# rahul003/dmlc-core

Measured on AMD Instinct MI355X. Metric: parsed rows/sec (LibSVM->CSR in device memory), aggregate over GPUs, higher is better.
Workload: dtype fp32 values / u32 indices (text parse, no matmul)

## Files before the change

dmlc_core_amd/data/__init__.py:

```python
from __future__ import annotations

from typing import Dict, Iterator, Optional

from .. import _dmlc

__all__ = ["Parser", "RowBlockIter", "GPUParser", "ShuffledGPUParser", "DeviceCSR", "csr_to_torch",
           "iter_blocks", "write_synthetic", "to_sparse_csr", "GPUBlockDataset", "PageCache",
           "write_page_cache", "RowBatches", "row_order"]

write_synthetic = _dmlc.write_synthetic
pack_text = _dmlc.pack_text
pack_isa_supported = _dmlc.pack_isa_supported
unpack_text_reference = _dmlc.unpack_text_reference
unpack_text_device = _dmlc.unpack_text_device


def _host_blocks_uri(uri: str) -> str:
    q = uri.split("#", 1)[0]
    if "?" not in q:
        return uri
    args = dict(kv.split("=", 1) for kv in q.split("?", 1)[1].split("&") if "=" in kv)
    if not args.get("device", "").startswith("gpu") or "to_host" in args:
        return uri
    head, _, tail = uri.partition("#")
    return head + "&to_host=1" + ("#" + tail if tail else "")


def Parser(uri: str, part: int = 0, nparts: int = 1, type: str = "auto",
           index64: bool = False):
    cls = _dmlc.Parser64 if index64 else _dmlc.Parser
    return cls(_host_blocks_uri(uri), part, nparts, type)


def RowBlockIter(uri: str, part: int = 0, nparts: int = 1, type: str = "auto",
                 index64: bool = False):
    cls = _dmlc.RowBlockIter64 if index64 else _dmlc.RowBlockIter
    return cls(_host_blocks_uri(uri), part, nparts, type)


def iter_blocks(uri: str, part: int = 0, nparts: int = 1, type: str = "auto",
                index64: bool = False) -> Iterator[Dict]:
    p = Parser(uri, part, nparts, type, index64)
    while p.next():
        yield p.value()


def DeviceCSR(index64: bool = False):
    return _dmlc.DeviceCSR64() if index64 else _dmlc.DeviceCSR()


def PageCache(path: str, device: int = -1, index64: bool = False):
    cls = _dmlc.PageCache64 if index64 else _dmlc.PageCache
    return cls.open(path, device)


def write_page_cache(csr, path: str, page_mb: float = 64.0) -> int:
    cls = _dmlc.PageCache64 if isinstance(csr, _dmlc.DeviceCSR64) else _dmlc.PageCache
    return cls.write(csr, path, page_mb)


class GPUParser:

    def __init__(self, uri: str, part: int = 0, nparts: int = 1, format: str = "libsvm",
                 index64: bool = False, **config):
        cfg = {"format": format}
        cfg.update({k: str(v) for k, v in config.items()})
        self.index64 = index64
        self._where = {"uri": uri, "part": part, "nparts": nparts, "format": format}
        cls = _dmlc.DeviceParser64 if index64 else _dmlc.DeviceParser
        self._p = cls(uri, part, nparts, cfg)

    def parse_all(self, out=None):
        if out is None:
            out = DeviceCSR(self.index64)
        self._p.parse_all(out)
        return out

    def parse_all_hashed(self, dim: int, seed: int = 0, fp8: bool = True, scale: float = 1.0,
                         strategy: str = "auto", out: Optional[Dict] = None):
        import torch
        import torch.utils.dlpack as tdl

        if strategy not in ("auto", "fused", "csr"):
            raise ValueError(f"strategy must be auto, fused or csr, not {strategy!r}")
        if strategy == "csr":
            from .. import ops

            t = csr_to_torch(self.parse_all())
            x = ops.hashed_dense(t, int(dim), seed=seed, fp8=fp8, scale=scale)
            return {"x": x, "label": t["label"].clone(), "batch": None}

        handle = out.get("batch") if isinstance(out, dict) else out
        if handle is not None and torch.cuda.is_available():
            if getattr(self, "_ext_stream", None) is None:
                self._ext_stream = torch.cuda.ExternalStream(self._p.stream())
            self._ext_stream.wait_stream(torch.cuda.current_stream())
        d = self._p.parse_all_hashed(int(dim), float(scale), int(seed) & 0xFFFFFFFF, bool(fp8), handle)
        if isinstance(out, dict) and out.get("batch") is d["batch"] and "x" in out:
            x0 = out["x"]
            if (tuple(x0.shape) == (d["rows"], d["dim"]) and x0.data_ptr() == d["x_ptr"]
                    and out["label"].data_ptr() == d["label_ptr"]
                    and (x0.dtype == torch.float8_e4m3fn) == bool(fp8)):
                return out
        x = tdl.from_dlpack(d["x"]).view(d["rows"], d["dim"])
        if fp8:
            x = x.view(torch.float8_e4m3fn)
        return {"x": x, "label": tdl.from_dlpack(d["label"]), "batch": d["batch"]}

    def before_first(self):
        self._p.before_first()

    def tell(self) -> int:
        return self._p.tell()

    def seek(self, cursor: int) -> None:
        self._p.seek(int(cursor))

    def state_dict(self) -> Dict:
        return dict(self._where, cursor=self.tell())

    def load_state_dict(self, state: Dict) -> None:
        for k in ("uri", "part", "nparts", "format"):
            if state[k] != self._where[k]:
                raise ValueError(f"state is for {k}={state[k]!r}, parser has {self._where[k]!r}")
        self.seek(state["cursor"])

    def next(self) -> bool:
        return self._p.next()

    def value_to_host(self) -> Dict:
        return self._p.value_to_host()

    def value_torch(self) -> Dict:
        import torch.utils.dlpack as tdl

        return {k: None if c is None else tdl.from_dlpack(c)
                for k, c in self._p.value_capsules().items()}

    def stream(self) -> int:
        return self._p.stream()

    def stats(self) -> Dict:
        return self._p.stats()

    @property
    def partition_bytes(self) -> int:
        return self._p.partition_bytes()


class ShuffledGPUParser(GPUParser):

    def __init__(self, uri: str, part: int = 0, nparts: int = 1, num_shuffle_parts: int = 2,
                 shuffle_seed: int = 0, format: str = "libsvm", index64: bool = False,
                 **config):
        if num_shuffle_parts < 1:
            raise ValueError("num_shuffle_parts must be >= 1")
        self.k, self.seed = int(num_shuffle_parts), int(shuffle_seed)
        super().__init__(uri, part, nparts, format=format, index64=index64,
                         shuffle_parts=self.k, shuffle_seed=self.seed, **config)
        self._where.update(num_shuffle_parts=self.k, shuffle_seed=self.seed)

    @property
    def order(self):
        return list(self._p.visit_order())

    @property
    def epoch(self) -> int:
        return self._p.epoch()

    def state_dict(self) -> Dict:
        return dict(self._where, epoch=self.epoch, cursor=self.tell())

    def load_state_dict(self, state: Dict) -> None:
        for k in ("uri", "part", "nparts", "format", "num_shuffle_parts", "shuffle_seed"):
            if state[k] != self._where[k]:
                raise ValueError(f"state is for {k}={state[k]!r}, parser has {self._where[k]!r}")
        self._p.set_epoch(int(state["epoch"]))
        self.seek(state["cursor"])


def csr_to_torch(csr) -> Dict[str, Optional["object"]]:
    import torch.utils.dlpack as tdl

    out = {}
    for k, cap in csr.capsules().items():
        out[k] = None if cap is None else tdl.from_dlpack(cap)
    return out


def to_sparse_csr(t: Dict, num_cols: Optional[int] = None):
    import torch

    offset = t["offset"]
    crow = (offset.view(torch.int64) if offset.dtype == torch.uint64 else offset).to(torch.int64)
    crow = crow - crow[0]
    idx = t["index"]
    if idx.dtype == torch.uint32:
        col = idx.view(torch.int32).to(torch.int64)
    elif idx.dtype == torch.uint64:
        col = idx.view(torch.int64)
    else:
        col = idx.to(torch.int64)
    base = int(offset[0].item()) if offset.numel() else 0
    nnz = int(crow[-1].item()) if crow.numel() else 0
    col = col[base:base + nnz]
    val = t.get("value")
    val = torch.ones(nnz, dtype=torch.float32, device=col.device) if val is None else val[base:base + nnz]
    ncols = int(num_cols) if num_cols is not None else (int(col.max().item()) + 1 if nnz else 0)
    return torch.sparse_csr_tensor(crow, col, val, size=(crow.numel() - 1, ncols))


class GPUBlockDataset:

    def __init__(self, uri: str, part: int = 0, nparts: int = 1, format: str = "libsvm",
                 epochs: int = 1, **config):
        self.args = (uri, part, nparts, format, config)
        self.epochs = epochs

    def __iter__(self):
        uri, part, nparts, fmt, config = self.args
        p = GPUParser(uri, part, nparts, format=fmt, **config)
        for epoch in range(self.epochs):
            if epoch:
                p.before_first()
            while p.next():
                yield p.value_torch()


def row_order(n_rows: int, seed: int, epoch: int):
    import torch

    if n_rows < 0 or epoch < 0:
        raise ValueError("n_rows and epoch must be >= 0")
    g = torch.Generator(device="cpu")
    g.manual_seed((int(seed) * 1000003 + int(epoch)) % (1 << 32))
    return torch.randperm(int(n_rows), generator=g, dtype=torch.int64)


class RowBatches:

    def __init__(self, csr_dict: Dict, batch_rows: int, shuffle: bool = True, seed: int = 0,
                 drop_last: bool = False, buffers: int = 2):
        if batch_rows < 1:
            raise ValueError("batch_rows must be >= 1")
        if buffers < 1:
            raise ValueError("buffers must be >= 1")
        self.csr = csr_dict
        self.n_rows = int(csr_dict["offset"].numel()) - 1
        self.batch_rows, self.shuffle, self.seed = int(batch_rows), bool(shuffle), int(seed)
        self.drop_last, self.buffers = bool(drop_last), int(buffers)
        self.epoch, self._next = 0, 0
        self._out = [None] * self.buffers
        self._order = None

    def __len__(self) -> int:
        if self.drop_last:
            return self.n_rows // self.batch_rows
        return (self.n_rows + self.batch_rows - 1) // self.batch_rows

    def set_epoch(self, epoch: int) -> None:
        if epoch < 0:
            raise ValueError("epoch must be >= 0")
        self.epoch, self._next = int(epoch), 0

    def batch_bounds(self, k: int):
        if not 0 <= k < len(self):
            raise IndexError(f"batch {k} of {len(self)}")
        b = k * self.batch_rows
        return b, min(self.n_rows, b + self.batch_rows)

    def state_dict(self) -> Dict:
        return {"seed": self.seed, "epoch": self.epoch, "next_batch": self._next,
                "batch_rows": self.batch_rows, "n_rows": self.n_rows}

    def load_state_dict(self, state: Dict) -> None:
        for k in ("seed", "batch_rows", "n_rows"):
            if state[k] != getattr(self, k):
                raise ValueError(f"state is for {k}={state[k]!r}, iterator has {getattr(self, k)!r}")
        nb = int(state["next_batch"])
        if not 0 <= nb <= len(self):
            raise ValueError(f"state is for next_batch={nb}, iterator has {len(self)} batches")
        self.epoch, self._next = int(state["epoch"]), nb

    def _device_order(self):
        import torch

        if self._order is None or self._order[0] != (self.epoch, self.shuffle):
            dev = self.csr["index"].device
            if self.shuffle:
                order = row_order(self.n_rows, self.seed, self.epoch).to(dev)
            else:
                order = torch.arange(self.n_rows, dtype=torch.int64, device=dev)
            self._order = ((self.epoch, self.shuffle), order)
        return self._order[1]

    def _gather(self, rows, slot: int) -> Dict:
        from .. import ops

        out = self._out[slot]
        if out is None or out["_buffers"]["offset"].numel() < rows.numel() + 2:
            return ops.gather_rows(self.csr, rows)
        try:
            return ops.gather_rows(self.csr, rows, out=self._out[slot])
        except ops._GatherOutTooSmall as e:
            grown = ops.gather_buffers(self.csr, self.batch_rows, e.nnz + e.nnz // 4)
            return ops.gather_rows(self.csr, rows, out=grown)

    def __iter__(self):
        order = self._device_order() if len(self) > self._next else None
        while self._next < len(self):
            k = self._next
            b, e = self.batch_bounds(k)
            item = self._gather(order[b:e], k % self.buffers)
            self._out[k % self.buffers] = item
            self._next = k + 1
# ... 3 lines not shown
```

include/dmlc/gpu/device_parser.h:

```cpp
#ifndef DMLC_GPU_DEVICE_PARSER_H_
#define DMLC_GPU_DEVICE_PARSER_H_

#include <map>
#include <memory>
#include <string>
#include <vector>

#include "./device_row_block.h"

namespace dmlc {
namespace gpu {

struct DeviceParserConfig {
  std::string format{"libsvm"};
  size_t chunk_bytes{64UL << 20};
  int pinned_slots{3};
  int device_slots{3};
  int read_threads{8};
  int device{-1};
  int label_column{-1};
  int weight_column{-1};
  char delimiter{','};
  bool fast_path{true};
  bool one_pass{false};
  bool hash_one_pass{false};
  bool prelaunch{true};
  int zero_copy{-1};
  int packed_h2d{-1};
  bool pack_wait{false};
  bool pack_head{true};
  int copy_streams{2};
  size_t zc_pin_budget{64UL << 30};
  size_t zc_window_bytes{1UL << 30};
  bool hbm_cache{false};
  size_t replay_chunk_bytes{(2UL << 30) - (64UL << 20)};
  size_t replay_first_bytes{0};
  double wait_spin_us{50};
  unsigned shuffle_parts{1};
  int shuffle_seed{0};
  void Update(const std::map<std::string, std::string>& args);
};

struct DeviceHashedBatch {
  std::shared_ptr<DeviceBuffer> x{std::make_shared<DeviceBuffer>()};
  std::shared_ptr<DeviceBuffer> label{std::make_shared<DeviceBuffer>()};
  size_t rows{0}, row_cap{0};
  int dim{0};
  bool fp8{true};
  int device{0};
  void Reserve(size_t rows, hipStream_t stream);
};

struct DeviceParserStats {
  size_t bytes{0};
  size_t chunks{0};
  size_t rows{0};
  size_t nnz{0};
  size_t exact_chunks{0};
  size_t one_pass_chunks{0};
  size_t one_pass_reruns{0};
  double wait_reader_sec{0};
  double wait_gpu_sec{0};
  bool zero_copy{false};
  double register_sec{0};
  size_t zc_pin_budget{0}, zc_pinned_peak{0};
  double last_pass_sec{0}, last_fill_sec{0}, last_drain_sec{0};
  size_t waits_spun{0}, waits_slept{0}, waits_timed_out{0};
  size_t packed_chunks{0}, raw_chunks{0}, link_bytes{0}, exception_blocks{0};
  size_t head_packed{0};
  double pack_sec{0}, wait_pack_sec{0}, wait_pack_idle_sec{0};
  size_t unpack_staging_bytes{0};
};

template <typename IndexType>
class DeviceParser {
 public:
  static DeviceParser* Create(const std::string& uri, unsigned part_index, unsigned num_parts,
                              const DeviceParserConfig& cfg = DeviceParserConfig());
  virtual ~DeviceParser() = default;
  virtual void BeforeFirst() = 0;
  virtual size_t Tell() const = 0;
  virtual void Seek(size_t cursor) = 0;
  virtual unsigned Epoch() const { return 0; }
  virtual void SetEpoch(unsigned ) {}
  virtual std::vector<unsigned> VisitOrder() const { return {0}; }
  virtual bool Next() = 0;
  virtual const DeviceRowBlock<IndexType>& Value() const = 0;
  virtual void ParseAll(DeviceCSR<IndexType>* out) = 0;
  virtual void ParseAllHashed(DeviceHashedBatch* out, int dim, float scale, uint32_t seed,
                              bool fp8) = 0;
  virtual size_t PartitionBytes() const = 0;
  virtual const DeviceParserStats& Stats() const = 0;
  virtual hipStream_t stream() const = 0;
};

}
}
#endif
```

src/gpu/chunk_feed.cc:

```cpp
#include "./chunk_feed.h"

#include <dmlc/fault.h>
#include <dmlc/logging.h>
#include <dmlc/timer.h>

#include <algorithm>
#include <cstring>

#include "../io/filesys.h"
#include "../io/line_split.h"
#include "./kernels.h"
#include "./text_pack.h"

namespace dmlc {
namespace gpu {

ChunkFeed::ChunkFeed(const std::string& uri, unsigned part, unsigned nparts,
                     const DeviceParserConfig& cfg, bool csv_alphabet, hipStream_t compute,
                     DeviceParserStats* stats)
    : cfg_(cfg),
      compute_(compute),
      stats_(stats),
      walk_(&plan_, cfg.replay_first_bytes, cfg.replay_chunk_bytes) {
  io::URI path(uri.c_str());
  split_.reset(new io::LineSplitter(io::FileSystem::GetInstance(path), uri.c_str(), part, nparts));
  if (cfg_.shuffle_parts > 1) {
    const unsigned k = cfg_.shuffle_parts;
    std::vector<std::vector<EpochOrder::Segment>> subs;
    for (unsigned i = 0; i < k; ++i) {
      split_->ResetPartition(part * k + i, nparts * k);
      subs.push_back(split_->ShardSegments());
    }
    order_ = EpochOrder(part, nparts, k, cfg_.shuffle_seed, subs);
    reader_.reset(new io::ShardReader(split_.get(), cfg_.read_threads, order_.Segments(),
                                      order_.Stops()));
  } else {
    order_ = EpochOrder(part, nparts, 1, cfg_.shuffle_seed, {split_->ShardSegments()});
    reader_.reset(new io::ShardReader(split_.get(), cfg_.read_threads));
  }
  ncopy_ = (cfg_.copy_streams == 1 || cfg_.hbm_cache) ? 1 : 2;
  for (size_t s = 0; s < ncopy_; ++s) copy_[s].reset(new Stream());
  zeroed_.reset(new Event());
  for (int d = 0; d < cfg_.device_slots; ++d) {
    dtext_.emplace_back(new DeviceBuffer(cfg_.chunk_bytes + kTextPadBytes));
    MemsetOrdered(dtext_.back()->get(), cfg_.chunk_bytes + kTextPadBytes);
    copied_.emplace_back(new Event());
    parsed_.emplace_back(new Event());
    parsed_.back()->Record(compute_);
  }
  iter_.set_max_capacity(static_cast<size_t>(cfg_.pinned_slots));
  if (cfg_.zero_copy != 0) {
    zc_.reset(new ZeroCopySource());
    const double t0 = GetTime();
    zc_->SetDrain([this]() {
      RescueLookahead();
      SyncCopyStreams();
    });
    stats_->zc_pin_budget = ZeroCopySource::ShardPinBudget(cfg_.zc_pin_budget);
    if (!zc_->Init(split_.get(), cfg_.chunk_bytes, stats_->zc_pin_budget, cfg_.zc_window_bytes,
                   order_.shuffled() ? &order_.all_segments() : nullptr)) {
      CHECK(cfg_.zero_copy != 1) << "zero_copy=1 but the input cannot be mmap'ed + registered";
      zc_.reset();
    } else {
      stats_->register_sec = GetTime() - t0;
      stats_->zero_copy = true;
      if (order_.shuffled()) zc_->Reorder(order_.SegmentIndices());
    }
  }
  if (zc_ == nullptr) StartReader();
  if (zc_ != nullptr &&
      (cfg_.packed_h2d == 1 ||
       (cfg_.packed_h2d < 0 && cfg_.read_threads >= 2 && cfg_.chunk_bytes >= (size_t(1) << 20)))) {
    StartPacking(csv_alphabet);
  }
  if (cfg_.hbm_cache) StartCaching();
}

ChunkFeed::~ChunkFeed() {
  for (auto& s : copy_) {
    if (s) (void)hipStreamSynchronize(s->get());
  }
  if (unpack_) (void)hipStreamSynchronize(unpack_->get());
  (void)hipStreamSynchronize(compute_);
  for (auto& f : inflight_) {
    if (f.slot != nullptr) iter_.Recycle(&f.slot);
  }
  inflight_.clear();
  iter_.Destroy();
  pool_.reset();
  zc_.reset();
}

void ChunkFeed::SyncCopyStreams() const {
  for (size_t s = 0; s < ncopy_; ++s) copy_[s]->Synchronize();
}

void ChunkFeed::MemsetOrdered(void* ptr, size_t bytes) {
  DMLC_HIP_CHECK(hipMemsetAsync(ptr, 0, bytes, copy_[0]->get()));
  if (ncopy_ < 2) return;
  zeroed_->Record(copy_[0]->get());
  DMLC_HIP_CHECK(hipStreamWaitEvent(copy_[1]->get(), zeroed_->get(), 0));
}

bool ChunkFeed::SetEpoch(unsigned e) {
  if (head_) DropLookahead();
  if (!order_.shuffled()) return Seek(0);
  DrainInflight();
  order_.Apply(e);
  if (zc_ != nullptr) {
    zc_->Reorder(order_.SegmentIndices());
  } else {
    reorder_reader_ = true;
  }
  return Seek(0);
}

bool ChunkFeed::Seek(size_t cursor) {
  CHECK_LE(cursor, PartitionBytes()) << "DeviceParser::Seek: cursor beyond the partition";
  const bool keep_prelaunch = cursor == 0 && cache_complete_ && !order_.shuffled();
  if (cursor == 0 && reader_done_ && inflight_.empty() && busy_ == 0 && cursor_ != 0 &&
      cursor_ == PartitionBytes()) {
    head_armed_ = true;
  }
  const bool adopt = head_ && cursor == 0 && !(cfg_.hbm_cache && cache_complete_);
  DrainInflight(adopt);
  replay_ = false;
  caching_ = false;
  if (cfg_.hbm_cache) {
    if (cache_complete_) {
      plan_.Build(order_);
      const size_t i = plan_.FindCursor(cursor, PartitionBytes());
      if (i != ReplayPlan::kNotABoundary) {
        replay_ = true;
        walk_.Start(i);
        cursor_ = cursor;
        return keep_prelaunch;
      }
    } else if (cursor == 0) {
      StartCaching();
    } else {
      plan_.Clear();
      arena_fill_ = 0;
    }
  }
  if (zc_ != nullptr) {
    if (!adopt) zc_->Seek(cursor);
  } else {
    seek_pos_ = cursor;
    iter_.BeforeFirst();
  }
  cursor_ = cursor;
  return keep_prelaunch;
}

void ChunkFeed::StartReader() {
  const size_t cap = cfg_.chunk_bytes;
  io::ShardReader* reader = reader_.get();
  iter_.Init(
      [reader, cap](HostSlot** dptr) {
        if (*dptr == nullptr) {
          *dptr = new HostSlot();
          (*dptr)->buf.Reserve(cap + kTextPadBytes);
          (*dptr)->cap = cap;
        }
        ScopedRange r("pinned_fill");
        HostSlot* slot = *dptr;
        size_t n = reader->Fill(slot->buf.get<char>(), slot->cap);
        while (n == io::ShardReader::kNeedMore) {
          slot->cap = reader->NeedCapacity();
          slot->buf.Free();
          slot->buf.Reserve(slot->cap + kTextPadBytes);
          n = reader->Fill(slot->buf.get<char>(), slot->cap);
        }
        (*dptr)->size = n;
        (*dptr)->end_pos = reader->Tell();
        return (*dptr)->size != 0;
      },
      [this, reader]() {
        if (reorder_reader_) {
          reader->SetSegments(order_.Segments(), order_.Stops());
          reorder_reader_ = false;
        }
        reader->Seek(seek_pos_);
      });
}

bool ChunkFeed::NextPiece(Piece* out) {
  if (pool_ != nullptr) {
    out->job = NextPackJob();
    if (out->job == nullptr) return false;
    out->src = out->job->ptr;
    out->size = out->job->size;
    out->end_pos = out->job->end_pos;
  } else if (zc_ != nullptr) {
    ZeroCopySource::Piece piece;
    if (!zc_->Next(&piece)) return false;
    out->src = piece.ptr;
    out->size = piece.size;
    out->end_pos = zc_->Tell();
  } else {
    const double t0 = GetTime();
    if (!iter_.Next(&out->slot)) return false;
    stats_->wait_reader_sec += GetTime() - t0;
    out->src = out->slot->buf.get();
    out->size = out->slot->size;
    out->end_pos = out->slot->end_pos;
  }
  return true;
}

void ChunkFeed::FillFromCache() {
  while (static_cast<int>(inflight_.size()) < cfg_.device_slots && !walk_.AtEnd()) {
    const ReplayPlan::Step s = walk_.Next(merge_);
    inflight_.push_back(
        Inflight{nullptr, -1, s.size, s.end_pos, arena_->get<char>() + s.off, -1, false});
  }
  reader_done_ = walk_.AtEnd();
}

size_t ChunkFeed::CacheChunk(const Piece& p) {
  const size_t begin_pos = plan_.cached_end();
  CHECK_LE(arena_fill_ + p.size, arena_bytes_) << "HBM cache arena overflow";
  const char last = p.job != nullptr ? p.job->last
                    : p.size != 0    ? static_cast<const char*>(p.src)[p.size - 1]
                                     : '\n';
  CachedChunk c{arena_fill_, p.size, begin_pos, p.end_pos, 0, 0, 0, last == '\n' || last == '\r'};
  c.sub = order_.SubOf(begin_pos, &c.sub_begin);
  c.sub_end = c.sub_begin + (p.end_pos - begin_pos);
  CHECK_LE(c.sub_end, order_.sub_bytes(c.sub)) << "internal error: a chunk spans two sub-shards";
  plan_.Add(c);
  arena_fill_ += p.size;
  return c.off;
}

void ChunkFeed::FillPipeline() {
  if (replay_) {
    FillFromCache();
    return;
  }
  while (static_cast<int>(inflight_.size()) + busy_ < cfg_.device_slots && !reader_done_) {
    if (pool_ != nullptr && !PreparePackJob()) break;
    if (zc_ != nullptr) DMLC_FAULT_POINT("read");
    DMLC_FAULT_POINT("h2d");
    Piece p;
    if (!NextPiece(&p)) {
      reader_done_ = true;
      if (caching_) cache_complete_ = true;
      QueueHeadJobs();
      break;
    }
    const PackJob* job = p.job.get();
    const size_t size = p.size;
    const int d = next_dslot_;
    next_dslot_ = (next_dslot_ + 1) % cfg_.device_slots;
    if (size + kTextPadBytes > dtext_[d]->bytes()) {
      parsed_[d]->Synchronize();
      dtext_[d].reset(new DeviceBuffer(size + kTextPadBytes));
      MemsetOrdered(dtext_[d]->get(), size + kTextPadBytes);
    }
    char* dst = dtext_[d]->get<char>();
    if (caching_) dst = arena_->get<char>() + CacheChunk(p);
    const size_t cs = pass_chunks_++ % ncopy_;
    hipStream_t copy = copy_[cs]->get();
    DMLC_HIP_CHECK(hipStreamWaitEvent(copy, parsed_[d]->get(), 0));
    int pack_slot = -1;
    const bool packed = job != nullptr && job->state.load() == PackJob::kPacked;
    if (packed) {
      if (dstage_[d] == nullptr || dstage_[d]->bytes() < job->packed_bytes) {
        parsed_[d]->Synchronize();
        if (dstage_[d] != nullptr) stats_->unpack_staging_bytes -= dstage_[d]->bytes();
        dstage_[d].reset(
            new DeviceBuffer(std::max(job->packed_bytes, PackSlotBytes(cfg_.chunk_bytes))));
        stats_->unpack_staging_bytes += dstage_[d]->bytes();
      }
      DMLC_HIP_CHECK(hipMemcpyAsync(dstage_[d]->get(), job->out, job->packed_bytes,
                                    hipMemcpyHostToDevice, copy));
      copied_[d]->Record(copy);
      DMLC_HIP_CHECK(hipStreamWaitEvent(unpack_->get(), copied_[d]->get(), 0));
      LaunchUnpackText(dstage_[d]->get(), size, job->nexc, alphabet_, dst, unpack_->get());
      unpacked_[d]->Record(unpack_->get());
      pack_slot = job->slot;
      stats_->packed_chunks += 1;
      if (job->head && job->seq == 0) stats_->head_packed += 1;
      stats_->exception_blocks += job->nexc;
      stats_->link_bytes += job->packed_bytes;
    } else {
      DMLC_HIP_CHECK(hipMemcpyAsync(dst, p.src, size, hipMemcpyHostToDevice, copy));
      stats_->raw_chunks += 1;
      stats_->link_bytes += size;
      if (job != nullptr) {
        if (job->rescued) {
          pack_slot = job->slot;
        } else {
          free_pack_slots_.push_back(job->slot);
        }
      }
      copied_[d]->Record(copy);
    }
    last_copy_d_[cs] = d;
    inflight_.push_back(Inflight{p.slot, d, size, p.end_pos, dst, pack_slot, packed});
  }
}

void ChunkFeed::StartPacking(bool csv_alphabet) {
  PackAlphabet(csv_alphabet, cfg_.delimiter, alphabet_);
  pool_.reset(new PackPool(cfg_.read_threads, alphabet_, 0));
  pack_slots_ =
      std::vector<PinnedBuffer>(kPackLookahead + static_cast<size_t>(cfg_.device_slots) + 1);
  for (size_t i = 0; i < pack_slots_.size(); ++i) free_pack_slots_.push_back(static_cast<int>(i));
  dstage_.resize(static_cast<size_t>(cfg_.device_slots));
  unpack_.reset(new Stream());
  for (int d = 0; d < cfg_.device_slots; ++d) unpacked_.emplace_back(new Event());
}

size_t ChunkFeed::PackSlotBytes(size_t n, bool may_hold_raw) const {
  const size_t packed = static_cast<size_t>(kPackMaxRatio * static_cast<double>(n)) + 64;
  return std::max<size_t>(may_hold_raw ? std::max(packed, n) : packed, 4096);
}

bool ChunkFeed::LinkBusy() const {
  for (size_t s = 0; s < ncopy_; ++s) {
    if (last_copy_d_[s] >= 0 && !copied_[last_copy_d_[s]]->Query()) return true;
  }
  return false;
}

void ChunkFeed::FetchLookahead(size_t limit, bool head) {
  while (!la_end_ && la_.size() < limit) {
    ZeroCopySource::Piece piece;
    if (!zc_->Next(&piece)) {
      la_end_ = true;
      break;
    }
    std::unique_ptr<PackJob> job(new PackJob());
    job->ptr = piece.ptr;
    job->size = piece.size;
    job->end_pos = zc_->Tell();
    if (piece.size != 0) job->last = piece.ptr[piece.size - 1];
    job->seq = la_seq_++;
    job->head = head;
    CHECK(!free_pack_slots_.empty()) << "internal error: no free pack slot";
    job->slot = free_pack_slots_.back();
    free_pack_slots_.pop_back();
    PinnedBuffer& buf = pack_slots_[job->slot];
    if (buf.bytes() < PackSlotBytes(piece.size, zc_->windowed())) {
      buf.Reserve(PackSlotBytes(std::max(piece.size, cfg_.chunk_bytes), zc_->windowed()));
    }
    job->out = buf.get<uint8_t>();
    la_.push_back(std::move(job));
  }
}

void ChunkFeed::QueueHeadJobs() {
  if (pool_ == nullptr || !cfg_.pack_head || !head_armed_ || cfg_.pack_wait ||
      cfg_.shuffle_parts > 1 || zc_->windowed() || (cfg_.hbm_cache && cache_complete_)) {
    return;
  }
  CHECK(la_.empty()) << "internal error: lookahead left at the end of a pass";
  la_seq_ = submitted_ = la_pushed_ = 0;
  la_end_ = front_unpushed_ = false;
  pool_->SetSubmitted(0);
  zc_->Seek(0);
  FetchLookahead(kHeadJobs, true);
  for (; la_pushed_ < la_.size(); ++la_pushed_) pool_->Push(la_[la_pushed_].get());
  head_ = true;
}

bool ChunkFeed::PreparePackJob() {
  FetchLookahead(kPackLookahead, false);
  if (la_.empty()) return true;
  PackJob* job = la_.front().get();
  const int state = job->state.load();
  next_action_ = job->rescued ? SubmitAction::kSubmit
                              : DecideSubmit(state, cfg_.pack_wait != 0,
                                             inflight_.empty(), pool_behind_,
                                             [this]() { return LinkBusy(); });
  if (pool_behind_ && !job->rescued) {
    packed_in_a_row_ = state == PackJob::kPacked ? packed_in_a_row_ + 1 : 0;
    if (packed_in_a_row_ >= kPackCaughtUp) SetPoolBehind(false);
  }
  if (la_pushed_ == 0 && next_action_ == SubmitAction::kClaimRaw) {
    front_unpushed_ = true;
    la_pushed_ = 1;
  } else if (front_unpushed_ && next_action_ != SubmitAction::kClaimRaw) {
    front_unpushed_ = false;
    if (job->state.load() == PackJob::kQueued) pool_->Push(job);
  }
  for (; la_pushed_ < la_.size(); ++la_pushed_) {
    if (la_[la_pushed_]->state.load() == PackJob::kQueued) pool_->Push(la_[la_pushed_].get());
  }
  return next_action_ != SubmitAction::kDefer;
}

void ChunkFeed::SetPoolBehind(bool behind) {
  pool_behind_ = behind;
  packed_in_a_row_ = 0;
  pool_->SetDistance(behind ? kPackDistance : 0);
}

std::unique_ptr<PackJob> ChunkFeed::NextPackJob() {
  if (la_.empty()) return nullptr;
  std::unique_ptr<PackJob> job = std::move(la_.front());
  la_.pop_front();
  --la_pushed_;
  front_unpushed_ = false;
  pool_->SetSubmitted(++submitted_);
  if (next_action_ == SubmitAction::kClaimRaw && !pool_->TryClaimRaw(job.get())) {
    next_action_ = SubmitAction::kWait;
  }
  if (next_action_ == SubmitAction::kWait) {
    const bool idle = !LinkBusy();
    const double t0 = GetTime();
    try {
      pool_->Wait(job.get());
    } catch (...) {
      free_pack_slots_.push_back(job->slot);
      throw;
    }
    stats_->wait_pack_sec += GetTime() - t0;
    if (idle) {
      stats_->wait_pack_idle_sec += GetTime() - t0;
      if (WaitMeansPoolBehind(idle, cfg_.pack_wait, job->head && job->seq == 0)) {
        SetPoolBehind(true);
      }
    }
  }
  stats_->pack_sec = pool_->pack_sec();
  return job;
}

void ChunkFeed::RescueLookahead() {
  for (auto& job : la_) {
    if (job->rescued || !zc_->Releasing(job->ptr)) continue;
    if (!pool_->TryClaimRaw(job.get())) {
      try {
        pool_->Wait(job.get());
      } catch (...) {
        job->state.store(PackJob::kRejected);
      }
    }
    if (job->state.load() == PackJob::kPacked) continue;
    std::memcpy(job->out, job->ptr, job->size);
    job->ptr = reinterpret_cast<const char*>(job->out);
    job->rescued = true;
  }
}

void ChunkFeed::DropLookahead() {
  if (pool_ == nullptr) return;
  pool_->Quiesce();
  for (auto& job : la_) free_pack_slots_.push_back(job->slot);
  la_.clear();
  la_end_ = false;
  front_unpushed_ = false;
  head_ = false;
  la_seq_ = submitted_ = la_pushed_ = 0;
  pool_->SetSubmitted(0);
}

void ChunkFeed::ReleasePackSlot(int* pack_slot) {
  if (*pack_slot < 0) return;
  free_pack_slots_.push_back(*pack_slot);
  *pack_slot = -1;
}

void ChunkFeed::StartCaching() {
  plan_.Clear();
  arena_fill_ = 0;
  cache_complete_ = false;
  if (arena_ == nullptr) {
    arena_bytes_ =
        PartitionBytes() + std::max(split_->files().size(), order_.all_segments().size()) + 16;
    arena_.reset(new DeviceBuffer(arena_bytes_ + kTextPadBytes));
    MemsetOrdered(arena_->get(), arena_bytes_ + kTextPadBytes);
  }
  caching_ = true;
}

void ChunkFeed::DrainInflight(bool keep_head) {
  SyncCopyStreams();
  if (unpack_) unpack_->Synchronize();
  DMLC_HIP_CHECK(hipStreamSynchronize(compute_));
  while (!inflight_.empty()) {
    if (inflight_.front().slot != nullptr) iter_.Recycle(&inflight_.front().slot);
    ReleasePackSlot(&inflight_.front().pack_slot);
    inflight_.pop_front();
  }
  ReleasePackSlot(&cur_.pack_slot);
  if (keep_head) {
    head_ = false;
  } else {
    DropLookahead();
  }
  last_copy_d_[0] = last_copy_d_[1] = -1;
  pass_chunks_ = 0;
  reader_done_ = false;
  busy_ = 0;
}

bool ChunkFeed::Acquire(Chunk* out) {
  FillPipeline();
  if (inflight_.empty()) return false;
  cur_ = inflight_.front();
  inflight_.pop_front();
  busy_ = 1;
  if (cur_.d >= 0) {
    Event* ready = cur_.packed ? unpacked_[cur_.d].get() : copied_[cur_.d].get();
    DMLC_HIP_CHECK(hipStreamWaitEvent(compute_, ready->get(), 0));
  }
  out->text = cur_.text;
  out->size = cur_.size;
  out->resident = cur_.d < 0;
  return true;
}

void ChunkFeed::FirstSyncDone() {
  if (cur_.slot != nullptr) iter_.Recycle(&cur_.slot);
  ReleasePackSlot(&cur_.pack_slot);
  FillPipeline();
}

void ChunkFeed::Release(bool delivered) {
  if (!delivered) {
    (void)hipStreamSynchronize(compute_);
    if (cur_.d >= 0) (void)hipEventRecord(parsed_[cur_.d]->get(), compute_);
    busy_ = 0;
    ReleasePackSlot(&cur_.pack_slot);
    if (head_) DropLookahead();
    if (cur_.slot != nullptr) {
      try {
        iter_.Recycle(&cur_.slot);
      } catch (...) {
      }
    }
    return;
  }
  if (cur_.slot != nullptr) iter_.Recycle(&cur_.slot);
  ReleasePackSlot(&cur_.pack_slot);
  if (cur_.d >= 0) parsed_[cur_.d]->Record(compute_);
  busy_ = 0;
  cursor_ = cur_.end_pos;
  stats_->bytes += cur_.size;
  stats_->chunks += 1;
  if (zc_ != nullptr) stats_->zc_pinned_peak = zc_->PeakPinnedBytes();
}

bool ChunkFeed::PeekNextResident(const char** text, size_t* size) const {
  if (inflight_.empty() || inflight_.front().d >= 0) return false;
  *text = inflight_.front().text;
  *size = inflight_.front().size;
  return true;
}

bool ChunkFeed::NextEpochFirst(const char** text, size_t* size) const {
  if (!replay_ || !inflight_.empty() || !reader_done_ || order_.shuffled()) return false;
  ReplayPlan::Step s;
  if (!walk_.NextEpochFirst(merge_, &s) || s.size == 0) return false;
  *text = arena_->get<char>() + s.off;
  *size = s.size;
  return true;
}

}
}
```

src/gpu/chunk_feed.h:

```cpp
#ifndef DMLC_SRC_GPU_CHUNK_FEED_H_
#define DMLC_SRC_GPU_CHUNK_FEED_H_

#include <dmlc/gpu/device_parser.h>
#include <dmlc/gpu/hip_utils.h>
#include <dmlc/threadediter.h>

#include <deque>
#include <memory>
#include <string>
#include <vector>

#include "../io/input_split_base.h"
#include "../io/shard_reader.h"
#include "./epoch_order.h"
#include "./pack_pool.h"
#include "./replay_plan.h"
#include "./zero_copy_source.h"

namespace dmlc {
namespace gpu {

class ChunkFeed {
 public:
  struct Chunk {
    const char* text{nullptr};
    size_t size{0};
    bool resident{false};
  };

  ChunkFeed(const std::string& uri, unsigned part, unsigned nparts, const DeviceParserConfig& cfg,
            bool csv_alphabet, hipStream_t compute, DeviceParserStats* stats);
  ~ChunkFeed();
  ChunkFeed(const ChunkFeed&) = delete;
  ChunkFeed& operator=(const ChunkFeed&) = delete;

  bool Seek(size_t cursor);
  bool SetEpoch(unsigned e);
  bool BeforeFirst() { return order_.shuffled() ? SetEpoch(order_.epoch() + 1) : Seek(0); }
  size_t Tell() const { return cursor_; }
  unsigned Epoch() const { return order_.epoch(); }
  const std::vector<unsigned>& VisitOrder() const { return order_.order(); }
  size_t PartitionBytes() const {
    return zc_ != nullptr ? zc_->PartitionBytes() : reader_->PartitionBytes();
  }

  bool Acquire(Chunk* out);
  void FirstSyncDone();
  void Release(bool delivered);

  bool Replaying() const { return replay_; }
  bool MergingReplay() const { return replay_ && merge_.merge; }
  bool InputDone() const { return reader_done_; }

  bool PeekNextResident(const char** text, size_t* size) const;
  bool NextEpochFirst(const char** text, size_t* size) const;

  class ReplayMerge {
   public:
    ReplayMerge(ChunkFeed* feed, size_t limit) : feed_(feed) {
      feed_->merge_ = ReplayMergeSettings{true, limit};
    }
    ~ReplayMerge() { feed_->merge_ = ReplayMergeSettings(); }
    ReplayMerge(const ReplayMerge&) = delete;
    ReplayMerge& operator=(const ReplayMerge&) = delete;

   private:
    ChunkFeed* feed_;
  };

 private:
  struct HostSlot {
    PinnedBuffer buf;
    size_t cap{0};
    size_t size{0};
    size_t end_pos{0};
  };
  struct Inflight {
    HostSlot* slot;
    int d;
    size_t size;
    size_t end_pos;
    const char* text;
    int pack_slot;
    bool packed;
  };
  struct Piece {
    HostSlot* slot{nullptr};
    const void* src{nullptr};
    size_t size{0}, end_pos{0};
    std::unique_ptr<PackJob> job;
  };
  static constexpr size_t kPackLookahead = 4;
  static constexpr size_t kPackDistance = 2;
  static constexpr size_t kPackCaughtUp = 8;
  static constexpr size_t kHeadJobs = 2;

  void SyncCopyStreams() const;
  void MemsetOrdered(void* ptr, size_t bytes);
  void FetchLookahead(size_t limit, bool head);
  void QueueHeadJobs();
  void StartReader();
  void StartPacking(bool csv_alphabet);
  void StartCaching();
  void FillPipeline();
  void FillFromCache();
  bool NextPiece(Piece* out);
  size_t CacheChunk(const Piece& p);
  size_t PackSlotBytes(size_t n, bool may_hold_raw = false) const;
  bool LinkBusy() const;
  bool PreparePackJob();
  void SetPoolBehind(bool behind);
  std::unique_ptr<PackJob> NextPackJob();
  void RescueLookahead();
  void DropLookahead();
  void ReleasePackSlot(int* pack_slot);
  void DrainInflight(bool keep_head = false);

  DeviceParserConfig cfg_;
  hipStream_t compute_;
  DeviceParserStats* stats_;
  std::unique_ptr<io::InputSplitBase> split_;
  std::unique_ptr<io::ShardReader> reader_;
  EpochOrder order_;
  std::unique_ptr<Stream> copy_[2];
  size_t ncopy_{2};
  size_t pass_chunks_{0};
  std::unique_ptr<Event> zeroed_;
  std::vector<std::unique_ptr<DeviceBuffer>> dtext_;
  std::vector<std::unique_ptr<Event>> copied_, parsed_;
  ThreadedIter<HostSlot> iter_;
  std::unique_ptr<ZeroCopySource> zc_;
  std::unique_ptr<PackPool> pool_;
  std::deque<std::unique_ptr<PackJob>> la_;
  bool la_end_{false};
  size_t la_seq_{0}, submitted_{0};
  size_t la_pushed_{0};
  bool front_unpushed_{false};
  bool pool_behind_{false};
  size_t packed_in_a_row_{0};
  SubmitAction next_action_{SubmitAction::kSubmit};
  bool head_{false};
  bool head_armed_{false};
  int last_copy_d_[2]{-1, -1};
  std::vector<PinnedBuffer> pack_slots_;
  std::vector<int> free_pack_slots_;
  std::vector<std::unique_ptr<DeviceBuffer>> dstage_;
  std::unique_ptr<Stream> unpack_;
  std::vector<std::unique_ptr<Event>> unpacked_;
  uint8_t alphabet_[16];
  std::deque<Inflight> inflight_;
  Inflight cur_{nullptr, -1, 0, 0, nullptr, -1, false};
  int busy_{0};
  int next_dslot_{0};
  bool reader_done_{false};
  size_t cursor_{0};
  bool reorder_reader_{false};
  size_t seek_pos_{0};
  std::unique_ptr<DeviceBuffer> arena_;
  size_t arena_bytes_{0}, arena_fill_{0};
  bool caching_{false}, cache_complete_{false}, replay_{false};
  ReplayPlan plan_;
  ReplayWalk walk_;
  ReplayMergeSettings merge_;
};

}
}
#endif
```

src/gpu/device_parser.cc:

```cpp
#include <dmlc/gpu/device_parser.h>
#include <dmlc/fault.h>
#include <dmlc/logging.h>
#include <dmlc/timer.h>

#include <cstdlib>

#include <algorithm>
#include <cstring>
#include <memory>
#include <vector>

#include "../io/uri_spec.h"
#include "./chunk_feed.h"
#include "./host_wait.h"
#include "./kernels.h"
#include "./tile_pipeline.h"

namespace dmlc {
namespace gpu {

void DeviceParserConfig::Update(const std::map<std::string, std::string>& args) {
  for (const auto& kv : args) {
    const std::string& k = kv.first;
    const std::string& v = kv.second;
    if (k == "chunk_mb") {
      chunk_bytes = static_cast<size_t>(std::atof(v.c_str()) * (1 << 20));
    } else if (k == "chunk_bytes") {
      chunk_bytes = std::strtoull(v.c_str(), nullptr, 10);
    } else if (k == "pinned_slots") {
      pinned_slots = std::atoi(v.c_str());
    } else if (k == "device_slots") {
      device_slots = std::atoi(v.c_str());
    } else if (k == "read_threads") {
      read_threads = std::atoi(v.c_str());
    } else if (k == "device") {
      device = std::atoi(v.c_str());
    } else if (k == "format") {
      format = v;
    } else if (k == "label_column") {
      label_column = std::atoi(v.c_str());
    } else if (k == "weight_column") {
      weight_column = std::atoi(v.c_str());
    } else if (k == "delimiter") {
      CHECK_EQ(v.size(), 1U) << "delimiter must be one character";
      delimiter = v[0];
    } else if (k == "fast_path") {
      fast_path = v != "0" && v != "false";
    } else if (k == "one_pass") {
      one_pass = v != "0" && v != "false";
    } else if (k == "hash_one_pass") {
      hash_one_pass = v != "0" && v != "false";
    } else if (k == "prelaunch") {
      prelaunch = v != "0" && v != "false";
    } else if (k == "replay_chunk_mb") {
      replay_chunk_bytes = static_cast<size_t>(std::atof(v.c_str()) * (1 << 20));
    } else if (k == "replay_first_mb") {
      replay_first_bytes = static_cast<size_t>(std::atof(v.c_str()) * (1 << 20));
    } else if (k == "zc_pin_budget_mb") {
      zc_pin_budget = static_cast<size_t>(std::atof(v.c_str()) * (1 << 20));
    } else if (k == "zc_window_mb") {
      zc_window_bytes = static_cast<size_t>(std::atof(v.c_str()) * (1 << 20));
    } else if (k == "hbm_cache") {
      hbm_cache = v != "0" && v != "false";
    } else if (k == "wait_spin_us") {
      wait_spin_us = std::atof(v.c_str());
    } else if (k == "shuffle_parts") {
      shuffle_parts = static_cast<unsigned>(std::atoi(v.c_str()));
    } else if (k == "shuffle_seed") {
      shuffle_seed = std::atoi(v.c_str());
    } else if (k == "zero_copy") {
      zero_copy = (v == "auto" || v == "-1") ? -1 : ((v == "0" || v == "false") ? 0 : 1);
    } else if (k == "pack_wait") {
      pack_wait = v != "0" && v != "false";
    } else if (k == "pack_head") {
      pack_head = v != "0" && v != "false";
    } else if (k == "copy_streams") {
      copy_streams = std::atoi(v.c_str());
    } else if (k == "packed_h2d") {
      packed_h2d = (v == "auto" || v == "-1") ? -1 : ((v == "0" || v == "false") ? 0 : 1);
    }
  }
  chunk_bytes = (chunk_bytes + 4095) & ~size_t(4095);
  CHECK_GE(chunk_bytes, 4096U) << "chunk_bytes too small";
  CHECK_LT(chunk_bytes, size_t(1) << 31) << "chunk_bytes must be < 2 GiB";
  CHECK_LT(replay_chunk_bytes, size_t(1) << 31) << "replay_chunk_bytes must be < 2 GiB";
  CHECK_GE(pinned_slots, 1);
  CHECK_GE(device_slots, 1);
  CHECK(copy_streams == 1 || copy_streams == 2) << "copy_streams must be 1 or 2";
  CHECK_GE(shuffle_parts, 1U) << "shuffle_parts must be >= 1";
}

namespace {

struct ChunkPlan {
  size_t nlines{0}, ntok{0};
  uint64_t nrows{0}, nnz{0};
  unsigned flags{0};
};

template <typename IndexType>
class DeviceParserImpl : public DeviceParser<IndexType> {
 public:
  DeviceParserImpl(const std::string& uri, unsigned part, unsigned nparts,
                   const DeviceParserConfig& cfg)
      : cfg_(cfg) {
    if (cfg_.device >= 0) SetDevice(cfg_.device);
    DMLC_HIP_CHECK(hipGetDevice(&device_));
    if (cfg_.format == "libsvm") {
      tcfg_.format = TextFormat::kLibSVM;
    } else if (cfg_.format == "libfm") {
      tcfg_.format = TextFormat::kLibFM;
    } else if (cfg_.format == "csv") {
      tcfg_.format = TextFormat::kCSV;
    } else {
      LOG(FATAL) << "DeviceParser: unsupported format " << cfg_.format;
    }
    CHECK(tcfg_.format != TextFormat::kCSV || cfg_.label_column < 0 ||
          cfg_.label_column != cfg_.weight_column)
        << "label_column and weight_column must differ";
    tcfg_.label_column = cfg_.label_column;
    tcfg_.weight_column = cfg_.weight_column;
    tcfg_.delimiter = cfg_.delimiter;
    int least_prio = 0, greatest_prio = 0;
    DMLC_HIP_CHECK(hipDeviceGetStreamPriorityRange(&least_prio, &greatest_prio));
    compute_.reset(new Stream(greatest_prio));
    feed_.reset(new ChunkFeed(uri, part, nparts, cfg_, tcfg_.format == TextFormat::kCSV,
                              compute_->get(), &stats_));
    tiles_.Reserve(LineIndexTiles(cfg_.chunk_bytes) * sizeof(uint64_t));
    pre_.Init(2 * sizeof(ChunkMeta), cfg_.hbm_cache);
    pre_.cur.Reserve(TileCount(cfg_.chunk_bytes), true);
    hmeta_.Reserve(2 * sizeof(ChunkMeta));
    slots_.Reserve(std::max<size_t>(kMaxPartialBlocks, TileScratchSlots(TileCount(cfg_.chunk_bytes))) *
                   sizeof(MetaPartial));
  }

  ~DeviceParserImpl() override {
    if (compute_) (void)hipStreamSynchronize(compute_->get());
    if (pre_.stream) (void)hipStreamSynchronize(pre_.stream->get());
  }

  void BeforeFirst() override {
    if (!feed_->BeforeFirst()) pre_.Drop();
  }
  void SetEpoch(unsigned e) override {
    if (!feed_->SetEpoch(e)) pre_.Drop();
  }
  void Seek(size_t cursor) override {
    if (!feed_->Seek(cursor)) pre_.Drop();
  }
  unsigned Epoch() const override { return feed_->Epoch(); }
  std::vector<unsigned> VisitOrder() const override { return feed_->VisitOrder(); }
  size_t Tell() const override { return feed_->Tell(); }

  bool Next() override {
    block_.Clear();
    block_.device_ = device_;
    ResetEpoch();
    if (!ProcessOne(&block_, false)) return false;
    FinishEpoch(&block_);
    view_ = block_.View();
    return true;
  }

  const DeviceRowBlock<IndexType>& Value() const override { return view_; }

  void ParseAll(DeviceCSR<IndexType>* out) override {
    ScopedRange range("DeviceParser::ParseAll");
    out->device_ = device_;
    ResetEpoch();
    const bool one_pass = cfg_.one_pass && feed_->Replaying() && cfg_.fast_path &&
                          tcfg_.format != TextFormat::kCSV && !one_pass_off_;
    ChunkFeed::ReplayMerge merge(feed_.get(), one_pass ? ResidentMergeLimit() : 0);
    const double t0 = GetTime();
    double t_first = 0, t_last_in = 0;
    while (ProcessOne(out, true)) {
      const double t = GetTime();
      if (t_first == 0) t_first = t;
      if (feed_->InputDone() && t_last_in == 0) t_last_in = t;
    }
    FinishEpoch(out);
    const double t_end = GetTime();
    stats_.last_pass_sec = t_end - t0;
    stats_.last_fill_sec = t_first != 0 ? t_first - t0 : 0;
    stats_.last_drain_sec = t_last_in != 0 ? t_end - t_last_in : 0;
  }

  size_t PartitionBytes() const override { return feed_->PartitionBytes(); }
  const DeviceParserStats& Stats() const override { return stats_; }
  hipStream_t stream() const override { return compute_->get(); }

 private:
  void ResetEpoch() {
    acc_max_index_ = acc_max_field_ = 0;
    acc_flags_ = 0;
  }

  ChunkMeta WaitMapped(ChunkMeta* hm) {
    const double t0 = GetTime();
    const ChunkMeta v = TakePublished(hm, cfg_.wait_spin_us, 0.05, &wait_stats_, [this] {
      compute_->Synchronize();
      if (pre_.stream) pre_.stream->Synchronize();
    });
    stats_.wait_gpu_sec += GetTime() - t0;
    stats_.waits_spun = wait_stats_.spun;
    stats_.waits_slept = wait_stats_.slept;
    stats_.waits_timed_out = wait_stats_.timed_out;
    return v;
  }

  template <typename T>
  T ReadBack(const void* src) {
    const double t0 = GetTime();
    DMLC_HIP_CHECK(hipMemcpyAsync(hmeta_.get(), src, sizeof(T), hipMemcpyDeviceToHost,
                                  compute_->get()));
    compute_->Synchronize();
    stats_.wait_gpu_sec += GetTime() - t0;
    T v;
    std::memcpy(&v, hmeta_.get(), sizeof(T));
    return v;
  }

  size_t ForPartition(uint64_t n, size_t nbytes, double margin) const {
    const double scale =
        static_cast<double>(PartitionBytes()) / std::max<size_t>(nbytes, 1) * margin;
    return static_cast<size_t>(n * scale) + 1;
  }

  size_t ResidentMergeLimit() const {
    return std::min(2 * cfg_.replay_chunk_bytes, (size_t(1) << 31) - (size_t(64) << 20));
  }

  void EnsureScratch(size_t nbytes) {
    const size_t tiles = TileCount(nbytes);
    pre_.cur.Reserve(tiles, true);
    slots_.Reserve(std::max<size_t>(kMaxPartialBlocks, TileScratchSlots(tiles)) * sizeof(MetaPartial));
    tiles_.Reserve(LineIndexTiles(nbytes) * sizeof(uint64_t));
  }

  void EnsureLineBuffers(size_t nlines) {
    lines_.Reserve((nlines + 1) * sizeof(uint32_t));
    info_.Reserve((nlines + 1) * sizeof(uint64_t));
    partials_.Reserve((ScanPartials(nlines) + 2) * sizeof(uint64_t));
  }

  FillTarget<IndexType> MakeFillTarget(DeviceCSR<IndexType>* out, size_t row_base, size_t nnz_base,
                                       size_t row_limit, size_t nnz_limit, bool with_qid) {
    FillTarget<IndexType> tgt;
    tgt.offset = out->offset();
    tgt.label = out->label();
    tgt.weight = out->weight_capacity() >= out->row_capacity() && out->row_capacity() != 0
                     ? out->weight()
                     : nullptr;
    tgt.qid = with_qid ? out->qid() : nullptr;
    tgt.field = tcfg_.format == TextFormat::kLibFM ? out->field() : nullptr;
    tgt.index = out->index();
    tgt.value = out->value();
    tgt.row_base = row_base;
    tgt.nnz_base = nnz_base;
    tgt.row_limit = row_limit;
    tgt.nnz_limit = nnz_limit;
    return tgt;
  }

  FillTarget<IndexType> PrepareOutput(DeviceCSR<IndexType>* out, size_t row_base, size_t nnz_base,
                                      const ChunkPlan& plan, bool need_weight, size_t nbytes) {
    hipStream_t s = compute_->get();
    const bool libfm = tcfg_.format == TextFormat::kLibFM;
    if (row_base == 0) {
      out->Reserve(ForPartition(plan.nrows, nbytes, 1.05), ForPartition(plan.nnz, nbytes, 1.05),
                   libfm, s, 0, 0);
    }
    out->Reserve(row_base + plan.nrows, nnz_base + plan.nnz, libfm, s, row_base, nnz_base);
    if (need_weight) out->EnableWeight(s);
    if (plan.flags & kFlagQid) {
      out->EnableQid(s);
      out->has_qid_ = true;
    }
    return MakeFillTarget(out, row_base, nnz_base, row_base + plan.nrows, nnz_base + plan.nnz,
                          out->has_qid_);
  }

  void LaunchCountScan(const char* text, size_t nbytes, const TileScratchSet& set, hipStream_t s) {
    uint64_t* counts = set.counts.get<uint64_t>();
    uint32_t* flags = set.flags.get<uint32_t>();
    uint32_t* masks = set.masks.get<uint32_t>();
    if (tcfg_.format == TextFormat::kCSV) {
      LaunchCsvTileCount(text, nbytes, tcfg_.label_column, tcfg_.weight_column, tcfg_.delimiter,
                         counts, flags, masks, s);
      LaunchTileScanRaw(counts, flags, TileCount(nbytes), set.dmeta(), set.hmeta(), s);
    } else {
      LaunchTileCountScan(text, nbytes, counts, flags, masks, set.dmeta(), set.hmeta(), s);
    }
  }

  void CountScanCurrent(const char* text, size_t nbytes) {
    if (pre_.Adopt(text, nbytes, compute_->get())) return;
    pre_.Drop();
    LaunchCountScan(text, nbytes, pre_.cur, compute_->get());
  }

  bool FastParse(const char* text, size_t nbytes, DeviceCSR<IndexType>* out, size_t row_base,
                 size_t nnz_base, ChunkPlan* plan) {
    hipStream_t s = compute_->get();
    CountScanCurrent(text, nbytes);
    ChunkMeta* dmeta = pre_.cur.dmeta();
    ChunkMeta* hm = pre_.cur.hmeta();
    const ChunkMeta sizes = WaitMapped(hm);
    feed_->FirstSyncDone();
    if (sizes.flags & kFlagIrregular) return false;
    plan->nlines = sizes.nlines;
    plan->nrows = sizes.nrows;
    plan->nnz = sizes.nnz;
    if (tcfg_.format == TextFormat::kLibSVM) plan->flags |= sizes.flags & kFlagQid;
    bool need_weight = false;
    for (;;) {
      FillTarget<IndexType> tgt = PrepareOutput(out, row_base, nnz_base, *plan, need_weight, nbytes);
      if (tgt.qid != nullptr && plan->nrows != 0) {
        DMLC_HIP_CHECK(hipMemsetAsync(tgt.qid + row_base, 0, plan->nrows * sizeof(uint64_t), s));
      }
      LaunchTileFill<IndexType>(text, nbytes, tcfg_.format, pre_.cur.counts.get<uint64_t>(),
                                pre_.cur.masks.get<uint32_t>(), tgt,
                                slots_.get<MetaPartial>(), dmeta, hm, s);
      PrelaunchCount();
      ChunkMeta m = WaitMapped(hm);
      if (m.flags & kFlagIrregular) return false;
      if ((m.flags & kFlagNeedWeight) && !need_weight) {
        need_weight = true;
        m.flags &= ~kFlagNeedWeight;
        DMLC_HIP_CHECK(hipMemcpyAsync(dmeta, &sizes, sizeof(ChunkMeta), hipMemcpyHostToDevice, s));
        continue;
      }
      CHECK(!(m.flags & kFlagNeedWeight)) << "internal error: weight column not allocated";
      Accumulate(m);
      return true;
    }
  }

  bool CsvFastParse(const char* text, size_t nbytes, DeviceCSR<IndexType>* out, size_t row_base,
                    size_t nnz_base, ChunkPlan* plan) {
    hipStream_t s = compute_->get();
    const size_t ntiles = TileCount(nbytes);
    CountScanCurrent(text, nbytes);
    ChunkMeta* dmeta = pre_.cur.dmeta();
    ChunkMeta* hm = pre_.cur.hmeta();
    const ChunkMeta sizes = WaitMapped(hm);
    feed_->FirstSyncDone();
    if (sizes.flags & kFlagIrregular) return false;
    plan->nlines = sizes.nrows;
    plan->nrows = sizes.nrows;
    plan->nnz = sizes.nnz;
    const bool need_weight = tcfg_.weight_column >= 0;
    FillTarget<IndexType> tgt = PrepareOutput(out, row_base, nnz_base, *plan, need_weight, nbytes);
    LaunchCsvTileFill<IndexType>(text, nbytes, tcfg_.label_column, tcfg_.weight_column,
                                 tcfg_.delimiter, pre_.cur.counts.get<uint64_t>(),
                                 pre_.cur.masks.get<uint32_t>(), tgt,
                                 slots_.get<MetaPartial>(), s);
    LaunchTileFinish(slots_.get<MetaPartial>(), ntiles, dmeta, hm, tgt.offset, row_base, nnz_base,
                     s);
    PrelaunchCount();
    const ChunkMeta m = WaitMapped(hm);
    if (m.flags & kFlagIrregular) return false;
    Accumulate(m);
    return true;
  }

  ChunkPlan ExactIndex(const char* text, size_t nbytes, bool first_sync_done) {
    hipStream_t s = compute_->get();
    ChunkMeta* dmeta = pre_.cur.dmeta();
    ChunkPlan plan;
    DMLC_HIP_CHECK(hipMemsetAsync(dmeta, 0, sizeof(ChunkMeta), s));
    LaunchLineCount(text, nbytes, tiles_.get<uint64_t>(), dmeta, s);
    plan.nlines = ReadBack<ChunkMeta>(dmeta).nlines;
    if (!first_sync_done) feed_->FirstSyncDone();
    EnsureLineBuffers(plan.nlines);
    LaunchLineEmit(text, nbytes, tiles_.get<uint64_t>(), lines_.get<uint32_t>(), s);
    LaunchTextCount(text, nbytes, lines_.get<uint32_t>(), plan.nlines, tcfg_,
                    info_.get<uint64_t>(), slots_.get<MetaPartial>(), dmeta, s);
    uint64_t* total = partials_.get<uint64_t>() + ScanPartials(plan.nlines) + 1;
    LaunchScanU64(info_.get<uint64_t>(), plan.nlines, partials_.get<uint64_t>(), total, s);
    LaunchMetaFromTotal(total, dmeta, s);
// ... 322 lines not shown
```

src/gpu/kernels.h:

```cpp
#ifndef DMLC_GPU_KERNELS_H_
#define DMLC_GPU_KERNELS_H_

#include <hip/hip_runtime_api.h>

#include <cstddef>
#include <cstdint>

namespace dmlc {
namespace gpu {

constexpr size_t kTextPadBytes = 4096;
constexpr size_t kLineTileBytes = 4096;

enum class TextFormat : int { kLibSVM = 0, kLibFM = 1, kCSV = 2 };

struct TextParseConfig {
  TextFormat format{TextFormat::kLibSVM};
  int label_column{-1};
  int weight_column{-1};
  char delimiter{','};
};

struct ChunkMeta {
  unsigned long long nlines;
  unsigned long long nrows;
  unsigned long long nnz;
  unsigned long long max_index;
  unsigned long long max_field;
  unsigned int flags;
  unsigned int pad;
};
constexpr unsigned kFlagWeight = 1u;
constexpr unsigned kFlagQid = 2u;
constexpr unsigned kFlagValue = 4u;
constexpr unsigned kFlagField = 8u;
constexpr unsigned kFlagNegIndex = 256u;
constexpr unsigned kFlagOverflow = 512u;

struct MetaPartial {
  unsigned long long max_index;
  unsigned long long max_field;
  unsigned int flags;
  unsigned int pad;
};
constexpr int kMaxPartialBlocks = 8192;
void LaunchReducePartials(const MetaPartial* partials, int nblocks, ChunkMeta* meta,
                          hipStream_t stream);

struct CsrView {
  const uint64_t* offset;
  const void* index;
  const float* value;
  const void* field;
  size_t nrows;
  bool index64;
  bool paired;
};

template <typename IndexType>
struct FillTarget {
  uint64_t* offset;
  float* label;
  float* weight;
  uint64_t* qid;
  IndexType* field;
  IndexType* index;
  float* value;
  uint64_t row_base;
  uint64_t nnz_base;
  uint64_t row_limit;
  uint64_t nnz_limit;
};

size_t LineIndexTiles(size_t nbytes);
size_t ScanPartials(size_t n);

void LaunchLineCount(const char* text, size_t nbytes, uint64_t* tile_scratch, ChunkMeta* meta,
                     hipStream_t stream);
void LaunchLineEmit(const char* text, size_t nbytes, const uint64_t* tile_scratch,
                    uint32_t* line_starts, hipStream_t stream);

void LaunchTextCount(const char* text, size_t nbytes, const uint32_t* line_starts,
                     size_t nlines, const TextParseConfig& cfg, uint64_t* line_info,
                     MetaPartial* partials, ChunkMeta* meta, hipStream_t stream);

void LaunchScanU64(uint64_t* data, size_t n, uint64_t* partials, uint64_t* total,
                   hipStream_t stream);

void LaunchMetaFromTotal(const uint64_t* total, ChunkMeta* meta, hipStream_t stream);

template <typename IndexType>
void LaunchTextFill(const char* text, size_t nbytes, const uint32_t* line_starts,
                    size_t nlines, const TextParseConfig& cfg, const uint64_t* line_info,
                    const FillTarget<IndexType>& out, uint64_t nrows, uint64_t nnz,
                    MetaPartial* partials, ChunkMeta* meta, hipStream_t stream);

void LaunchCloseOffsets(uint64_t* offset, uint64_t row_end, uint64_t nnz_end, hipStream_t stream);

constexpr unsigned kFlagIrregular = 1024u;

struct LookBack {
  uint64_t* status;
  unsigned long long* ticket;
  unsigned long long ticket0;
};
constexpr size_t kTileBytes = 8192;
constexpr unsigned kFlagNeedWeight = 2048u;
size_t TileCount(size_t nbytes);
size_t TileScratchWords(size_t ntiles);
size_t TileScratchSlots(size_t ntiles);
void LaunchTileCountScan(const char* text, size_t nbytes, uint64_t* tile_counts,
                         uint32_t* tile_flags, uint32_t* tile_masks, ChunkMeta* meta,
                         ChunkMeta* host_meta, hipStream_t stream);
size_t TileMaskWords(size_t ntiles);
struct FillOnePass : LookBack {};
template <typename IndexType>
size_t LaunchTileFill(const char* text, size_t nbytes, TextFormat format,
                      const uint64_t* tile_prefix, const uint32_t* tile_masks,
                      const FillTarget<IndexType>& out, MetaPartial* partials, ChunkMeta* meta,
                      ChunkMeta* host_meta, hipStream_t stream,
                      const FillOnePass* one_pass = nullptr);

struct HashOnePass : LookBack {
  uint32_t tag;
  uint64_t row_cap;
};
template <typename IndexType>
size_t LaunchTileHashed(const char* text, size_t nbytes, TextFormat format,
                        const uint64_t* tile_prefix, const uint32_t* tile_masks,
                        uint64_t row_base, uint64_t nlines, int dim,
                        float scale, uint32_t seed, bool fp8, void* out, float* labels,
                        MetaPartial* partials, ChunkMeta* meta, ChunkMeta* host_meta,
                        hipStream_t stream, const HashOnePass* one_pass = nullptr);

void LaunchTileScanRaw(uint64_t* tile_counts, uint32_t* tile_flags, size_t ntiles,
                       ChunkMeta* meta, ChunkMeta* host_meta, hipStream_t stream);
void LaunchTileFinish(MetaPartial* partials, size_t nslots, ChunkMeta* meta, ChunkMeta* host_meta,
                      uint64_t* offset, uint64_t row_base, uint64_t nnz_base, hipStream_t stream);

void LaunchCsvTileCount(const char* text, size_t nbytes, int label_column, int weight_column,
                        char delimiter, uint64_t* tile_counts, uint32_t* tile_flags,
                        uint32_t* tile_masks, hipStream_t stream);
template <typename IndexType>
void LaunchCsvTileFill(const char* text, size_t nbytes, int label_column, int weight_column,
                       char delimiter, const uint64_t* tile_prefix, const uint32_t* tile_masks,
                       const FillTarget<IndexType>& out, MetaPartial* partials,
                       hipStream_t stream);

constexpr uint32_t kRecErrTruncated = 1;
constexpr uint32_t kRecErrBadPart = 2;
size_t RecordIOTiles(size_t nwords);
void LaunchRecordIOTileCount(const uint32_t* words, size_t nwords, uint64_t* tile_counts,
                             uint32_t* tile_flags, hipStream_t stream);
struct RecordIOOnePass : LookBack {
  ChunkMeta* meta;
  uint64_t rec_cap;
  uint64_t byte_cap;
};
struct RecordIOCaps {
  ChunkMeta* meta;
  uint64_t rec_cap;
  uint64_t byte_cap;
};
size_t LaunchRecordIOTileFill(const uint32_t* words, size_t nwords, const uint64_t* tile_prefix,
                              uint64_t* offset, uint64_t rec_base, uint8_t* data,
                              uint64_t byte_base, MetaPartial* partials, hipStream_t stream,
                              const RecordIOOnePass* one_pass = nullptr,
                              const RecordIOCaps* caps = nullptr);
void LaunchRecordIOTileCountChain(const uint32_t* words, size_t nwords, uint64_t* tile_counts,
                                  uint32_t* tile_flags, hipStream_t stream);
void LaunchRecordIOGather(const uint8_t* src, const uint64_t* src_off, const uint32_t* len,
                          const uint64_t* dst_off, size_t nrec, uint8_t* dst, hipStream_t stream);

void LaunchHashedDenseFP8(const CsrView& csr, int dim, float scale, uint32_t seed, uint8_t* out,
                          hipStream_t stream);
void LaunchHashedDenseF32(const CsrView& csr, int dim, uint32_t seed, float* out,
                          hipStream_t stream);
template <typename IndexType>
void LaunchTextHashed(const char* text, size_t nbytes, const uint32_t* line_starts, size_t nlines,
                      TextFormat format, const uint64_t* line_info, uint64_t row_base, int dim,
                      float scale, uint32_t seed, bool fp8, void* out, float* labels,
                      MetaPartial* partials, ChunkMeta* meta, hipStream_t stream);
void LaunchCSRSpMV(const CsrView& csr, const float* w, float bias, float* y, hipStream_t stream);
void LaunchCSRSpMVT(const CsrView& csr, const float* d, float* g, hipStream_t stream);
constexpr int kSpMMMaxCols = 256;
void LaunchCSRSpMM(const CsrView& csr, const float* w, const float* bias, int k, float* y,
                   hipStream_t stream);
void LaunchCSRSpMMT(const CsrView& csr, const float* d, int k, float* g, hipStream_t stream);
constexpr int kFFMMaxRank = 32;
constexpr uint32_t kFFMStagedRowEntries = 128;
constexpr uint32_t kFFMErrIndex = 1, kFFMErrField = 2;
void LaunchFFMForward(const CsrView& csr, const float* v, uint64_t features, int num_fields, int k,
                      float* y, int* error, hipStream_t stream);
void LaunchFFMBackward(const CsrView& csr, const float* g, const float* v, uint64_t features,
                       int num_fields, int k, float* dv, hipStream_t stream);
constexpr uint32_t kRankMaxLabel = 31;
constexpr uint32_t kRankWaveGroupRows = 256;
constexpr uint32_t kRankTileRows = 256;
constexpr uint32_t kRankErrGroup = 1, kRankErrLabel = 2;
void LaunchQidFlags(const uint64_t* qid, size_t rows, uint64_t* flag, hipStream_t stream);
void LaunchQidGroupPtr(const uint64_t* qid, size_t rows, const uint64_t* scanned,
                       const uint64_t* total, uint64_t capacity, uint64_t* group_ptr,
                       hipStream_t stream);
void LaunchRankLoss(const float* score, const float* label, const uint64_t* group_ptr, size_t groups,
                    uint64_t rows, bool ndcg_weights, float sigma, float* row_scratch, float* grad,
                    float* loss_g, int64_t* pairs_g, int* error, hipStream_t stream);
void LaunchRankNdcg(const float* score, const float* label, const uint64_t* group_ptr, size_t groups,
                    uint64_t rows, uint32_t k, float* ndcg, int* error, hipStream_t stream);
constexpr int kFmRank = 16;
constexpr int kFmCols = kFmRank + 1;
size_t FmForwardSharedBytes(int dim);
void LaunchFmForward(const uint8_t* x, int64_t rows, int dim, const void* wt_bf16, const float* q,
                     const float* bias, float sx, float* y, float* xv, int num_cus,
                     hipStream_t stream);
void LaunchFmBackward(const uint8_t* x, int64_t rows, int dim, const float* g, const float* xv,
                      int nblocks, float* part, hipStream_t stream);
void LaunchFmPrep(const float* w, const float* v, int dim, void* wt_bf16, float* q,
                  hipStream_t stream);
void LaunchFmReduceGrads(const float* part, int nblocks, int dim, const float* v, float sx,
                         float* z, float* gw, float* gv, hipStream_t stream);
enum FmLoss : int { kFmLogistic = 0, kFmSquared = 1 };
constexpr int kFmFusedMaxDim = 1024;
void LaunchFmFused(const uint8_t* x, int64_t rows, int dim, const void* wt_bf16, const float* q,
                   const float* bias, float sx, const float* label, const float* weight,
                   int loss, float inv_n, int nblocks, float* y, float* part, float* lpart,
                   hipStream_t stream);

void LaunchOffsetRebase(const uint64_t* src_offset, size_t nrows, uint64_t src_base,
                        uint64_t dst_base, uint64_t* dst_offset, hipStream_t stream);
void LaunchPageRebase(uint64_t* offset, size_t nrows, const uint64_t* page_row_end,
                      const uint64_t* page_nnz_base, int npages, hipStream_t stream);
void LaunchCSRTranspose(const CsrView& csr, uint64_t base, uint64_t nnz, uint64_t num_features,
                        uint64_t* col_ptr, uint32_t* row_out, float* val_out, void* scratch,
                        uint32_t* error, hipStream_t stream);
size_t CSRTransposeScratchBytes(uint64_t nnz, uint64_t num_features);
uint64_t CSRTransposeMaxFeatures();
constexpr uint32_t kGatherErrRow = 1;
constexpr uint32_t kGatherErrCapacity = 2;
constexpr uint32_t kGatherErrSource = 4;
uint64_t CSRGatherRunEntries();
size_t CSRGatherScratchWords(size_t n_sel);
void LaunchCSRGatherCount(const uint64_t* offset, uint64_t nrows_src, uint64_t src_entries,
                          const void* rows, bool rows64, size_t n_sel, const float* label,
                          const float* weight, const uint64_t* qid, uint64_t* out_offset,
                          float* out_label, float* out_weight, uint64_t* out_qid, uint32_t* error,
                          hipStream_t stream);
void LaunchCSRGatherFill(const CsrView& src, uint64_t src_entries, const void* rows, bool rows64,
                         size_t n_sel, uint64_t* out_offset, const uint64_t* total,
                         void* out_index, float* out_value, void* out_field,
                         uint64_t out_capacity, uint32_t* error, hipStream_t stream);
constexpr uint64_t kCompactMaxFeatures = 1ull << 32;
constexpr uint32_t kCompactErrIndex = 1;
size_t CompactScratchBytes(uint64_t num_features);
void LaunchCompactMark(const CsrView& csr, uint64_t base, uint64_t nnz, uint64_t num_features,
                       void* scratch, uint32_t* error, hipStream_t stream);
void LaunchCompactCount(uint64_t num_features, void* scratch, uint64_t* total, hipStream_t stream);
void LaunchCompactEmit(uint64_t num_features, const void* scratch, uint64_t capacity, int64_t* ids,
                       hipStream_t stream);
void LaunchCompactRemap(const CsrView& csr, uint64_t base, uint64_t nnz, uint64_t num_features,
                        const void* scratch, int32_t* slot, hipStream_t stream);
enum LazyRule : int { kLazyAdagrad = 0, kLazyFtrl = 1 };
struct LazyHyper {
  float a, b, c, d;
};
constexpr uint32_t kLazyErrIds = 1;
void LaunchLazyUpdate(int rule, float* param, const int64_t* ids, const float* grad, float* state0,
                      float* state1, uint64_t features, uint64_t nrows, uint64_t width,
                      const LazyHyper& hyper, uint32_t* error, hipStream_t stream);
void LaunchFill(float* p, size_t n, float v, hipStream_t stream);
void LaunchUnpackText(const void* packed, size_t n, uint32_t nexc, const uint8_t alphabet[16],
                      char* dst, hipStream_t stream);

}
}
#endif
```

src/gpu/pack_pool.h:

```cpp
#ifndef DMLC_SRC_GPU_PACK_POOL_H_
#define DMLC_SRC_GPU_PACK_POOL_H_

#include <dmlc/fault.h>
#include <dmlc/logging.h>
#include <dmlc/timer.h>

#include <algorithm>
#include <atomic>
#include <condition_variable>
#include <cstring>
#include <deque>
#include <exception>
#include <memory>
#include <mutex>
#include <thread>
#include <vector>

#include "./text_pack.h"

namespace dmlc {
namespace gpu {

struct PackJob {
  enum State : int { kQueued = 0, kPacking, kPacked, kRejected, kClaimedRaw, kFailed };
  const char* ptr{nullptr};
  size_t size{0};
  size_t end_pos{0};
  char last{'\n'};
  size_t seq{0};
  int slot{-1};
  uint8_t* out{nullptr};
  double ratio{kPackMaxRatio};
  std::atomic<int> state{kQueued};
  size_t packed_bytes{0};
  uint32_t nexc{0};
  bool rescued{false};
  bool head{false};
};

enum class SubmitAction : int {
  kSubmit = 0,
  kClaimRaw,
  kWait,
  kDefer
};

template <typename LinkBusy>
inline SubmitAction DecideSubmit(int state, bool pack_wait, bool nothing_inflight,
                                 bool pool_behind, LinkBusy&& link_busy) {
  if (state == PackJob::kFailed) return SubmitAction::kWait;
  if (state != PackJob::kQueued && state != PackJob::kPacking) return SubmitAction::kSubmit;
  if (pack_wait) return SubmitAction::kWait;
  if (!nothing_inflight && !pool_behind && link_busy()) return SubmitAction::kDefer;
  return state == PackJob::kQueued ? SubmitAction::kClaimRaw : SubmitAction::kWait;
}

inline bool WaitMeansPoolBehind(bool link_idle, bool pack_wait, bool head_of_pass) {
  return link_idle && !pack_wait && !head_of_pass;
}

class PackPool {
 public:
  static constexpr size_t kRangeBlocks = 1024;
  static constexpr size_t kCopyBlocks = 1024;

  PackPool(int threads, const uint8_t alphabet[16], size_t distance,
           size_t range_blocks = kRangeBlocks)
      : nthreads_(std::max(threads, 1)),
        distance_(distance),
        range_blocks_(std::max<size_t>(range_blocks, 1)),
        encoder_(alphabet) {
    std::memcpy(alphabet_, alphabet, 16);
    for (int t = 0; t < nthreads_; ++t) workers_.emplace_back([this]() { Work(); });
  }
  ~PackPool() {
    {
      std::unique_lock<std::mutex> lk(mu_);
      queue_.clear();
      cv_done_.wait(lk, [&] { return nopen_ == 0; });
      stop_ = true;
    }
    cv_work_.notify_all();
    for (auto& w : workers_) w.join();
  }
  PackPool(const PackPool&) = delete;
  PackPool& operator=(const PackPool&) = delete;

  void Push(PackJob* job) {
    {
      std::lock_guard<std::mutex> lk(mu_);
      queue_.push_back(job);
    }
    cv_work_.notify_all();
  }
  void SetDistance(size_t distance) { distance_.store(distance, std::memory_order_relaxed); }
  void SetSubmitted(size_t n) { submitted_.store(n, std::memory_order_relaxed); }
  bool TryClaimRaw(PackJob* job) {
    std::lock_guard<std::mutex> lk(mu_);
    int expect = PackJob::kQueued;
    if (!job->state.compare_exchange_strong(expect, PackJob::kClaimedRaw)) return false;
    queue_.erase(std::remove(queue_.begin(), queue_.end(), job), queue_.end());
    return true;
  }
  void Wait(PackJob* job) {
    std::unique_lock<std::mutex> lk(mu_);
    cv_done_.wait(lk, [&] {
      const int st = job->state.load();
      return st != PackJob::kPacking && st != PackJob::kQueued;
    });
    if (job->state.load() == PackJob::kFailed) {
      std::exception_ptr e = error_;
      error_ = nullptr;
      lk.unlock();
      if (e) std::rethrow_exception(e);
      LOG(FATAL) << "text pack failed";
    }
  }
  void Quiesce() {
    std::unique_lock<std::mutex> lk(mu_);
    queue_.clear();
    cv_done_.wait(lk, [&] { return nopen_ == 0; });
    error_ = nullptr;
  }
  double pack_sec() const { return pack_sec_.load(std::memory_order_relaxed); }

 private:
  struct Open {
    PackJob* job{nullptr};
    size_t nranges{0};
    size_t order{0};
    long exc_limit{0};
    std::atomic<size_t> next{0}, done{0};
    std::atomic<long> exc_total{0};
    std::atomic<bool> fits{true};
    std::vector<std::vector<uint32_t>> exc;
    std::vector<uint32_t> all;
    bool copying{false};
    int result{PackJob::kRejected};
    std::exception_ptr err;
  };
  static constexpr int kOpenJobs = 2;

  Open* ClaimLocked(size_t* range) {
    Open* order[kOpenJobs] = {&open_[0], &open_[1]};
    if (order[1]->job != nullptr && (order[0]->job == nullptr || order[1]->order < order[0]->order)) {
      std::swap(order[0], order[1]);
    }
    for (Open* o : order) {
      if (o->job == nullptr || o->next.load(std::memory_order_relaxed) >= o->nranges) continue;
      const size_t r = o->next.fetch_add(1);
      if (r < o->nranges) {
        *range = r;
        return o;
      }
    }
    return nullptr;
  }
  bool OpenLocked() {
    Open* o = open_[0].job == nullptr ? &open_[0] : open_[1].job == nullptr ? &open_[1] : nullptr;
    while (o != nullptr && !queue_.empty()) {
      PackJob* job = queue_.front();
      queue_.pop_front();
      const size_t distance = distance_.load(std::memory_order_relaxed);
      if (distance != 0 && job->seq < submitted_.load(std::memory_order_relaxed) + distance) {
        continue;
      }
      int expect = PackJob::kQueued;
      if (!job->state.compare_exchange_strong(expect, PackJob::kPacking)) continue;
      o->job = job;
      o->nranges = std::max<size_t>(1, (PackBlocks(job->size) + range_blocks_ - 1) / range_blocks_);
      o->order = ++opened_;
      o->exc_limit = PackMaxExceptions(job->size, job->ratio);
      o->next.store(0);
      o->done.store(0);
      o->exc_total.store(0);
      o->fits.store(o->exc_limit >= 0);
      if (o->exc.size() < o->nranges) o->exc.resize(o->nranges);
      o->err = nullptr;
      o->copying = false;
      o->result = PackJob::kRejected;
      try {
        DMLC_FAULT_POINT("pack");
      } catch (...) {
        o->err = std::current_exception();
        o->fits.store(false);
      }
      if (nopen_++ == 0) open_since_ = GetTime();
      return true;
    }
    return false;
  }
  void RunRange(Open* o, size_t r) {
    const PackJob* job = o->job;
    const uint8_t* text = reinterpret_cast<const uint8_t*>(job->ptr);
    if (o->copying) {
      PackCopyExceptions(text, job->size, o->all, r * kCopyBlocks,
                         std::min(o->all.size(), (r + 1) * kCopyBlocks), job->out);
      return;
    }
    std::vector<uint32_t>& exc = o->exc[r];
    exc.clear();
    if (!o->fits.load(std::memory_order_relaxed)) return;
    const size_t b0 = r * range_blocks_;
    const size_t b1 = std::min(PackBlocks(job->size), b0 + range_blocks_);
    if (!PackRange(text, job->size, b0, b1, encoder_, job->out + sizeof(PackedHeader), &exc,
                   &o->exc_total, o->exc_limit)) {
      o->fits.store(false, std::memory_order_relaxed);
    }
  }
  bool FinishPack(Open* o) {
    PackJob* job = o->job;
    if (!o->fits.load()) return false;
    try {
      o->all.clear();
      for (size_t r = 0; r < o->nranges; ++r) {
        o->all.insert(o->all.end(), o->exc[r].begin(), o->exc[r].end());
      }
      if (static_cast<long>(o->all.size()) > o->exc_limit) return false;
      job->packed_bytes = PackFinishHeader(job->size, alphabet_, o->all, job->out);
      job->nexc = static_cast<uint32_t>(o->all.size());
      o->result = PackJob::kPacked;
      const size_t ncopy = (o->all.size() + kCopyBlocks - 1) / kCopyBlocks;
      if (ncopy <= 1) {
        PackCopyExceptions(reinterpret_cast<const uint8_t*>(job->ptr), job->size, o->all, 0,
                           o->all.size(), job->out);
        return false;
      }
      {
        std::lock_guard<std::mutex> lk(mu_);
        o->copying = true;
        o->nranges = ncopy;
        o->done.store(0);
        o->next.store(1);
      }
      cv_work_.notify_all();
      return true;
    } catch (...) {
      std::lock_guard<std::mutex> lk(mu_);
      if (!o->err) o->err = std::current_exception();
      return false;
    }
  }
  void Settle(Open* o) {
    {
      std::lock_guard<std::mutex> lk(mu_);
      int result = o->result;
      if (o->err) {
        error_ = o->err;
        result = PackJob::kFailed;
      }
      o->job->state.store(result);
      o->job = nullptr;
      if (--nopen_ == 0) {
        pack_sec_.store(pack_sec_.load(std::memory_order_relaxed) + (GetTime() - open_since_),
                        std::memory_order_relaxed);
      }
    }
    cv_done_.notify_all();
    cv_work_.notify_all();
  }
  void Work() {
    for (;;) {
      Open* o = nullptr;
      size_t r = 0;
      {
        std::unique_lock<std::mutex> lk(mu_);
        for (;;) {
          if (stop_) return;
          if ((o = ClaimLocked(&r)) != nullptr) break;
          if (OpenLocked()) {
            cv_work_.notify_all();
            continue;
          }
          cv_work_.wait(lk);
        }
      }
      while (o != nullptr) {
        const size_t nranges = o->nranges;
        try {
          RunRange(o, r);
        } catch (...) {
          o->fits.store(false);
          std::lock_guard<std::mutex> lk(mu_);
          if (!o->err) o->err = std::current_exception();
        }
        const size_t next = o->next.fetch_add(1);
        if (o->done.fetch_add(1) + 1 == nranges) {
          if (!o->copying && FinishPack(o)) {
            r = 0;
          } else {
            Settle(o);
            o = nullptr;
          }
        } else if (next < nranges) {
          r = next;
        } else {
          o = nullptr;
        }
      }
    }
  }

  const int nthreads_;
  std::atomic<size_t> distance_;
  const size_t range_blocks_;
  const PackEncoder encoder_;
  uint8_t alphabet_[16];
  std::mutex mu_;
  std::condition_variable cv_work_, cv_done_;
  std::deque<PackJob*> queue_;
  Open open_[kOpenJobs];
  int nopen_{0};
  size_t opened_{0};
  double open_since_{0};
  std::atomic<size_t> submitted_{0};
  std::atomic<double> pack_sec_{0};
  std::exception_ptr error_;
  bool stop_{false};
  std::vector<std::thread> workers_;
};

}
}
#endif
```

src/gpu/unpack_kernels.hip:

```cpp
#include <hip/hip_runtime.h>

#include "./kernels.h"
#include "./text_pack.h"

namespace dmlc {
namespace gpu {

namespace {
constexpr int kThreads = 256;

struct Alphabet4 {
  uint32_t w[4];
};

__device__ __forceinline__ uint32_t decode(const Alphabet4& a, uint32_t code) {
  const uint32_t sel = code >> 2;
  const uint32_t lo = sel & 1 ? a.w[1] : a.w[0];
  const uint32_t hi = sel & 1 ? a.w[3] : a.w[2];
  const uint32_t word = sel & 2 ? hi : lo;
  return (word >> ((code & 3) * 8)) & 0xffu;
}

__global__ __launch_bounds__(kThreads) void k_unpack_nibbles(const uint64_t* __restrict__ nib,
                                                             size_t n, Alphabet4 alpha,
                                                             char* __restrict__ dst,
                                                             unsigned lead) {
  const size_t g = static_cast<size_t>(blockIdx.x) * kThreads + threadIdx.x;
  const long long s = static_cast<long long>(g) * 16 - static_cast<long long>(lead);
  const long long end = static_cast<long long>(n);
  if (s >= end) return;
  if (s >= 0 && s + 16 <= end) {
    const size_t w = static_cast<size_t>(s) >> 4;
    const unsigned sh = (static_cast<unsigned>(s) & 15u) * 4u;
    uint64_t v = nib[w];
    if (sh != 0) v = (v >> sh) | (nib[w + 1] << (64u - sh));
    uint32_t o[4];
#pragma unroll
    for (int q = 0; q < 4; ++q) {
      const uint32_t c = static_cast<uint32_t>(v >> (16 * q)) & 0xffffu;
      o[q] = decode(alpha, c & 15u) | (decode(alpha, (c >> 4) & 15u) << 8) |
             (decode(alpha, (c >> 8) & 15u) << 16) | (decode(alpha, c >> 12) << 24);
    }
    *reinterpret_cast<uint4*>(dst + s) = make_uint4(o[0], o[1], o[2], o[3]);
  } else {
    const uint8_t* bytes = reinterpret_cast<const uint8_t*>(nib);
    const long long j0 = s < 0 ? 0 : s;
    const long long j1 = s + 16 < end ? s + 16 : end;
    for (long long j = j0; j < j1; ++j) {
      const uint32_t b = bytes[j >> 1];
      dst[j] = static_cast<char>(decode(alpha, (j & 1) ? b >> 4 : b & 15u));
    }
  }
}

__global__ __launch_bounds__(kThreads) void k_unpack_exceptions(const uint32_t* __restrict__ index,
                                                                const uint8_t* __restrict__ raw,
                                                                size_t n, char* __restrict__ dst) {
  const size_t e = blockIdx.x;
  const size_t off = static_cast<size_t>(index[e]) * kPackBlockBytes + threadIdx.x;
  if (off < n) dst[off] = static_cast<char>(raw[e * kPackBlockBytes + threadIdx.x]);
}
}

void LaunchUnpackText(const void* packed, size_t n, uint32_t nexc, const uint8_t alphabet[16],
                      char* dst, hipStream_t stream) {
  static_assert(kPackBlockBytes == kThreads, "one lane per byte of an exception block");
  if (n == 0) return;
  const uint8_t* base = static_cast<const uint8_t*>(packed);
  const uint8_t* nib = base + sizeof(PackedHeader);
  const uint8_t* idx = nib + NibbleAreaBytes(n);
  const uint8_t* raw = idx + ((static_cast<size_t>(nexc) * 4 + 15) & ~size_t(15));
  Alphabet4 alpha;
  for (int i = 0; i < 4; ++i) {
    alpha.w[i] = static_cast<uint32_t>(alphabet[4 * i]) | static_cast<uint32_t>(alphabet[4 * i + 1]) << 8 |
                 static_cast<uint32_t>(alphabet[4 * i + 2]) << 16 |
                 static_cast<uint32_t>(alphabet[4 * i + 3]) << 24;
  }
  const unsigned lead = static_cast<unsigned>(reinterpret_cast<uintptr_t>(dst) & 15u);
  const size_t groups = (n + lead + 15) / 16;
  hipLaunchKernelGGL(k_unpack_nibbles, dim3((groups + kThreads - 1) / kThreads), dim3(kThreads), 0,
                     stream, reinterpret_cast<const uint64_t*>(nib), n, alpha, dst, lead);
  if (nexc != 0) {
    hipLaunchKernelGGL(k_unpack_exceptions, dim3(nexc), dim3(kThreads), 0, stream,
                       reinterpret_cast<const uint32_t*>(idx), raw, n, dst);
  }
}

}
}
```

src/python/module.cc:

```cpp
#include <dmlc/data.h>
#include <dmlc/fault.h>
#include <dmlc/dist/communicator.h>
#include <dmlc/dist/tracker_client.h>
#include <dmlc/gpu/device_page_cache.h>
#include <dmlc/gpu/device_parser.h>
#include <dmlc/gpu/device_recordio.h>
#include <dmlc/gpu/hip_utils.h>
#include <dmlc/input_split_shuffle.h>
#include <dmlc/io.h>
#include <dmlc/logging.h>
#include <dmlc/recordio.h>
#include <dmlc/synthetic.h>
#include <dmlc/timer.h>
#include <pybind11/numpy.h>
#include <pybind11/pybind11.h>
#include <pybind11/stl.h>

#include <memory>
#include <string>
#include <tuple>
#include <vector>

#include "../gpu/kernels.h"
#include "../gpu/text_pack.h"
#include "../io/http.h"
#include "../io/line_split.h"
#include "../io/recordio_split.h"
#include "../io/shard_reader.h"
#include "./dlpack.h"

namespace py = pybind11;
using namespace dmlc;

namespace {

struct DLCtx {
  std::shared_ptr<void> owner;
  std::vector<int64_t> shape;
};

void DLDeleter(DLManagedTensor* t) {
  delete static_cast<DLCtx*>(t->manager_ctx);
  delete t;
}

void CapsuleDeleter(PyObject* cap) {
  if (PyCapsule_IsValid(cap, "dltensor")) {
    auto* t = static_cast<DLManagedTensor*>(PyCapsule_GetPointer(cap, "dltensor"));
    if (t != nullptr && t->deleter != nullptr) t->deleter(t);
  }
}

template <typename T>
DLDataType DType() {
  DLDataType d;
  d.lanes = 1;
  d.bits = sizeof(T) * 8;
  d.code = std::is_floating_point<T>::value ? kDLFloat
                                            : (std::is_signed<T>::value ? kDLInt : kDLUInt);
  return d;
}

template <typename T>
py::object ToCapsule(const T* ptr, int64_t n, int device, std::shared_ptr<void> owner) {
  auto* ctx = new DLCtx();
  ctx->owner = std::move(owner);
  ctx->shape = {n};
  auto* t = new DLManagedTensor();
  t->dl_tensor.data = const_cast<T*>(ptr);
  t->dl_tensor.device = DLDevice{kDLROCM, device};
  t->dl_tensor.ndim = 1;
  t->dl_tensor.dtype = DType<T>();
  t->dl_tensor.shape = ctx->shape.data();
  t->dl_tensor.strides = nullptr;
  t->dl_tensor.byte_offset = 0;
  t->manager_ctx = ctx;
  t->deleter = DLDeleter;
  return py::reinterpret_steal<py::object>(PyCapsule_New(t, "dltensor", CapsuleDeleter));
}

template <typename T>
py::array_t<T> ToNumpy(const T* ptr, size_t n) {
  py::array_t<T> a(n);
  if (n != 0) std::memcpy(a.mutable_data(), ptr, n * sizeof(T));
  return a;
}

template <typename I>
py::dict BlockToDict(const RowBlock<I>& b) {
  py::dict d;
  const size_t nnz = b.offset[b.size] - b.offset[0];
  std::vector<uint64_t> off(b.size + 1);
  for (size_t i = 0; i <= b.size; ++i) off[i] = b.offset[i] - b.offset[0];
  d["offset"] = ToNumpy(off.data(), off.size());
  d["label"] = ToNumpy(b.label, b.size);
  d["weight"] = b.weight ? py::object(ToNumpy(b.weight, b.size)) : py::none();
  d["qid"] = b.qid ? py::object(ToNumpy(b.qid, b.size)) : py::none();
  d["field"] = b.field ? py::object(ToNumpy(b.field + b.offset[0], nnz)) : py::none();
  d["index"] = ToNumpy(b.index + b.offset[0], nnz);
  d["value"] = b.value ? py::object(ToNumpy(b.value + b.offset[0], nnz)) : py::none();
  return d;
}

template <typename I>
class PyParser {
 public:
  PyParser(const std::string& uri, unsigned part, unsigned nparts, const std::string& type) {
    py::gil_scoped_release nogil;
    p_.reset(Parser<I>::Create(uri.c_str(), part, nparts, type.c_str()));
  }
  ~PyParser() {
    py::gil_scoped_release nogil;
    p_.reset();
  }
  bool Next() {
    py::gil_scoped_release nogil;
    return p_->Next();
  }
  py::dict Value() { return BlockToDict(p_->Value()); }
  void BeforeFirst() { p_->BeforeFirst(); }
  size_t BytesRead() const { return p_->BytesRead(); }
  py::tuple Drain() {
    size_t rows = 0, nnz = 0;
    double t0 = GetTime();
    {
      py::gil_scoped_release nogil;
      while (p_->Next()) {
        const auto& b = p_->Value();
        rows += b.size;
        nnz += b.offset[b.size] - b.offset[0];
      }
    }
    return py::make_tuple(rows, nnz, GetTime() - t0);
  }

 private:
  std::unique_ptr<Parser<I>> p_;
};

template <typename I>
class PyRowBlockIter {
 public:
  PyRowBlockIter(const std::string& uri, unsigned part, unsigned nparts, const std::string& type) {
    py::gil_scoped_release nogil;
    it_.reset(RowBlockIter<I>::Create(uri.c_str(), part, nparts, type.c_str()));
  }
  bool Next() {
    py::gil_scoped_release nogil;
    return it_->Next();
  }
  py::dict Value() { return BlockToDict(it_->Value()); }
  void BeforeFirst() { it_->BeforeFirst(); }
  size_t NumCol() const { return it_->NumCol(); }

 private:
  std::unique_ptr<RowBlockIter<I>> it_;
};

class PyPartitionReader {
 public:
  PyPartitionReader(const std::string& uri, unsigned part, unsigned nparts,
                    const std::string& type, int nthread, size_t chunk_bytes)
      : buf_(chunk_bytes, '\0') {
    CHECK(type == "text" || type == "recordio")
        << "PartitionReader: type must be text or recordio, got " << type;
    py::gil_scoped_release nogil;
    io::URI path(uri.c_str());
    io::FileSystem* fs = io::FileSystem::GetInstance(path);
    if (type == "text") {
      split_.reset(new io::LineSplitter(fs, uri.c_str(), part, nparts));
    } else {
      split_.reset(new io::RecordIOSplitter(fs, uri.c_str(), part, nparts));
    }
    reader_.reset(new io::ShardReader(split_.get(), nthread));
  }
  ~PyPartitionReader() {
    py::gil_scoped_release nogil;
    reader_.reset();
    split_.reset();
  }
  py::object Next() {
    size_t n;
    {
      py::gil_scoped_release nogil;
      n = reader_->Fill(&buf_[0], buf_.size());
      while (n == io::ShardReader::kNeedMore) {
        buf_.resize(reader_->NeedCapacity());
        n = reader_->Fill(&buf_[0], buf_.size());
      }
    }
    if (n == 0) return py::none();
    return py::bytes(buf_.data(), n);
  }
  size_t Tell() const { return reader_->Tell(); }
  void Seek(size_t pos) { reader_->Seek(pos); }
  size_t PartitionBytes() const { return reader_->PartitionBytes(); }

 private:
  std::string buf_;
  std::unique_ptr<io::InputSplitBase> split_;
  std::unique_ptr<io::ShardReader> reader_;
};

class PyInputSplit {
 public:
  PyInputSplit(const std::string& uri, unsigned part, unsigned nparts, const std::string& type,
               const std::string& index_uri, bool shuffle, int seed, size_t batch_size,
               unsigned num_shuffle_parts) {
    py::gil_scoped_release nogil;
    if (num_shuffle_parts > 0) {
      CHECK(index_uri.empty()) << "num_shuffle_parts does not combine with an index file";
      s_.reset(InputSplitShuffle::Create(uri.c_str(), part, nparts, type.c_str(),
                                         num_shuffle_parts, seed));
      return;
    }
    s_.reset(index_uri.empty()
                 ? InputSplit::Create(uri.c_str(), part, nparts, type.c_str())
                 : InputSplit::Create(uri.c_str(), index_uri.c_str(), part, nparts, type.c_str(),
                                      shuffle, seed, batch_size));
  }
  ~PyInputSplit() {
    py::gil_scoped_release nogil;
    s_.reset();
  }
  py::object NextRecord() {
    InputSplit::Blob b;
    bool ok;
    {
      py::gil_scoped_release nogil;
      ok = s_->NextRecord(&b);
    }
    if (!ok) return py::none();
    return py::bytes(static_cast<const char*>(b.dptr), b.size);
  }
  py::object NextChunk() {
    InputSplit::Blob b;
    bool ok;
    {
      py::gil_scoped_release nogil;
      ok = s_->NextChunk(&b);
    }
    if (!ok) return py::none();
    return py::bytes(static_cast<const char*>(b.dptr), b.size);
  }
  py::object NextBatch(size_t n) {
    InputSplit::Blob b;
    bool ok;
    {
      py::gil_scoped_release nogil;
      ok = s_->NextBatch(&b, n);
    }
    if (!ok) return py::none();
    return py::bytes(static_cast<const char*>(b.dptr), b.size);
  }
  void BeforeFirst() {
    py::gil_scoped_release nogil;
    s_->BeforeFirst();
  }
  void ResetPartition(unsigned part, unsigned nparts) { s_->ResetPartition(part, nparts); }
  size_t TotalSize() { return s_->GetTotalSize(); }
  void HintChunkSize(size_t n) { s_->HintChunkSize(n); }

 private:
  std::unique_ptr<InputSplit> s_;
};

class PyStream {
 public:
  PyStream(const std::string& uri, const std::string& mode) {
    py::gil_scoped_release nogil;
    s_.reset(Stream::Create(uri.c_str(), mode.c_str()));
  }
  ~PyStream() {
    py::gil_scoped_release nogil;
    s_.reset();
  }
  py::bytes Read(size_t n) {
    std::string buf(n, '\0');
    {
      py::gil_scoped_release nogil;
      size_t got = s_->Read(&buf[0], n);
      buf.resize(got);
    }
    return py::bytes(buf);
  }
  void Write(const std::string& data) {
    py::gil_scoped_release nogil;
    s_->Write(data.data(), data.size());
  }
  void Close() {
    py::gil_scoped_release nogil;
    s_.reset();
  }

 private:
  std::unique_ptr<Stream> s_;
};

class PyRecordIOWriter {
 public:
  explicit PyRecordIOWriter(const std::string& uri)
      : s_(Stream::Create(uri.c_str(), "w")), w_(new RecordIOWriter(s_.get())) {}
  void Write(const std::string& rec) { w_->WriteRecord(rec.data(), rec.size()); }
  size_t Tell() const { return w_->Tell(); }
  size_t ExceptCounter() const { return w_->except_counter(); }
  void Close() {
    w_.reset();
    s_.reset();
  }

 private:
  std::unique_ptr<Stream> s_;
  std::unique_ptr<RecordIOWriter> w_;
};

class PyRecordIOReader {
 public:
  explicit PyRecordIOReader(const std::string& uri)
      : s_(Stream::Create(uri.c_str(), "r")), r_(new RecordIOReader(s_.get())) {}
  py::object Next() {
    std::string rec;
    if (!r_->NextRecord(&rec)) return py::none();
    return py::bytes(rec);
  }

 private:
  std::unique_ptr<Stream> s_;
  std::unique_ptr<RecordIOReader> r_;
};

template <typename I>
class PyDeviceCSR {
 public:
  PyDeviceCSR() : csr_(std::make_shared<gpu::DeviceCSR<I>>()) {}
  std::shared_ptr<gpu::DeviceCSR<I>> csr_;
  size_t rows() const { return csr_->rows_; }
  size_t nnz() const { return csr_->nnz_; }
  uint64_t max_index() const { return csr_->max_index_; }
  uint64_t max_field() const { return csr_->max_field_; }
  size_t allocated_bytes() const { return csr_->AllocatedBytes(); }
  py::dict Capsules() {
    auto v = csr_->View();
    std::shared_ptr<void> owner = csr_;
    py::dict d;
    d["offset"] = ToCapsule(v.offset, static_cast<int64_t>(v.size + 1), v.device, owner);
    d["label"] = ToCapsule(v.label, static_cast<int64_t>(v.size), v.device, owner);
    d["index"] = ToCapsule(v.index, static_cast<int64_t>(v.nnz), v.device, owner);
    d["value"] = v.value ? ToCapsule(v.value, static_cast<int64_t>(v.nnz), v.device, owner)
                         : py::none();
    d["weight"] = v.weight ? ToCapsule(v.weight, static_cast<int64_t>(v.size), v.device, owner)
                           : py::none();
    d["qid"] = v.qid ? ToCapsule(v.qid, static_cast<int64_t>(v.size), v.device, owner)
                     : py::none();
    d["field"] = v.field ? ToCapsule(v.field, static_cast<int64_t>(v.nnz), v.device, owner)
                         : py::none();
    return d;
  }
  py::dict ToHost() {
    auto h = gpu::CopyToHost(csr_->View());
    return BlockToDict(h.GetBlock());
  }
  void Clear() { csr_->Clear(); }
};

template <typename I>
class PyDeviceParser {
 public:
  PyDeviceParser(const std::string& uri, unsigned part, unsigned nparts, py::dict cfg_dict) {
    gpu::DeviceParserConfig cfg;
    std::map<std::string, std::string> args;
    for (auto kv : cfg_dict) args[py::str(kv.first)] = py::str(kv.second);
    cfg.Update(args);
    py::gil_scoped_release nogil;
    p_.reset(gpu::DeviceParser<I>::Create(uri, part, nparts, cfg));
  }
  void ParseAll(PyDeviceCSR<I>& out) {
    py::gil_scoped_release nogil;
    p_->ParseAll(out.csr_.get());
  }
  py::dict ParseAllHashed(int dim, float scale, uint32_t seed, bool fp8, py::object out) {
    std::shared_ptr<gpu::DeviceHashedBatch> batch;
    if (!out.is_none()) batch = out.cast<std::shared_ptr<gpu::DeviceHashedBatch>>();
    if (batch == nullptr) batch = std::make_shared<gpu::DeviceHashedBatch>();
    {
      py::gil_scoped_release nogil;
      p_->ParseAllHashed(batch.get(), dim, scale, seed, fp8);
    }
    py::dict d;
    const int64_t n = static_cast<int64_t>(batch->rows) * dim;
    if (fp8) {
      d["x"] = ToCapsule(batch->x->get<uint8_t>(), n, batch->device, batch->x);
    } else {
      d["x"] = ToCapsule(batch->x->get<float>(), n, batch->device, batch->x);
    }
    d["label"] = ToCapsule(batch->label->get<float>(), static_cast<int64_t>(batch->rows),
                           batch->device, batch->label);
    d["rows"] = batch->rows;
    d["dim"] = dim;
    d["x_ptr"] = reinterpret_cast<uintptr_t>(batch->x->get());
    d["label_ptr"] = reinterpret_cast<uintptr_t>(batch->label->get());
    d["batch"] = py::cast(batch);
    return d;
  }
  bool Next() {
    py::gil_scoped_release nogil;
    return p_->Next();
  }
  py::dict ValueToHost() {
    auto h = gpu::CopyToHost(p_->Value());
    return BlockToDict(h.GetBlock());
  }
  py::tuple ValueShape() const {
    const auto& v = p_->Value();
    return py::make_tuple(v.size, v.nnz, v.max_index);
  }
  void BeforeFirst() {
    py::gil_scoped_release nogil;
    p_->BeforeFirst();
  }
  size_t Tell() const { return p_->Tell(); }
  void Seek(size_t cursor) {
    py::gil_scoped_release nogil;
    p_->Seek(cursor);
  }
  unsigned Epoch() const { return p_->Epoch(); }
  void SetEpoch(unsigned e) {
    py::gil_scoped_release nogil;
    p_->SetEpoch(e);
  }
  std::vector<unsigned> VisitOrder() const { return p_->VisitOrder(); }
  size_t PartitionBytes() const { return p_->PartitionBytes(); }
  py::dict Stats() const {
    const auto& s = p_->Stats();
    py::dict d;
    d["bytes"] = s.bytes;
    d["chunks"] = s.chunks;
    d["rows"] = s.rows;
    d["nnz"] = s.nnz;
    d["exact_chunks"] = s.exact_chunks;
    d["one_pass_chunks"] = s.one_pass_chunks;
    d["one_pass_reruns"] = s.one_pass_reruns;
    d["wait_reader_sec"] = s.wait_reader_sec;
    d["wait_gpu_sec"] = s.wait_gpu_sec;
    d["zero_copy"] = s.zero_copy;
    d["register_sec"] = s.register_sec;
    d["zc_pin_budget"] = s.zc_pin_budget;
    d["zc_pinned_peak"] = s.zc_pinned_peak;
    d["last_pass_sec"] = s.last_pass_sec;
    d["last_fill_sec"] = s.last_fill_sec;
    d["last_drain_sec"] = s.last_drain_sec;
    d["waits_spun"] = s.waits_spun;
    d["waits_slept"] = s.waits_slept;
    d["waits_timed_out"] = s.waits_timed_out;
    d["packed_chunks"] = s.packed_chunks;
    d["raw_chunks"] = s.raw_chunks;
    d["link_bytes"] = s.link_bytes;
    d["exception_blocks"] = s.exception_blocks;
    d["head_packed"] = s.head_packed;
    d["pack_sec"] = s.pack_sec;
    d["wait_pack_sec"] = s.wait_pack_sec;
    d["wait_pack_idle_sec"] = s.wait_pack_idle_sec;
    d["unpack_staging_bytes"] = s.unpack_staging_bytes;
    return d;
  }
  uintptr_t Stream() const { return reinterpret_cast<uintptr_t>(p_->stream()); }
  py::dict ValueCapsules() {
    const auto& v = p_->Value();
    std::shared_ptr<void> owner = p_;
    py::dict d;
    d["offset"] = ToCapsule(v.offset, static_cast<int64_t>(v.size + 1), v.device, owner);
    d["label"] = ToCapsule(v.label, static_cast<int64_t>(v.size), v.device, owner);
    d["index"] = ToCapsule(v.index, static_cast<int64_t>(v.nnz), v.device, owner);
    d["value"] = v.value ? ToCapsule(v.value, static_cast<int64_t>(v.nnz), v.device, owner)
                         : py::none();
    d["weight"] = v.weight ? ToCapsule(v.weight, static_cast<int64_t>(v.size), v.device, owner)
                           : py::none();
    d["qid"] = v.qid ? ToCapsule(v.qid, static_cast<int64_t>(v.size), v.device, owner) : py::none();
    d["field"] = v.field ? ToCapsule(v.field, static_cast<int64_t>(v.nnz), v.device, owner)
                         : py::none();
    return d;
  }

 private:
  std::shared_ptr<gpu::DeviceParser<I>> p_;
};

template <typename I>
class PyPageCache {
 public:
  explicit PyPageCache(std::unique_ptr<gpu::DevicePageCache<I>> c) : c_(std::move(c)) {}
  static py::object Open(const std::string& path, int device) {
    std::unique_ptr<gpu::DevicePageCache<I>> c;
    {
      py::gil_scoped_release nogil;
      c = gpu::DevicePageCache<I>::Open(path, device);
    }
    if (c == nullptr) return py::none();
    return py::cast(new PyPageCache<I>(std::move(c)), py::return_value_policy::take_ownership);
  }
  static size_t Write(PyDeviceCSR<I>& csr, const std::string& path, double page_mb) {
    py::gil_scoped_release nogil;
    return gpu::DevicePageCache<I>::Write(*csr.csr_, path, static_cast<size_t>(page_mb * (1 << 20)));
  }
  void Load(PyDeviceCSR<I>& out) {
    py::gil_scoped_release nogil;
    c_->Load(out.csr_.get());
  }
  py::list Pages() const {
    py::list l;
    for (const auto& p : c_->pages()) {
      py::dict d;
      d["rows"] = p.rows;
      d["nnz"] = p.nnz;
      d["begin"] = p.begin;
      d["end"] = p.end;
      d["max_index"] = p.max_index;
      l.append(d);
    }
    return l;
  }
  std::unique_ptr<gpu::DevicePageCache<I>> c_;
};

template <typename I>
void BindIndexType(py::module_& m, const std::string& suffix) {
  py::class_<PyParser<I>>(m, ("Parser" + suffix).c_str())
      .def(py::init<const std::string&, unsigned, unsigned, const std::string&>(),
           py::arg("uri"), py::arg("part") = 0, py::arg("nparts") = 1, py::arg("type") = "auto")
      .def("next", &PyParser<I>::Next)
      .def("value", &PyParser<I>::Value)
      .def("before_first", &PyParser<I>::BeforeFirst)
      .def("bytes_read", &PyParser<I>::BytesRead)
      .def("drain", &PyParser<I>::Drain);
  py::class_<PyRowBlockIter<I>>(m, ("RowBlockIter" + suffix).c_str())
      .def(py::init<const std::string&, unsigned, unsigned, const std::string&>(),
           py::arg("uri"), py::arg("part") = 0, py::arg("nparts") = 1, py::arg("type") = "auto")
      .def("next", &PyRowBlockIter<I>::Next)
      .def("value", &PyRowBlockIter<I>::Value)
      .def("before_first", &PyRowBlockIter<I>::BeforeFirst)
      .def("num_col", &PyRowBlockIter<I>::NumCol);
  py::class_<PyDeviceCSR<I>>(m, ("DeviceCSR" + suffix).c_str())
      .def(py::init<>())
      .def_property_readonly("rows", &PyDeviceCSR<I>::rows)
      .def_property_readonly("nnz", &PyDeviceCSR<I>::nnz)
      .def_property_readonly("max_index", &PyDeviceCSR<I>::max_index)
      .def_property_readonly("max_field", &PyDeviceCSR<I>::max_field)
      .def_property_readonly("allocated_bytes", &PyDeviceCSR<I>::allocated_bytes)
      .def("capsules", &PyDeviceCSR<I>::Capsules)
      .def("to_host", &PyDeviceCSR<I>::ToHost)
      .def("clear", &PyDeviceCSR<I>::Clear);
  py::class_<PyPageCache<I>>(m, ("PageCache" + suffix).c_str())
      .def_static("open", &PyPageCache<I>::Open, py::arg("path"), py::arg("device") = -1)
      .def_static("write", &PyPageCache<I>::Write, py::arg("csr"), py::arg("path"),
                  py::arg("page_mb") = 64.0)
      .def("load", &PyPageCache<I>::Load)
      .def("pages", &PyPageCache<I>::Pages)
      .def_property_readonly("rows", [](const PyPageCache<I>& c) { return c.c_->rows(); })
      .def_property_readonly("nnz", [](const PyPageCache<I>& c) { return c.c_->nnz(); })
      .def_property_readonly("bytes", [](const PyPageCache<I>& c) { return c.c_->bytes(); })
      .def_property_readonly("zero_copy", [](const PyPageCache<I>& c) { return c.c_->zero_copy(); });
  py::class_<PyDeviceParser<I>>(m, ("DeviceParser" + suffix).c_str())
      .def(py::init<const std::string&, unsigned, unsigned, py::dict>(), py::arg("uri"),
           py::arg("part") = 0, py::arg("nparts") = 1, py::arg("config") = py::dict())
      .def("parse_all", &PyDeviceParser<I>::ParseAll)
      .def("parse_all_hashed", &PyDeviceParser<I>::ParseAllHashed, py::arg("dim"),
           py::arg("scale") = 1.0f, py::arg("seed") = 0u, py::arg("fp8") = true,
           py::arg("out") = py::none())
      .def("next", &PyDeviceParser<I>::Next)
      .def("value_to_host", &PyDeviceParser<I>::ValueToHost)
      .def("value_shape", &PyDeviceParser<I>::ValueShape)
      .def("value_capsules", &PyDeviceParser<I>::ValueCapsules)
      .def("before_first", &PyDeviceParser<I>::BeforeFirst)
      .def("tell", &PyDeviceParser<I>::Tell)
      .def("seek", &PyDeviceParser<I>::Seek)
      .def("epoch", &PyDeviceParser<I>::Epoch)
      .def("set_epoch", &PyDeviceParser<I>::SetEpoch)
      .def("visit_order", &PyDeviceParser<I>::VisitOrder)
      .def("partition_bytes", &PyDeviceParser<I>::PartitionBytes)
      .def("stats", &PyDeviceParser<I>::Stats)
      .def("stream", &PyDeviceParser<I>::Stream);
}

class PyDeviceRecordIO {
 public:
  PyDeviceRecordIO(const std::string& uri, unsigned part, unsigned nparts, py::dict kwargs) {
    gpu::DeviceRecordIOConfig cfg;
    std::map<std::string, std::string> args;
    for (auto kv : kwargs) args[py::str(kv.first)] = py::str(kv.second);
    cfg.Update(args);
    {
      py::gil_scoped_release nogil;
      reader_.reset(gpu::DeviceRecordIOReader::Create(uri, part, nparts, cfg));
    }
    DMLC_HIP_CHECK(hipGetDevice(&device_));
  }
  bool Next() {
    py::gil_scoped_release nogil;
    return reader_->Next();
  }
  py::dict ValueCapsules() { return Batch(reader_->Value()); }
  py::tuple ValueToHost() { return ToHost(reader_->Value()); }
  py::tuple ResidentToHost() { return ToHost(Resident()); }
  void BeforeFirst() { reader_->BeforeFirst(); }
  size_t PartitionBytes() const { return reader_->PartitionBytes(); }
  py::dict Stats() const {
    const auto& s = reader_->Stats();
    py::dict d;
    d["bytes"] = s.bytes;
    d["chunks"] = s.chunks;
    d["records"] = s.records;
    d["zero_copy"] = s.zero_copy;
    d["wait_reader_sec"] = s.wait_reader_sec;
    d["wait_gpu_sec"] = s.wait_gpu_sec;
    d["replayed_chunks"] = s.replayed_chunks;
    d["one_pass_chunks"] = s.one_pass_chunks;
    d["one_pass_reruns"] = s.one_pass_reruns;
    d["chain_counts"] = s.chain_counts;
    return d;
  }
  uintptr_t Stream() const { return reinterpret_cast<uintptr_t>(reader_->stream()); }

 private:
  const gpu::DeviceRecordBatch& Resident() { return resident_view_; }
  py::dict Batch(const gpu::DeviceRecordBatch& b) {
    py::dict d;
    d["size"] = b.size;
    d["bytes"] = b.bytes;
    d["offset"] = ToCapsule(b.offset, static_cast<int64_t>(b.size + 1), device_, reader_);
    d["data"] = ToCapsule(b.data, static_cast<int64_t>(b.bytes), device_, reader_);
    return d;
  }
  py::tuple ToHost(const gpu::DeviceRecordBatch& b) {
    std::vector<uint64_t> off(b.size + 1, 0);
    std::string data(b.bytes, '\0');
    DMLC_HIP_CHECK(hipStreamSynchronize(reader_->stream()));
    if (b.size > 0) {
      DMLC_HIP_CHECK(hipMemcpy(off.data(), b.offset, off.size() * 8, hipMemcpyDeviceToHost));
    }
    if (b.bytes > 0) DMLC_HIP_CHECK(hipMemcpy(&data[0], b.data, b.bytes, hipMemcpyDeviceToHost));
    return py::make_tuple(ToNumpy(off.data(), off.size()), py::bytes(data));
  }
  std::shared_ptr<gpu::DeviceRecordIOReader> reader_;
  gpu::DeviceRecordBatch resident_view_;
  int device_{0};

  friend void BindRecordIO(py::module_& m);
};

void BindRecordIO(py::module_& m) {
  py::class_<PyDeviceRecordIO>(m, "DeviceRecordIO")
      .def(py::init<const std::string&, unsigned, unsigned, py::dict>(), py::arg("uri"),
           py::arg("part") = 0, py::arg("nparts") = 1, py::arg("config") = py::dict())
      .def("next", &PyDeviceRecordIO::Next)
      .def("read_all",
           [](PyDeviceRecordIO& self) {
             {
               py::gil_scoped_release nogil;
               self.resident_view_ = self.reader_->ReadAll();
             }
             return self.Batch(self.resident_view_);
           })
      .def("value", &PyDeviceRecordIO::ValueCapsules)
      .def("value_to_host", &PyDeviceRecordIO::ValueToHost)
      .def("resident_to_host", &PyDeviceRecordIO::ResidentToHost)
      .def("before_first", &PyDeviceRecordIO::BeforeFirst)
      .def("partition_bytes", &PyDeviceRecordIO::PartitionBytes)
      .def("stats", &PyDeviceRecordIO::Stats)
      .def("stream", &PyDeviceRecordIO::Stream);
}

py::object PackTextPy(const std::string& text, const std::string& format, const std::string& delimiter,
                      double ratio, int isa) {
  CHECK(format == "libsvm" || format == "libfm" || format == "csv") << "unknown format " << format;
  CHECK_EQ(delimiter.size(), 1U) << "delimiter must be one character";
  CHECK(gpu::PackIsaSupported(static_cast<gpu::PackIsa>(isa))) << "instruction set not supported";
  uint8_t alphabet[16];
  gpu::PackAlphabet(format == "csv", delimiter[0], alphabet);
  std::vector<uint8_t> packed;
  if (!gpu::PackText(reinterpret_cast<const uint8_t*>(text.data()), text.size(), alphabet, ratio,
                     &packed, static_cast<gpu::PackIsa>(isa))) {
    return py::none();
  }
  return py::bytes(reinterpret_cast<const char*>(packed.data()), packed.size());
}

size_t CheckedPackedSize(const std::string& packed) {
  CHECK_GE(packed.size(), sizeof(gpu::PackedHeader)) << "not a packed chunk";
  const gpu::PackedView v = gpu::ViewPacked(reinterpret_cast<const uint8_t*>(packed.data()));
  CHECK_EQ(v.bytes, packed.size()) << "packed chunk size mismatch";
  for (uint32_t i = 0; i < v.header.nexc; ++i) {
    uint32_t b;
    std::memcpy(&b, reinterpret_cast<const uint8_t*>(v.exc_index) + 4 * i, 4);
    CHECK_LT(static_cast<size_t>(b), gpu::PackBlocks(v.header.n)) << "exception block out of range";
  }
  return v.header.n;
}

py::bytes UnpackTextReferencePy(const std::string& packed) {
  std::string out(CheckedPackedSize(packed), '\0');
  gpu::UnpackReference(reinterpret_cast<const uint8_t*>(packed.data()),
                       reinterpret_cast<uint8_t*>(&out[0]));
  return py::bytes(out);
}

py::bytes UnpackTextDevicePy(const std::string& packed, size_t dst_offset, size_t pad, int fill) {
  const size_t n = CheckedPackedSize(packed);
  const gpu::PackedView v = gpu::ViewPacked(reinterpret_cast<const uint8_t*>(packed.data()));
  gpu::DeviceBuffer src(packed.size()), dst(dst_offset + n + pad);
  gpu::Stream stream;
  DMLC_HIP_CHECK(hipMemcpyAsync(src.get(), packed.data(), packed.size(), hipMemcpyHostToDevice,
                                stream.get()));
  DMLC_HIP_CHECK(hipMemsetAsync(dst.get(), fill, dst_offset + n + pad, stream.get()));
  gpu::LaunchUnpackText(src.get(), n, v.header.nexc, v.header.alphabet,
                        dst.get<char>() + dst_offset, stream.get());
  DMLC_HIP_CHECK(hipGetLastError());
  std::string out(dst_offset + n + pad, '\0');
  DMLC_HIP_CHECK(hipMemcpyAsync(&out[0], dst.get(), out.size(), hipMemcpyDeviceToHost, stream.get()));
  stream.Synchronize();
  return py::bytes(out);
}

template <typename T>
T* Ptr(uintptr_t p) {
  return reinterpret_cast<T*>(p);
}

using CsrArg = std::tuple<uintptr_t, uintptr_t, uintptr_t, uintptr_t, size_t, bool, bool>;

gpu::CsrView View(const CsrArg& a) {
  return gpu::CsrView{Ptr<const uint64_t>(std::get<0>(a)), Ptr<const void>(std::get<1>(a)),
                      Ptr<const float>(std::get<2>(a)),    Ptr<const void>(std::get<3>(a)),
                      std::get<4>(a),                      std::get<5>(a),
                      std::get<6>(a)};
}

}

PYBIND11_MODULE(_dmlc, m) {
  m.doc() = "dmlc-core for MI355X: native runtime bindings";
  py::register_exception<dmlc::Error>(m, "DMLCError");
  m.def("pack_text", &PackTextPy, py::arg("text"), py::arg("format") = "libsvm",
        py::arg("delimiter") = ",", py::arg("ratio") = gpu::kPackMaxRatio, py::arg("isa") = 0);
  m.def("pack_isa_supported",
        [](int isa) { return gpu::PackIsaSupported(static_cast<gpu::PackIsa>(isa)); });
  m.def("unpack_text_reference", &UnpackTextReferencePy, py::arg("packed"));
  m.def("unpack_text_device", &UnpackTextDevicePy, py::arg("packed"), py::arg("dst_offset") = 0,
        py::arg("pad") = 64, py::arg("fill") = 0xA5);
  py::class_<gpu::DeviceHashedBatch, std::shared_ptr<gpu::DeviceHashedBatch>>(m, "HashedBatch")
      .def_readonly("rows", &gpu::DeviceHashedBatch::rows)
      .def_readonly("row_capacity", &gpu::DeviceHashedBatch::row_cap)
      .def_readonly("dim", &gpu::DeviceHashedBatch::dim);
  BindIndexType<uint32_t>(m, "");
  BindIndexType<uint64_t>(m, "64");
  BindRecordIO(m);
  py::class_<PyPartitionReader>(m, "PartitionReader")
      .def(py::init<const std::string&, unsigned, unsigned, const std::string&, int, size_t>(),
           py::arg("uri"), py::arg("part") = 0, py::arg("nparts") = 1, py::arg("type") = "text",
           py::arg("nthread") = 8, py::arg("chunk_bytes") = 64UL << 20)
      .def("next", &PyPartitionReader::Next)
      .def("tell", &PyPartitionReader::Tell)
      .def("seek", &PyPartitionReader::Seek)
      .def("partition_bytes", &PyPartitionReader::PartitionBytes);
  py::class_<PyInputSplit>(m, "InputSplit")
      .def(py::init<const std::string&, unsigned, unsigned, const std::string&,
                    const std::string&, bool, int, size_t, unsigned>(),
           py::arg("uri"), py::arg("part") = 0, py::arg("nparts") = 1, py::arg("type") = "text",
           py::arg("index_uri") = "", py::arg("shuffle") = false, py::arg("seed") = 0,
           py::arg("batch_size") = 256, py::arg("num_shuffle_parts") = 0)
      .def("next_record", &PyInputSplit::NextRecord)
      .def("next_chunk", &PyInputSplit::NextChunk)
      .def("next_batch", &PyInputSplit::NextBatch)
      .def("before_first", &PyInputSplit::BeforeFirst)
      .def("reset_partition", &PyInputSplit::ResetPartition)
      .def("total_size", &PyInputSplit::TotalSize)
      .def("hint_chunk_size", &PyInputSplit::HintChunkSize);
  py::class_<PyStream>(m, "Stream")
      .def(py::init<const std::string&, const std::string&>(), py::arg("uri"),
           py::arg("mode") = "r")
      .def("read", &PyStream::Read)
      .def("write", &PyStream::Write)
      .def("close", &PyStream::Close);
  py::class_<PyRecordIOWriter>(m, "RecordIOWriter")
      .def(py::init<const std::string&>())
      .def("write", &PyRecordIOWriter::Write)
      .def("tell", &PyRecordIOWriter::Tell)
      .def("except_counter", &PyRecordIOWriter::ExceptCounter)
      .def("close", &PyRecordIOWriter::Close);
  py::class_<PyRecordIOReader>(m, "RecordIOReader")
      .def(py::init<const std::string&>())
      .def("next", &PyRecordIOReader::Next);
  m.def(
      "write_synthetic",
      [](const std::string& path, uint64_t row_begin, uint64_t row_end, const std::string& format,
         uint64_t seed, uint32_t min_nnz, uint32_t max_nnz, uint64_t num_features,
         uint32_t num_fields, uint32_t csv_columns, uint32_t record_bytes, uint32_t weight_every,
         bool qid, int nthread, const std::string& shape) {
        synthetic::Spec s;
        s.format = format;
        s.seed = seed;
        s.min_nnz = min_nnz;
        s.max_nnz = max_nnz;
        s.num_features = num_features;
        s.num_fields = num_fields;
        s.csv_columns = csv_columns;
        s.record_bytes = record_bytes;
        s.weight_every = weight_every;
        s.qid = qid;
        s.shape = shape;
        py::gil_scoped_release nogil;
        return synthetic::WriteRows(s, path, row_begin, row_end, nthread);
      },
      py::arg("path"), py::arg("row_begin"), py::arg("row_end"), py::arg("format") = "libsvm",
      py::arg("seed") = 0, py::arg("min_nnz") = 20, py::arg("max_nnz") = 60,
      py::arg("num_features") = 1000000, py::arg("num_fields") = 32, py::arg("csv_columns") = 29,
      py::arg("record_bytes") = 512, py::arg("weight_every") = 0, py::arg("qid") = false,
      py::arg("nthread") = 8, py::arg("shape") = "uniform");
  auto stream_of = [](uintptr_t s) { return reinterpret_cast<hipStream_t>(s); };
  m.def(
      "fm_forward",
      [stream_of](uintptr_t x, int64_t rows, int dim, uintptr_t wt, uintptr_t q, uintptr_t bias,
                  float sx, uintptr_t y, uintptr_t xv, int num_cus, uintptr_t stream) {
        CHECK(dim > 0 && dim % 128 == 0 && dim <= 2048)
            << "HashedFM kernels need dim a multiple of 128, <= 2048 (got " << dim << ")";
        gpu::LaunchFmForward(reinterpret_cast<const uint8_t*>(x), rows, dim,
                             reinterpret_cast<const void*>(wt), reinterpret_cast<const float*>(q),
                             reinterpret_cast<const float*>(bias), sx, reinterpret_cast<float*>(y),
                             reinterpret_cast<float*>(xv), num_cus, stream_of(stream));
      },
      py::arg("x"), py::arg("rows"), py::arg("dim"), py::arg("wt"), py::arg("q"), py::arg("bias"),
      py::arg("sx"), py::arg("y"), py::arg("xv"), py::arg("num_cus"), py::arg("stream"));
  m.def(
      "fm_backward",
      [stream_of](uintptr_t x, int64_t rows, int dim, uintptr_t g, uintptr_t xv, int nblocks,
                  uintptr_t part, uintptr_t stream) {
        CHECK(dim > 0 && dim % 128 == 0) << "HashedFM kernels need dim a multiple of 128";
        gpu::LaunchFmBackward(reinterpret_cast<const uint8_t*>(x), rows, dim,
                              reinterpret_cast<const float*>(g), reinterpret_cast<const float*>(xv),
                              nblocks, reinterpret_cast<float*>(part), stream_of(stream));
      },
      py::arg("x"), py::arg("rows"), py::arg("dim"), py::arg("g"), py::arg("xv"),
      py::arg("nblocks"), py::arg("part"), py::arg("stream"));
  m.def(
      "fm_prep",
      [stream_of](uintptr_t w, uintptr_t v, int dim, uintptr_t wt, uintptr_t q, uintptr_t stream) {
        gpu::LaunchFmPrep(reinterpret_cast<const float*>(w), reinterpret_cast<const float*>(v),
                          dim, reinterpret_cast<void*>(wt), reinterpret_cast<float*>(q),
                          stream_of(stream));
      },
      py::arg("w"), py::arg("v"), py::arg("dim"), py::arg("wt"), py::arg("q"), py::arg("stream"));
  m.def(
      "fm_reduce_grads",
      [stream_of](uintptr_t part, int nblocks, int dim, uintptr_t v, float sx, uintptr_t z,
                  uintptr_t gw, uintptr_t gv, uintptr_t stream) {
        gpu::LaunchFmReduceGrads(reinterpret_cast<const float*>(part), nblocks, dim,
                                 reinterpret_cast<const float*>(v), sx, reinterpret_cast<float*>(z),
                                 reinterpret_cast<float*>(gw), reinterpret_cast<float*>(gv),
                                 stream_of(stream));
      },
      py::arg("part"), py::arg("nblocks"), py::arg("dim"), py::arg("v"), py::arg("sx"),
      py::arg("z"), py::arg("gw"), py::arg("gv"), py::arg("stream"));
  m.def(
      "fm_fused",
      [stream_of](uintptr_t x, int64_t rows, int dim, uintptr_t wt, uintptr_t q, uintptr_t bias,
                  float sx, uintptr_t label, uintptr_t weight, int loss, float inv_n, int nblocks,
                  uintptr_t y, uintptr_t part, uintptr_t lpart, uintptr_t stream) {
        CHECK(dim == 128 || dim == 256 || dim == 512 || dim == 1024)
            << "fused HashedFM step: dim must be 128, 256, 512 or 1024 (got " << dim << ")";
        CHECK(loss == gpu::kFmLogistic || loss == gpu::kFmSquared) << "unknown loss " << loss;
        gpu::LaunchFmFused(reinterpret_cast<const uint8_t*>(x), rows, dim,
                           reinterpret_cast<const void*>(wt), reinterpret_cast<const float*>(q),
                           reinterpret_cast<const float*>(bias), sx,
                           reinterpret_cast<const float*>(label),
                           reinterpret_cast<const float*>(weight), loss, inv_n, nblocks,
                           reinterpret_cast<float*>(y), reinterpret_cast<float*>(part),
                           reinterpret_cast<float*>(lpart), stream_of(stream));
      },
      py::arg("x"), py::arg("rows"), py::arg("dim"), py::arg("wt"), py::arg("q"), py::arg("bias"),
      py::arg("sx"), py::arg("label"), py::arg("weight"), py::arg("loss"), py::arg("inv_n"),
      py::arg("nblocks"), py::arg("y"), py::arg("part"), py::arg("lpart"), py::arg("stream"));
  m.attr("fm_rank") = gpu::kFmRank;
  m.def("shuffle_parts_order", &InputSplitShuffle::VisitOrder, py::arg("part"), py::arg("nparts"),
        py::arg("num_shuffle_parts"), py::arg("seed"), py::arg("epoch"),
        "sub-shard visiting order of InputSplitShuffle in a given epoch");
  m.def(
      "spmv",
      [stream_of](const CsrArg& csr, uintptr_t w, float bias, uintptr_t y, uintptr_t stream) {
        gpu::LaunchCSRSpMV(View(csr), Ptr<const float>(w), bias, Ptr<float>(y), stream_of(stream));
      },
      py::arg("csr"), py::arg("w"), py::arg("bias"), py::arg("y"), py::arg("stream"));
  m.def(
      "spmv_t",
      [stream_of](const CsrArg& csr, uintptr_t d, uintptr_t g, uintptr_t stream) {
        gpu::LaunchCSRSpMVT(View(csr), Ptr<const float>(d), Ptr<float>(g), stream_of(stream));
      },
      py::arg("csr"), py::arg("d"), py::arg("g"), py::arg("stream"));
  m.def(
      "spmm",
      [stream_of](const CsrArg& csr, uintptr_t w, uintptr_t bias, int k, uintptr_t y,
                  uintptr_t stream) {
        gpu::LaunchCSRSpMM(View(csr), Ptr<const float>(w), Ptr<const float>(bias), k,
                           Ptr<float>(y), stream_of(stream));
      },
      py::arg("csr"), py::arg("w"), py::arg("bias"), py::arg("k"), py::arg("y"),
      py::arg("stream"));
  m.def(
      "spmm_t",
      [stream_of](const CsrArg& csr, uintptr_t d, int k, uintptr_t g, uintptr_t stream) {
        gpu::LaunchCSRSpMMT(View(csr), Ptr<const float>(d), k, Ptr<float>(g), stream_of(stream));
      },
      py::arg("csr"), py::arg("d"), py::arg("k"), py::arg("g"), py::arg("stream"));
  m.def("spmm_max_cols", []() { return gpu::kSpMMMaxCols; },
        "widest dense operand (columns) ops.spmm / ops.spmm_t take");
  m.def(
      "ffm_forward",
      [stream_of](const CsrArg& csr, uintptr_t v, uint64_t features, int num_fields, int k,
                  uintptr_t y, uintptr_t error, uintptr_t stream) {
        gpu::LaunchFFMForward(View(csr), Ptr<const float>(v), features, num_fields, k,
                              Ptr<float>(y), Ptr<int>(error), stream_of(stream));
      },
      py::arg("csr"), py::arg("v"), py::arg("features"), py::arg("num_fields"), py::arg("k"),
      py::arg("y"), py::arg("error"), py::arg("stream"));
  m.def(
      "ffm_backward",
      [stream_of](const CsrArg& csr, uintptr_t g, uintptr_t v, uint64_t features, int num_fields,
                  int k, uintptr_t dv, uintptr_t stream) {
        gpu::LaunchFFMBackward(View(csr), Ptr<const float>(g), Ptr<const float>(v), features,
                               num_fields, k, Ptr<float>(dv), stream_of(stream));
      },
      py::arg("csr"), py::arg("g"), py::arg("v"), py::arg("features"), py::arg("num_fields"),
      py::arg("k"), py::arg("dv"), py::arg("stream"));
  m.def("ffm_max_rank", []() { return gpu::kFFMMaxRank; },
        "largest factor rank (a multiple of 4) ops.ffm / ops.ffm_t take");
  m.def("ffm_staged_row_entries", []() { return gpu::kFFMStagedRowEntries; },
        "entries of a row FF1 / FF2 stage in LDS; longer rows re-read global memory");
  m.def(
      "qid_flags",
      [stream_of](uintptr_t qid, size_t rows, uintptr_t flag, uintptr_t partials, uintptr_t total,
                  uintptr_t stream) {
        auto* f = Ptr<uint64_t>(flag);
        gpu::LaunchQidFlags(Ptr<const uint64_t>(qid), rows, f, stream_of(stream));
        gpu::LaunchScanU64(f, rows, Ptr<uint64_t>(partials), Ptr<uint64_t>(total),
                           stream_of(stream));
      },
      py::arg("qid"), py::arg("rows"), py::arg("flag"), py::arg("partials"), py::arg("total"),
      py::arg("stream"));
  m.def(
      "qid_group_ptr",
      [stream_of](uintptr_t qid, size_t rows, uintptr_t scanned, uintptr_t total,
                  uint64_t capacity, uintptr_t group_ptr, uintptr_t stream) {
        gpu::LaunchQidGroupPtr(Ptr<const uint64_t>(qid), rows, Ptr<const uint64_t>(scanned),
                               Ptr<const uint64_t>(total), capacity, Ptr<uint64_t>(group_ptr),
                               stream_of(stream));
      },
      py::arg("qid"), py::arg("rows"), py::arg("scanned"), py::arg("total"), py::arg("capacity"),
      py::arg("group_ptr"), py::arg("stream"));
  m.def("qid_scan_words", [](size_t rows) { return gpu::ScanPartials(rows) + 1; }, py::arg("rows"),
        "u64 words of scan scratch qid_flags needs next to its `rows` flags");
  m.def(
      "rank_loss",
      [stream_of](uintptr_t score, uintptr_t label, uintptr_t group_ptr, size_t groups,
                  uint64_t rows, bool ndcg_weights, float sigma, uintptr_t row_scratch,
                  uintptr_t grad, uintptr_t loss_g, uintptr_t pairs_g, uintptr_t error,
                  uintptr_t stream) {
        gpu::LaunchRankLoss(Ptr<const float>(score), Ptr<const float>(label),
                            Ptr<const uint64_t>(group_ptr), groups, rows, ndcg_weights, sigma,
                            Ptr<float>(row_scratch), Ptr<float>(grad), Ptr<float>(loss_g),
                            Ptr<int64_t>(pairs_g), Ptr<int>(error), stream_of(stream));
      },
      py::arg("score"), py::arg("label"), py::arg("group_ptr"), py::arg("groups"), py::arg("rows"),
      py::arg("ndcg_weights"), py::arg("sigma"), py::arg("row_scratch"), py::arg("grad"),
      py::arg("loss_g"), py::arg("pairs_g"), py::arg("error"), py::arg("stream"));
  m.def(
      "rank_ndcg",
      [stream_of](uintptr_t score, uintptr_t label, uintptr_t group_ptr, size_t groups,
                  uint64_t rows, uint32_t k, uintptr_t ndcg, uintptr_t error, uintptr_t stream) {
        gpu::LaunchRankNdcg(Ptr<const float>(score), Ptr<const float>(label),
                            Ptr<const uint64_t>(group_ptr), groups, rows, k, Ptr<float>(ndcg),
                            Ptr<int>(error), stream_of(stream));
      },
      py::arg("score"), py::arg("label"), py::arg("group_ptr"), py::arg("groups"), py::arg("rows"),
      py::arg("k"), py::arg("ndcg"), py::arg("error"), py::arg("stream"));
  m.def("rank_wave_group_rows", []() { return gpu::kRankWaveGroupRows; },
        "rows of a group RK1 (one wave per group) takes; longer groups run on RK2");
  m.def("rank_tile_rows", []() { return gpu::kRankTileRows; },
        "rows of the tiles RK2 passes a long group through LDS in");
  m.def("rank_max_label", []() { return gpu::kRankMaxLabel; },
        "largest label ops.rank_loss / ops.ndcg take");
  m.attr("rank_err_group") = gpu::kRankErrGroup;
  m.attr("rank_err_label") = gpu::kRankErrLabel;
  m.def(
      "csr_transpose",
      [stream_of](const CsrArg& csr, uint64_t base, uint64_t nnz, uint64_t num_features,
                  uintptr_t col_ptr, uintptr_t row_out, uintptr_t val_out, uintptr_t scratch,
                  uintptr_t error, uintptr_t stream) {
        gpu::LaunchCSRTranspose(View(csr), base, nnz, num_features, Ptr<uint64_t>(col_ptr),
                                Ptr<uint32_t>(row_out), Ptr<float>(val_out), Ptr<void>(scratch),
                                Ptr<uint32_t>(error), stream_of(stream));
      },
      py::arg("csr"), py::arg("base"), py::arg("nnz"), py::arg("num_features"),
      py::arg("col_ptr"), py::arg("row_out"), py::arg("val_out"), py::arg("scratch"),
      py::arg("error"), py::arg("stream"));
  m.def("csr_transpose_scratch_bytes", &gpu::CSRTransposeScratchBytes, py::arg("nnz"),
        py::arg("num_features"));
  m.def("csr_transpose_max_features", &gpu::CSRTransposeMaxFeatures);
  m.def(
      "csr_gather_count",
      [stream_of](uintptr_t offset, uint64_t nrows_src, uint64_t src_entries, uintptr_t rows,
                  bool rows64, size_t n_sel, uintptr_t label, uintptr_t weight, uintptr_t qid,
                  uintptr_t out_offset, uintptr_t out_label, uintptr_t out_weight,
                  uintptr_t out_qid, uintptr_t scratch, uintptr_t total, uintptr_t error,
                  uintptr_t stream) {
        auto* oo = Ptr<uint64_t>(out_offset);
        gpu::LaunchCSRGatherCount(Ptr<const uint64_t>(offset), nrows_src, src_entries,
                                  Ptr<const void>(rows), rows64, n_sel, Ptr<const float>(label),
                                  Ptr<const float>(weight), Ptr<const uint64_t>(qid), oo,
                                  Ptr<float>(out_label), Ptr<float>(out_weight),
                                  Ptr<uint64_t>(out_qid), Ptr<uint32_t>(error), stream_of(stream));
        gpu::LaunchScanU64(oo, n_sel, Ptr<uint64_t>(scratch), Ptr<uint64_t>(total),
                           stream_of(stream));
      },
      py::arg("offset"), py::arg("nrows_src"), py::arg("src_entries"), py::arg("rows"),
      py::arg("rows64"), py::arg("n_sel"), py::arg("label"), py::arg("weight"), py::arg("qid"),
      py::arg("out_offset"), py::arg("out_label"), py::arg("out_weight"), py::arg("out_qid"),
      py::arg("scratch"), py::arg("total"), py::arg("error"), py::arg("stream"));
  m.def(
      "csr_gather_fill",
      [stream_of](const CsrArg& csr, uint64_t src_entries, uintptr_t rows, bool rows64,
                  size_t n_sel, uintptr_t out_offset, uintptr_t total, uintptr_t out_index,
                  uintptr_t out_value, uintptr_t out_field, uint64_t out_capacity,
                  uintptr_t error, uintptr_t stream) {
        gpu::LaunchCSRGatherFill(View(csr), src_entries, Ptr<const void>(rows), rows64, n_sel,
                                 Ptr<uint64_t>(out_offset), Ptr<const uint64_t>(total),
                                 Ptr<void>(out_index), Ptr<float>(out_value), Ptr<void>(out_field),
                                 out_capacity, Ptr<uint32_t>(error), stream_of(stream));
      },
      py::arg("csr"), py::arg("src_entries"), py::arg("rows"), py::arg("rows64"),
      py::arg("n_sel"), py::arg("out_offset"), py::arg("total"), py::arg("out_index"),
      py::arg("out_value"), py::arg("out_field"), py::arg("out_capacity"), py::arg("error"),
      py::arg("stream"));
  m.def("csr_gather_scratch_words", &gpu::CSRGatherScratchWords, py::arg("n_sel"));
  m.def("csr_gather_run_entries", &gpu::CSRGatherRunEntries);
  m.def(
      "compact_mark",
      [stream_of](const CsrArg& csr, uint64_t base, uint64_t nnz, uint64_t num_features,
                  uintptr_t scratch, uintptr_t total, uintptr_t error, uintptr_t stream) {
// ... 232 lines not shown
```

Before: 177.3 million.

## Add dense per-chunk text code for packed host-to-device transfer with GPU unpack

```diff
diff --git a/dmlc_core_amd/data/__init__.py b/dmlc_core_amd/data/__init__.py
--- a/dmlc_core_amd/data/__init__.py
+++ b/dmlc_core_amd/data/__init__.py
@@ -10,7 +10,9 @@
 
 write_synthetic = _dmlc.write_synthetic
 pack_text = _dmlc.pack_text
+pack_text_pool = _dmlc.pack_text_pool
 pack_isa_supported = _dmlc.pack_isa_supported
+pack_isa_supported_dense = _dmlc.pack_isa_supported_dense
 unpack_text_reference = _dmlc.unpack_text_reference
 unpack_text_device = _dmlc.unpack_text_device
 
diff --git a/include/dmlc/gpu/device_parser.h b/include/dmlc/gpu/device_parser.h
--- a/include/dmlc/gpu/device_parser.h
+++ b/include/dmlc/gpu/device_parser.h
@@ -27,6 +27,7 @@
   bool prelaunch{true};
   int zero_copy{-1};
   int packed_h2d{-1};
+  int pack_code{-1};
   bool pack_wait{false};
   bool pack_head{true};
   int copy_streams{2};
@@ -67,6 +68,7 @@
   double last_pass_sec{0}, last_fill_sec{0}, last_drain_sec{0};
   size_t waits_spun{0}, waits_slept{0}, waits_timed_out{0};
   size_t packed_chunks{0}, raw_chunks{0}, link_bytes{0}, exception_blocks{0};
+  size_t dense_chunks{0}, escape_bytes{0}, raw_blocks{0};
   size_t head_packed{0};
   double pack_sec{0}, wait_pack_sec{0}, wait_pack_idle_sec{0};
   size_t unpack_staging_bytes{0};
diff --git a/src/gpu/chunk_feed.cc b/src/gpu/chunk_feed.cc
--- a/src/gpu/chunk_feed.cc
+++ b/src/gpu/chunk_feed.cc
@@ -11,6 +11,7 @@
 #include "../io/line_split.h"
 #include "./kernels.h"
 #include "./text_pack.h"
+#include "./text_pack_dense.h"
 
 namespace dmlc {
 namespace gpu {
@@ -277,7 +278,16 @@
                                     hipMemcpyHostToDevice, copy));
       copied_[d]->Record(copy);
       DMLC_HIP_CHECK(hipStreamWaitEvent(unpack_->get(), copied_[d]->get(), 0));
-      LaunchUnpackText(dstage_[d]->get(), size, job->nexc, alphabet_, dst, unpack_->get());
+      if (job->dense) {
+        LaunchUnpackDense(dstage_[d]->get(), size,
+                          static_cast<uint32_t>(DenseRanges(size, pool_->range_blocks())),
+                          static_cast<uint32_t>(pool_->range_blocks()), dst, unpack_->get());
+        stats_->dense_chunks += 1;
+        stats_->escape_bytes += job->escape_bytes;
+        stats_->raw_blocks += job->raw_blocks;
+      } else {
+        LaunchUnpackText(dstage_[d]->get(), size, job->nexc, alphabet_, dst, unpack_->get());
+      }
       unpacked_[d]->Record(unpack_->get());
       pack_slot = job->slot;
       stats_->packed_chunks += 1;
@@ -304,7 +314,12 @@
 
 void ChunkFeed::StartPacking(bool csv_alphabet) {
   PackAlphabet(csv_alphabet, cfg_.delimiter, alphabet_);
-  pool_.reset(new PackPool(cfg_.read_threads, alphabet_, 0));
+  const bool dense = cfg_.pack_code == 1 ||
+                     (cfg_.pack_code < 0 && cfg_.chunk_bytes >= (size_t(1) << 20) &&
+                      cfg_.read_threads >= kDenseMinThreads);
+  pool_.reset(new PackPool(cfg_.read_threads, alphabet_, 0, PackPool::kRangeBlocks,
+                           dense ? PackCode::kDense : PackCode::kNibble, csv_alphabet,
+                           cfg_.delimiter));
   pack_slots_ =
       std::vector<PinnedBuffer>(kPackLookahead + static_cast<size_t>(cfg_.device_slots) + 1);
   for (size_t i = 0; i < pack_slots_.size(); ++i) free_pack_slots_.push_back(static_cast<int>(i));
diff --git a/src/gpu/chunk_feed.h b/src/gpu/chunk_feed.h
--- a/src/gpu/chunk_feed.h
+++ b/src/gpu/chunk_feed.h
@@ -93,6 +93,7 @@
   static constexpr size_t kPackLookahead = 4;
   static constexpr size_t kPackDistance = 2;
   static constexpr size_t kPackCaughtUp = 8;
+  static constexpr int kDenseMinThreads = 16;
   static constexpr size_t kHeadJobs = 2;
 
   void SyncCopyStreams() const;
diff --git a/src/gpu/device_parser.cc b/src/gpu/device_parser.cc
--- a/src/gpu/device_parser.cc
+++ b/src/gpu/device_parser.cc
@@ -76,6 +76,10 @@
       pack_head = v != "0" && v != "false";
     } else if (k == "copy_streams") {
       copy_streams = std::atoi(v.c_str());
+    } else if (k == "pack_code") {
+      CHECK(v == "auto" || v == "-1" || v == "nibble" || v == "dense")
+          << "pack_code must be auto, nibble or dense";
+      pack_code = v == "nibble" ? 0 : (v == "dense" ? 1 : -1);
     } else if (k == "packed_h2d") {
       packed_h2d = (v == "auto" || v == "-1") ? -1 : ((v == "0" || v == "false") ? 0 : 1);
     }
diff --git a/src/gpu/kernels.h b/src/gpu/kernels.h
--- a/src/gpu/kernels.h
+++ b/src/gpu/kernels.h
@@ -270,6 +270,8 @@
 void LaunchFill(float* p, size_t n, float v, hipStream_t stream);
 void LaunchUnpackText(const void* packed, size_t n, uint32_t nexc, const uint8_t alphabet[16],
                       char* dst, hipStream_t stream);
+void LaunchUnpackDense(const void* packed, size_t n, uint32_t nranges, uint32_t range_blocks,
+                       char* dst, hipStream_t stream);
 
 }
 }
diff --git a/src/gpu/pack_pool.h b/src/gpu/pack_pool.h
--- a/src/gpu/pack_pool.h
+++ b/src/gpu/pack_pool.h
@@ -17,6 +17,7 @@
 #include <vector>
 
 #include "./text_pack.h"
+#include "./text_pack_dense.h"
 
 namespace dmlc {
 namespace gpu {
@@ -34,6 +35,9 @@
   std::atomic<int> state{kQueued};
   size_t packed_bytes{0};
   uint32_t nexc{0};
+  DenseTable table;
+  bool dense{false};
+  size_t escape_bytes{0}, raw_blocks{0};
   bool rescued{false};
   bool head{false};
 };
@@ -59,16 +63,22 @@
   return link_idle && !pack_wait && !head_of_pass;
 }
 
+enum class PackCode : int { kNibble = 0, kDense = 1 };
+
 class PackPool {
  public:
   static constexpr size_t kRangeBlocks = 1024;
   static constexpr size_t kCopyBlocks = 1024;
 
   PackPool(int threads, const uint8_t alphabet[16], size_t distance,
-           size_t range_blocks = kRangeBlocks)
+           size_t range_blocks = kRangeBlocks, PackCode code = PackCode::kNibble,
+           bool csv = false, char delimiter = ',')
       : nthreads_(std::max(threads, 1)),
         distance_(distance),
         range_blocks_(std::max<size_t>(range_blocks, 1)),
+        code_(code),
+        csv_(csv),
+        delimiter_(delimiter),
         encoder_(alphabet) {
     std::memcpy(alphabet_, alphabet, 16);
     for (int t = 0; t < nthreads_; ++t) workers_.emplace_back([this]() { Work(); });
@@ -87,6 +97,10 @@
   PackPool& operator=(const PackPool&) = delete;
 
   void Push(PackJob* job) {
+    if (code_ == PackCode::kDense) {
+      job->table = DenseSelectTable(reinterpret_cast<const uint8_t*>(job->ptr), job->size, csv_,
+                                    delimiter_);
+    }
     {
       std::lock_guard<std::mutex> lk(mu_);
       queue_.push_back(job);
@@ -123,6 +137,8 @@
     error_ = nullptr;
   }
   double pack_sec() const { return pack_sec_.load(std::memory_order_relaxed); }
+  PackCode code() const { return code_; }
+  size_t range_blocks() const { return range_blocks_; }
 
  private:
   struct Open {
@@ -138,6 +154,10 @@
     bool copying{false};
     int result{PackJob::kRejected};
     std::exception_ptr err;
+    std::atomic<size_t> cursor{0}, escape_bytes{0}, raw_blocks{0};
+    size_t limit{0};
+    std::vector<DenseDirEntry> dir;
+    std::unique_ptr<DenseEncoder> dense;
   };
   static constexpr int kOpenJobs = 2;
 
@@ -180,6 +200,18 @@
       o->copying = false;
       o->result = PackJob::kRejected;
       try {
+        if (code_ == PackCode::kDense) {
+          const size_t nranges = DenseRanges(job->size, range_blocks_);
+          o->dense.reset(new DenseEncoder(job->table));
+          o->dir.assign(nranges, DenseDirEntry{0, 0});
+          o->cursor.store(DenseHeaderBytes(nranges, DenseEntryBytes(job->table)));
+          o->escape_bytes.store(0);
+          o->raw_blocks.store(0);
+          o->limit = job->ratio < 0
+                         ? DenseMaxBytes(job->size, range_blocks_)
+                         : static_cast<size_t>(job->ratio * static_cast<double>(job->size));
+          o->fits.store(true);
+        }
         DMLC_FAULT_POINT("pack");
       } catch (...) {
         o->err = std::current_exception();
@@ -190,7 +222,27 @@
     }
     return false;
   }
-  void RunRange(Open* o, size_t r) {
+  void RunRangeDense(Open* o, size_t r, uint8_t* scratch) {
+    const PackJob* job = o->job;
+    if (!o->fits.load(std::memory_order_relaxed)) return;
+    const size_t b0 = r * range_blocks_;
+    const size_t b1 = std::min(PackBlocks(job->size), b0 + range_blocks_);
+    if (b0 >= b1) return;
+    size_t escapes = 0, raw = 0;
+    const size_t len = PackRangeDense(reinterpret_cast<const uint8_t*>(job->ptr), job->size, b0,
+                                      b1, *o->dense, scratch, &escapes, &raw);
+    const size_t at = o->cursor.fetch_add(len);
+    if (at + len > o->limit) {
+      o->fits.store(false, std::memory_order_relaxed);
+      return;
+    }
+    DenseCopyOut(scratch, len, job->out + at);
+    o->dir[r] = DenseDirEntry{static_cast<uint32_t>(at), static_cast<uint32_t>(len)};
+    o->escape_bytes.fetch_add(escapes, std::memory_order_relaxed);
+    o->raw_blocks.fetch_add(raw, std::memory_order_relaxed);
+  }
+  void RunRange(Open* o, size_t r, uint8_t* scratch) {
+    if (code_ == PackCode::kDense) return RunRangeDense(o, r, scratch);
     const PackJob* job = o->job;
     const uint8_t* text = reinterpret_cast<const uint8_t*>(job->ptr);
     if (o->copying) {
@@ -212,6 +264,16 @@
     PackJob* job = o->job;
     if (!o->fits.load()) return false;
     try {
+      if (code_ == PackCode::kDense) {
+        DenseWriteHeader(job->size, range_blocks_, job->table, o->dir, job->out);
+        job->packed_bytes = o->cursor.load();
+        job->nexc = 0;
+        job->dense = true;
+        job->escape_bytes = o->escape_bytes.load();
+        job->raw_blocks = o->raw_blocks.load();
+        o->result = PackJob::kPacked;
+        return false;
+      }
       o->all.clear();
       for (size_t r = 0; r < o->nranges; ++r) {
         o->all.insert(o->all.end(), o->exc[r].begin(), o->exc[r].end());
@@ -260,6 +322,10 @@
     cv_work_.notify_all();
   }
   void Work() {
+    std::vector<uint8_t> buffer(
+        code_ == PackCode::kDense ? DenseRangeCapacity(range_blocks_) + 64 : 0);
+    uint8_t* scratch =
+        buffer.data() + ((64 - (reinterpret_cast<uintptr_t>(buffer.data()) & 63)) & 63);
     for (;;) {
       Open* o = nullptr;
       size_t r = 0;
@@ -278,7 +344,7 @@
       while (o != nullptr) {
         const size_t nranges = o->nranges;
         try {
-          RunRange(o, r);
+          RunRange(o, r, scratch);
         } catch (...) {
           o->fits.store(false);
           std::lock_guard<std::mutex> lk(mu_);
@@ -304,6 +370,9 @@
   const int nthreads_;
   std::atomic<size_t> distance_;
   const size_t range_blocks_;
+  const PackCode code_;
+  const bool csv_;
+  const char delimiter_;
   const PackEncoder encoder_;
   uint8_t alphabet_[16];
   std::mutex mu_;
diff --git a/src/gpu/text_pack_dense.cc b/src/gpu/text_pack_dense.cc
--- /dev/null
+++ b/src/gpu/text_pack_dense.cc
@@ -0,0 +1,667 @@
+#include "./text_pack_dense.h"
+
+#include <dmlc/logging.h>
+
+#include <algorithm>
+#include <cstring>
+
+#if defined(__x86_64__)
+#include <immintrin.h>
+#define DMLC_PACK_X86 1
+#else
+#define DMLC_PACK_X86 0
+#endif
+
+namespace dmlc {
+namespace gpu {
+
+namespace {
+
+constexpr uint8_t kBad = 0x80;
+
+inline bool Blank(uint8_t c) { return c == ' ' || c == '\t' || c == '\r' || c == '\n'; }
+
+size_t BlockScalarDense(const uint8_t* src, size_t len, const DenseEncoder& e, uint8_t* out,
+                        uint8_t* meta, size_t* escapes, size_t* raw_blocks) {
+  uint8_t codes[kPackBlockBytes + 1];
+  uint8_t lits[kPackBlockBytes];
+  size_t cnt = 0, nlit = 0;
+  for (size_t i = 0; i < len;) {
+    int hit = -1;
+    for (int m = 0; m < e.nmulti && hit < 0; ++m) {
+      if (i + e.mlen[m] <= len && std::memcmp(src + i, e.mbytes[m], e.mlen[m]) == 0) hit = m;
+    }
+    if (hit >= 0) {
+      codes[cnt++] = e.mcode[hit];
+      i += e.mlen[hit];
+      continue;
+    }
+    const uint8_t c = e.enc[src[i]];
+    if (c & kBad) {
+      codes[cnt++] = e.table.escape;
+      lits[nlit++] = src[i];
+    } else {
+      codes[cnt++] = c;
+    }
+    ++i;
+  }
+  codes[cnt] = 0;
+  const size_t nb = (cnt + 1) / 2;
+  if (nb + nlit > kDenseMaxPayload) {
+    std::memcpy(out, src, len);
+    meta[0] = meta[1] = kDenseRawMeta;
+    if (raw_blocks != nullptr) ++*raw_blocks;
+    return len;
+  }
+  for (size_t k = 0; k < nb; ++k) {
+    out[k] = static_cast<uint8_t>(codes[2 * k] | (codes[2 * k + 1] << 4));
+  }
+  std::memcpy(out + nb, lits, nlit);
+  meta[0] = static_cast<uint8_t>(nb);
+  meta[1] = static_cast<uint8_t>(nlit);
+  if (escapes != nullptr) *escapes += nlit;
+  return nb + nlit;
+}
+
+#if DMLC_PACK_X86
+#define DMLC_DENSE_TARGET \
+  __attribute__((target("avx512f,avx512bw,avx512vl,avx512vbmi,avx512vbmi2,avx2,popcnt")))
+
+struct DenseBlock {
+  alignas(64) uint8_t codes[kPackBlockBytes + 64];
+  alignas(64) uint8_t lits[kPackBlockBytes + 64];
+  const uint8_t* src;
+  uint8_t* out;
+  size_t cnt, nlit;
+  bool raw;
+};
+
+DMLC_DENSE_TARGET inline void BlockPayloadAvx512(const DenseBlock* blk) {
+  uint8_t* out = blk->out;
+  if (blk->raw) {
+    for (int v = 0; v < 4; ++v) {
+      _mm512_storeu_si512(out + 64 * v, _mm512_loadu_si512(blk->src + 64 * v));
+    }
+    return;
+  }
+  const __m512i k1001 = _mm512_set1_epi16(0x1001);
+  const size_t cnt = blk->cnt, nlit = blk->nlit;
+  for (size_t k = 0; k < cnt; k += 64) {
+    const __m512i a = _mm512_load_si512(blk->codes + k);
+    _mm256_storeu_si256(reinterpret_cast<__m256i*>(out + k / 2),
+                        _mm512_cvtepi16_epi8(_mm512_maddubs_epi16(a, k1001)));
+  }
+  if (nlit != 0) {
+    uint8_t* lit = out + (cnt + 1) / 2;
+    if (nlit <= 64) {
+      _mm512_storeu_si512(lit, _mm512_load_si512(blk->lits));
+    } else {
+      std::memcpy(lit, blk->lits, nlit);
+    }
+  }
+}
+
+template <int NM>
+DMLC_DENSE_TARGET void RangeAvx512Dense(const uint8_t* text, size_t n, size_t block_begin,
+                                        size_t block_end, const DenseEncoder& e, uint8_t* meta,
+                                        uint8_t* payload, size_t* pos, size_t* escapes,
+                                        size_t* raw_blocks) {
+  constexpr int kM = NM > 0 ? NM : 1;
+  const __m512i tlo = _mm512_loadu_si512(e.enc);
+  const __m512i thi = _mm512_loadu_si512(e.enc + 64);
+  const __m512i vesc = _mm512_set1_epi8(static_cast<char>(e.table.escape));
+  __m512i mcode[kM], mb[kM][4];
+  int mlen[kM];
+  int maxlen = 1;
+  for (int m = 0; m < NM; ++m) {
+    mcode[m] = _mm512_set1_epi8(static_cast<char>(e.mcode[m]));
+    mlen[m] = e.mlen[m];
+    maxlen = std::max(maxlen, mlen[m]);
+    for (int k = 0; k < 4; ++k) mb[m][k] = _mm512_set1_epi8(static_cast<char>(e.mbytes[m][k]));
+  }
+  DenseBlock blocks[2];
+  DenseBlock* blk = &blocks[0];
+  DenseBlock* prev = nullptr;
+  size_t at = *pos, nesc = 0, nraw = 0;
+  for (size_t b = block_begin; b < block_end; ++b) {
+    const size_t off = b * kPackBlockBytes;
+    uint8_t* mt = meta + 2 * (b - block_begin);
+    if (off + kPackBlockBytes + 3 > n) {
+      if (prev != nullptr) BlockPayloadAvx512(prev);
+      prev = nullptr;
+      at += BlockScalarDense(text + off, std::min(kPackBlockBytes, n - off), e, payload + at, mt,
+                             &nesc, &nraw);
+      continue;
+    }
+    const uint8_t* src = text + off;
+    uint8_t* codes = blk->codes;
+    uint8_t* lits = blk->lits;
+    size_t cnt = 0, nlit = 0;
+    uint64_t carry = 0;
+#pragma GCC unroll 4
+    for (int v = 0; v < 4; ++v) {
+      const uint8_t* p = src + 64 * v;
+      const __m512i x0 = _mm512_loadu_si512(p);
+      __m512i code = _mm512_permutex2var_epi8(tlo, x0, thi);
+      uint64_t esc = _mm512_movepi8_mask(_mm512_or_si512(code, x0));
+      uint64_t cover = carry, start = 0;
+      carry = 0;
+      if (NM != 0) {
+        const __m512i x1 = _mm512_loadu_si512(p + 1);
+        const __m512i x2 = maxlen > 2 ? _mm512_loadu_si512(p + 2) : x1;
+        const __m512i x3 = maxlen > 3 ? _mm512_loadu_si512(p + 3) : x1;
+#pragma GCC unroll 4
+        for (int m = 0; m < NM; ++m) {
+          const int len = mlen[m];
+          __mmask64 k = _mm512_cmpeq_epi8_mask(x0, mb[m][0]);
+          k = _mm512_mask_cmpeq_epi8_mask(k, x1, mb[m][1]);
+          if (len > 2) k = _mm512_mask_cmpeq_epi8_mask(k, x2, mb[m][2]);
+          if (len > 3) k = _mm512_mask_cmpeq_epi8_mask(k, x3, mb[m][3]);
+          uint64_t mk = k;
+          if (v == 3) mk &= ~uint64_t(0) >> (len - 1);
+          code = _mm512_mask_mov_epi8(code, mk, mcode[m]);
+          start |= mk;
+          cover |= mk << 1;
+          carry |= mk >> 63;
+          if (len > 2) {
+            cover |= mk << 2;
+            carry |= mk >> 62;
+          }
+          if (len > 3) {
+            cover |= mk << 3;
+            carry |= mk >> 61;
+          }
+        }
+      }
+      const uint64_t keep = ~cover;
+      esc &= keep & ~start;
+      code = _mm512_mask_mov_epi8(code, esc, vesc);
+      _mm512_storeu_si512(codes + cnt, _mm512_maskz_compress_epi8(keep, code));
+      cnt += static_cast<size_t>(_mm_popcnt_u64(keep));
+      if (esc != 0) {
+        _mm512_storeu_si512(lits + nlit, _mm512_maskz_compress_epi8(esc, x0));
+        nlit += static_cast<size_t>(_mm_popcnt_u64(esc));
+      }
+    }
+    codes[cnt] = 0;
+    const size_t nb = (cnt + 1) / 2;
+    const bool raw = nb + nlit > kDenseMaxPayload;
+    blk->src = src;
+    blk->out = payload + at;
+    blk->cnt = cnt;
+    blk->nlit = nlit;
+    blk->raw = raw;
+    if (raw) {
+      mt[0] = mt[1] = kDenseRawMeta;
+      ++nraw;
+      at += kPackBlockBytes;
+    } else {
+      mt[0] = static_cast<uint8_t>(nb);
+      mt[1] = static_cast<uint8_t>(nlit);
+      nesc += nlit;
+      at += nb + nlit;
+    }
+    if (prev != nullptr) BlockPayloadAvx512(prev);
+    prev = blk;
+    blk = blk == &blocks[0] ? &blocks[1] : &blocks[0];
+  }
+  if (prev != nullptr) BlockPayloadAvx512(prev);
+  *pos = at;
+  if (escapes != nullptr) *escapes += nesc;
+  if (raw_blocks != nullptr) *raw_blocks += nraw;
+}
+
+DMLC_DENSE_TARGET void CopyOutAvx512(const uint8_t* src, size_t bytes, uint8_t* dst) {
+  size_t k = 0;
+  for (; k < bytes && ((reinterpret_cast<uintptr_t>(dst + k) & 63) != 0); k += 16) {
+    _mm_stream_si128(reinterpret_cast<__m128i*>(dst + k),
+                     _mm_loadu_si128(reinterpret_cast<const __m128i*>(src + k)));
+  }
+  for (; k + 64 <= bytes; k += 64) {
+    _mm512_stream_si512(reinterpret_cast<__m512i*>(dst + k), _mm512_loadu_si512(src + k));
+  }
+  for (; k < bytes; k += 16) {
+    _mm_stream_si128(reinterpret_cast<__m128i*>(dst + k),
+                     _mm_loadu_si128(reinterpret_cast<const __m128i*>(src + k)));
+  }
+}
+#endif
+
+struct Candidate {
+  uint64_t score;
+  int len;
+  uint8_t bytes[4];
+};
+
+bool CandidateBefore(const Candidate& a, const Candidate& b) {
+  if (a.score != b.score) return a.score > b.score;
+  if (a.len != b.len) return a.len < b.len;
+  return std::memcmp(a.bytes, b.bytes, 4) < 0;
+}
+
+}
+
+bool DenseCompatible(const uint8_t* a, int alen, const uint8_t* b, int blen) {
+  const bool same = alen == blen && std::memcmp(a, b, alen) == 0;
+  for (int pass = 0; pass < 2; ++pass) {
+    const uint8_t* x = pass == 0 ? a : b;
+    const uint8_t* y = pass == 0 ? b : a;
+    const int xl = pass == 0 ? alen : blen, yl = pass == 0 ? blen : alen;
+    for (int s = (same || pass == 1) ? 1 : 0; s < xl; ++s) {
+      const int shared = std::min(xl - s, yl);
+      if (std::memcmp(x + s, y, shared) == 0) return false;
+    }
+  }
+  return true;
+}
+
+bool DenseTableValid(const DenseTable& t) {
+  if (t.escape > 15 || t.len[t.escape] != 0) return false;
+  bool single[256] = {false};
+  for (int c = 0; c < 16; ++c) {
+    if (t.len[c] > 4) return false;
+    if (t.len[c] == 1) {
+      if (single[t.bytes[c][0]]) return false;
+      single[t.bytes[c][0]] = true;
+    }
+    if (t.len[c] < 2) continue;
+    for (int d = 0; d <= c; ++d) {
+      if (t.len[d] >= 2 && !DenseCompatible(t.bytes[c], t.len[c], t.bytes[d], t.len[d])) {
+        return false;
+      }
+    }
+  }
+  return true;
+}
+
+bool DenseMakeTable(const std::vector<std::vector<uint8_t>>& entries, DenseTable* out) {
+  if (entries.size() > 15) return false;
+  std::memset(out, 0, sizeof(*out));
+  for (size_t c = 0; c < entries.size(); ++c) {
+    if (entries[c].empty() || entries[c].size() > 4) return false;
+    out->len[c] = static_cast<uint8_t>(entries[c].size());
+    std::memcpy(out->bytes[c], entries[c].data(), entries[c].size());
+  }
+  out->escape = static_cast<uint8_t>(entries.size());
+  return DenseTableValid(*out);
+}
+
+DenseTable DenseDefaultTable(bool csv, char delimiter) {
+  uint8_t alphabet[16];
+  PackAlphabet(csv, delimiter, alphabet);
+  DenseTable t;
+  std::memset(&t, 0, sizeof(t));
+  for (int c = 0; c < 15; ++c) {
+    t.bytes[c][0] = alphabet[c];
+    t.len[c] = 1;
+  }
+  t.escape = 15;
+  return t;
+}
+
+DenseTable DenseSelectTable(const uint8_t* text, size_t n, bool csv, char delimiter) {
+  uint8_t alphabet[16];
+  PackAlphabet(csv, delimiter, alphabet);
+  bool format[256] = {false};
+  for (int c = 0; c < 16; ++c) format[alphabet[c]] = true;
+
+  struct Window {
+    size_t begin, end;
+  };
+  std::vector<Window> windows;
+  for (size_t at = 0; at < n; at += kDenseSampleStride) {
+    windows.push_back(Window{at, std::min(n, at + kDenseSampleBytes)});
+  }
+  uint32_t count[256] = {0};
+  size_t sampled = 0;
+  for (const Window& w : windows) {
+    for (size_t i = w.begin; i < w.end; ++i) ++count[text[i]];
+    sampled += w.end - w.begin;
+  }
+  int order[256];
+  for (int b = 0; b < 256; ++b) order[b] = b;
+  std::stable_sort(order, order + 256, [&](int a, int b) { return count[a] > count[b]; });
+  uint8_t cls[256] = {0}, cls_byte[16] = {0};
+  int ncls = 0;
+  for (int k = 0; k < 256 && ncls < 15; ++k) {
+    const int b = order[k];
+    if (count[b] == 0) break;
+    if (Blank(static_cast<uint8_t>(b))) continue;
+    cls[b] = static_cast<uint8_t>(++ncls);
+    cls_byte[ncls] = static_cast<uint8_t>(b);
+  }
+  uint32_t c2[256] = {0};
+  std::vector<uint32_t> c3(4096, 0);
+  for (const Window& w : windows) {
+    unsigned h = 0, run = 0;
+    for (size_t i = w.begin; i < w.end; ++i) {
+      const unsigned c = cls[text[i]];
+      h = ((h << 4) | c) & 0xfffu;
+      run = c != 0 ? run + 1 : 0;
+      c2[h & 0xffu] += run >= 2;
+      c3[h] += run >= 3;
+    }
+  }
+  std::vector<Candidate> cand;
+  auto add = [&](unsigned h, int len, uint32_t cnt) {
+    const uint64_t score = static_cast<uint64_t>(len - 1) * cnt;
+    if (cnt == 0 || score * 256 < sampled) return;
+    Candidate c;
+    c.score = score;
+    c.len = len;
+    std::memset(c.bytes, 0, 4);
+    for (int k = 0; k < len; ++k) c.bytes[k] = cls_byte[(h >> (4 * (len - 1 - k))) & 15u];
+    cand.push_back(c);
+  };
+  for (unsigned h = 0; h < 256; ++h) add(h, 2, c2[h]);
+  for (unsigned h = 0; h < 4096; ++h) add(h, 3, c3[h]);
+  std::sort(cand.begin(), cand.end(), CandidateBefore);
+  std::vector<int64_t> left(count, count + 256);
+  auto loss = [](const std::vector<int64_t>& a, size_t slots) {
+    std::vector<int64_t> v(a);
+    std::sort(v.begin(), v.end(), [](int64_t x, int64_t y) { return x > y; });
+    int64_t sum = 0;
+    for (size_t k = slots; k < v.size(); ++k) sum += 2 * v[k];
+    return sum;
+  };
+  std::vector<Candidate> multi;
+  int64_t cur_loss = loss(left, 15);
+  const size_t tries = std::min<size_t>(cand.size(), 64);
+  for (size_t i = 0; i < tries && static_cast<int>(multi.size()) < kDenseMaxMulti; ++i) {
+    const Candidate& c = cand[i];
+    bool ok = DenseCompatible(c.bytes, c.len, c.bytes, c.len);
+    for (size_t k = 0; k < multi.size() && ok; ++k) {
+      ok = DenseCompatible(c.bytes, c.len, multi[k].bytes, multi[k].len);
+    }
+    if (!ok) continue;
+    std::vector<int64_t> after(left);
+    const int64_t cnt = static_cast<int64_t>(c.score) / (c.len - 1);
+    for (int k = 0; k < c.len; ++k) after[c.bytes[k]] = std::max<int64_t>(0, after[c.bytes[k]] - cnt);
+    const int64_t new_loss = loss(after, 15 - multi.size() - 1);
+    if (static_cast<int64_t>(c.score) <= new_loss - cur_loss + static_cast<int64_t>(sampled / 256)) {
+      continue;
+    }
+    multi.push_back(c);
+    left.swap(after);
+    cur_loss = new_loss;
+  }
+  std::stable_sort(order, order + 256, [&](int a, int b) {
+    if (left[a] != left[b]) return left[a] > left[b];
+    if (count[a] != count[b]) return count[a] > count[b];
+    return format[a] && !format[b];
+  });
+  const size_t nsingle = 15 - multi.size();
+  std::vector<uint8_t> singles;
+  for (int k = 0; k < 256 && singles.size() < nsingle; ++k) {
+    if (count[order[k]] == 0 && !format[order[k]]) break;
+    singles.push_back(static_cast<uint8_t>(order[k]));
+  }
+  std::sort(singles.begin(), singles.end());
+  DenseTable t;
+  std::memset(&t, 0, sizeof(t));
+  int code = 0;
+  for (uint8_t b : singles) {
+    t.bytes[code][0] = b;
+    t.len[code++] = 1;
+  }
+  for (const Candidate& c : multi) {
+    std::memcpy(t.bytes[code], c.bytes, 4);
+    t.len[code++] = static_cast<uint8_t>(c.len);
+  }
+  t.escape = static_cast<uint8_t>(code);
+  return t;
+}
+
+DenseEncoder::DenseEncoder(const DenseTable& t) : table(t), nmulti(0) {
+  CHECK(DenseTableValid(t)) << "dense pack: the table breaks the no-overlap rule";
+  std::memset(enc, kBad, sizeof(enc));
+  for (int c = 0; c < 16; ++c) {
+    if (t.len[c] == 1 && t.bytes[c][0] < 0x80) enc[t.bytes[c][0]] = static_cast<uint8_t>(c);
+    if (t.len[c] >= 2) {
+      mcode[nmulti] = static_cast<uint8_t>(c);
+      mlen[nmulti] = t.len[c];
+      std::memcpy(mbytes[nmulti], t.bytes[c], 4);
+      ++nmulti;
+    }
+  }
+}
+
+bool PackIsaSupportedDense(PackIsa isa) {
+#if DMLC_PACK_X86
+  if (isa == PackIsa::kAvx512) {
+    return PackIsaSupported(isa) && __builtin_cpu_supports("avx512vbmi2") &&
+           __builtin_cpu_supports("popcnt");
+  }
+#endif
+  return PackIsaSupported(isa);
+}
+
+size_t PackRangeDense(const uint8_t* text, size_t n, size_t block_begin, size_t block_end,
+                      const DenseEncoder& e, uint8_t* out, size_t* escapes, size_t* raw_blocks,
+                      PackIsa isa) {
+  const size_t nblocks = block_end - block_begin;
+  const size_t meta_bytes = DenseMetaBytes(nblocks);
+  std::memset(out + 2 * nblocks, 0, meta_bytes - 2 * nblocks);
+  uint8_t* payload = out + meta_bytes;
+  size_t pos = 0;
+  bool simd = false;
+#if DMLC_PACK_X86
+  static const bool have512 = PackIsaSupportedDense(PackIsa::kAvx512);
+  if ((isa == PackIsa::kAvx512 || (isa == PackIsa::kAuto && have512)) &&
+      e.nmulti <= kDenseMaxMulti) {
+    switch (e.nmulti) {
+#define DMLC_DENSE_CASE(NM)                                                                \
+  case NM:                                                                                 \
+    RangeAvx512Dense<NM>(text, n, block_begin, block_end, e, out, payload, &pos, escapes, \
+                         raw_blocks);                                                      \
+    break;
+      DMLC_DENSE_CASE(0)
+      DMLC_DENSE_CASE(1)
+      default:
+        static_assert(kDenseMaxMulti == 2, "a case per count of multi-byte entries");
+        DMLC_DENSE_CASE(2)
+#undef DMLC_DENSE_CASE
+    }
+    simd = true;
+  }
+#endif
+  if (!simd) {
+    for (size_t b = block_begin; b < block_end; ++b) {
+      const size_t off = b * kPackBlockBytes;
+      pos += BlockScalarDense(text + off, std::min(kPackBlockBytes, n - off), e, payload + pos,
+                              out + 2 * (b - block_begin), escapes, raw_blocks);
+    }
+  }
+  const size_t used = meta_bytes + pos;
+  const size_t length = DenseAlign(used, kDenseRangeAlign);
+  std::memset(out + used, 0, length - used);
+  return length;
+}
+
+void DenseWriteHeader(size_t n, size_t range_blocks, const DenseTable& table,
+                      const std::vector<DenseDirEntry>& dir, uint8_t* packed) {
+  DenseHeader h;
+  std::memset(&h, 0, sizeof(h));
+  h.n = n;
+  h.nranges = static_cast<uint32_t>(dir.size());
+  h.magic = kDenseMagic;
+  h.range_blocks = static_cast<uint32_t>(range_blocks);
+  h.escape = table.escape;
+  const size_t entry_bytes = DenseEntryBytes(table);
+  h.entry_bytes = static_cast<uint8_t>(entry_bytes);
+  const size_t total = DenseHeaderBytes(dir.size(), entry_bytes);
+  std::memset(packed + sizeof(h), 0, total - sizeof(h));
+  uint8_t* at = packed + sizeof(h);
+  for (int c = 0; c < 16; ++c) {
+    h.len[c / 2] |= static_cast<uint8_t>(table.len[c] << (4 * (c & 1)));
+    std::memcpy(at, table.bytes[c], table.len[c]);
+    at += table.len[c];
+  }
+  std::memcpy(packed, &h, sizeof(h));
+  if (!dir.empty()) {
+    std::memcpy(packed + DenseDirOffset(entry_bytes), dir.data(),
+                dir.size() * sizeof(DenseDirEntry));
+  }
+}
+
+void DenseCopyOut(const uint8_t* src, size_t bytes, uint8_t* dst) {
+#if DMLC_PACK_X86
+  static const bool have512 = __builtin_cpu_supports("avx512f");
+  if (have512 && bytes % 16 == 0 && (reinterpret_cast<uintptr_t>(dst) & 15) == 0) {
+    CopyOutAvx512(src, bytes, dst);
+    _mm_sfence();
+    return;
+  }
+#endif
+  std::memcpy(dst, src, bytes);
+}
+
+bool PackTextDense(const uint8_t* text, size_t n, const DenseTable& table, size_t range_blocks,
+                   double ratio, std::vector<uint8_t>* packed, PackIsa isa, size_t* escapes,
+                   size_t* raw_blocks) {
+  CHECK_GE(range_blocks, 1u);
+  const DenseEncoder encoder(table);
+  const size_t nranges = DenseRanges(n, range_blocks);
+  const size_t limit = ratio < 0 ? DenseMaxBytes(n, range_blocks)
+                                 : static_cast<size_t>(ratio * static_cast<double>(n));
+  std::vector<uint8_t> range(DenseRangeCapacity(range_blocks));
+  std::vector<DenseDirEntry> dir(nranges);
+  packed->assign(DenseHeaderBytes(nranges, DenseEntryBytes(table)), 0);
+  for (size_t r = 0; r < nranges; ++r) {
+    const size_t b0 = r * range_blocks, b1 = std::min(PackBlocks(n), b0 + range_blocks);
+    const size_t len =
+        PackRangeDense(text, n, b0, b1, encoder, range.data(), escapes, raw_blocks, isa);
+    dir[r].offset = static_cast<uint32_t>(packed->size());
+    dir[r].length = static_cast<uint32_t>(len);
+    packed->insert(packed->end(), range.begin(), range.begin() + len);
+    if (packed->size() > limit) return false;
+  }
+  if (packed->size() > limit) return false;
+  DenseWriteHeader(n, range_blocks, table, dir, packed->data());
+  return true;
+}
+
+bool IsDenseChunk(const uint8_t* packed, size_t bytes) {
+  if (bytes < sizeof(DenseHeader)) return false;
+  DenseHeader h;
+  std::memcpy(&h, packed, sizeof(h));
+  return h.magic == kDenseMagic;
+}
+
+namespace {
+struct DenseView {
+  DenseHeader h;
+  DenseTable table;
+  const uint8_t* dir;
+};
+
+DenseView ViewDense(const uint8_t* packed) {
+  DenseView v;
+  std::memcpy(&v.h, packed, sizeof(v.h));
+  std::memset(&v.table, 0, sizeof(v.table));
+  v.table.escape = v.h.escape;
+  const uint8_t* at = packed + sizeof(DenseHeader);
+  size_t left = v.h.entry_bytes;
+  for (int c = 0; c < 16; ++c) {
+    const uint8_t len = (v.h.len[c / 2] >> (4 * (c & 1))) & 15u;
+    v.table.len[c] = len;
+    if (len <= 4 && len <= left) {
+      std::memcpy(v.table.bytes[c], at, len);
+      at += len;
+      left -= len;
+    } else {
+      v.table.len[c] = 15;
+    }
+  }
+  v.dir = packed + DenseDirOffset(v.h.entry_bytes);
+  return v;
+}
+
+inline DenseDirEntry DirEntry(const DenseView& v, size_t r) {
+  DenseDirEntry e;
+  std::memcpy(&e, v.dir + r * sizeof(e), sizeof(e));
+  return e;
+}
+}
+
+size_t DenseCheck(const uint8_t* packed, size_t bytes) {
+  CHECK_GE(bytes, sizeof(DenseHeader)) << "not a dense chunk";
+  const DenseView v = ViewDense(packed);
+  CHECK_EQ(v.h.magic, kDenseMagic) << "not a dense chunk";
+  CHECK_LT(v.h.escape, 16u) << "dense chunk: escape code";
+  CHECK_LE(DenseDirOffset(v.h.entry_bytes), bytes) << "dense chunk: entries";
+  CHECK(DenseTableValid(v.table) && DenseEntryBytes(v.table) == v.h.entry_bytes)
+      << "dense chunk: table";
+  const size_t header_bytes = DenseHeaderBytes(v.h.nranges, v.h.entry_bytes);
+  const size_t n = v.h.n;
+  if (n == 0) {
+    CHECK_EQ(v.h.nranges, 0u);
+    return 0;
+  }
+  CHECK_GE(v.h.range_blocks, 1u) << "dense chunk: range_blocks";
+  CHECK_EQ(DenseRanges(n, v.h.range_blocks), v.h.nranges) << "dense chunk: range count";
+  CHECK_LE(header_bytes, bytes) << "dense chunk: directory";
+  for (size_t r = 0; r < v.h.nranges; ++r) {
+    const DenseDirEntry e = DirEntry(v, r);
+    CHECK(e.offset >= header_bytes &&
+          static_cast<size_t>(e.offset) + e.length <= bytes)
+        << "dense chunk: range " << r << " outside the chunk";
+    const size_t b0 = r * v.h.range_blocks;
+    const size_t nblocks = std::min<size_t>(v.h.range_blocks, PackBlocks(n) - b0);
+    size_t used = DenseMetaBytes(nblocks);
+    CHECK_LE(used, e.length) << "dense chunk: metadata of range " << r;
+    const uint8_t* meta = packed + e.offset;
+    for (size_t b = 0; b < nblocks; ++b) {
+      const size_t len = std::min(kPackBlockBytes, n - (b0 + b) * kPackBlockBytes);
+      const bool raw = meta[2 * b] == kDenseRawMeta && meta[2 * b + 1] == kDenseRawMeta;
+      if (!raw) {
+        CHECK(meta[2 * b] <= kPackBlockBytes / 2 &&
+              static_cast<size_t>(meta[2 * b]) + meta[2 * b + 1] <= kDenseMaxPayload)
+            << "dense chunk: metadata of block " << b0 + b;
+      }
+      used += raw ? len : static_cast<size_t>(meta[2 * b]) + meta[2 * b + 1];
+    }
+    CHECK_LE(used, e.length) << "dense chunk: payloads of range " << r;
+  }
+  return n;
+}
+
+DenseDirEntry DenseDirectory(const uint8_t* packed, size_t r) {
+  return DirEntry(ViewDense(packed), r);
+}
+
+void UnpackDenseReference(const uint8_t* packed, uint8_t* dst) {
+  const DenseView v = ViewDense(packed);
+  const size_t n = v.h.n;
+  for (size_t r = 0; r < v.h.nranges; ++r) {
+    const DenseDirEntry e = DirEntry(v, r);
+    const size_t b0 = r * v.h.range_blocks;
+    const size_t nblocks = std::min<size_t>(v.h.range_blocks, PackBlocks(n) - b0);
+    const uint8_t* meta = packed + e.offset;
+    const uint8_t* p = meta + DenseMetaBytes(nblocks);
+    for (size_t b = 0; b < nblocks; ++b) {
+      uint8_t* o = dst + (b0 + b) * kPackBlockBytes;
+      const size_t len = std::min(kPackBlockBytes, n - (b0 + b) * kPackBlockBytes);
+      if (meta[2 * b] == kDenseRawMeta && meta[2 * b + 1] == kDenseRawMeta) {
+        std::memcpy(o, p, len);
+        p += len;
+        continue;
+      }
+      const size_t nb = meta[2 * b], nlit = meta[2 * b + 1];
+      const uint8_t* lit = p + nb;
+      size_t at = 0;
+      for (size_t k = 0; k < 2 * nb && at < len; ++k) {
+        const unsigned c = (k & 1) ? p[k / 2] >> 4 : p[k / 2] & 15u;
+        if (c == v.table.escape) {
+          o[at++] = *lit++;
+        } else {
+          for (int j = 0; j < v.table.len[c] && at < len; ++j) o[at++] = v.table.bytes[c][j];
+        }
+      }
+      p += nb + nlit;
+    }
+  }
+}
+
+}
+}
diff --git a/src/gpu/text_pack_dense.h b/src/gpu/text_pack_dense.h
--- /dev/null
+++ b/src/gpu/text_pack_dense.h
@@ -0,0 +1,105 @@
+#ifndef DMLC_SRC_GPU_TEXT_PACK_DENSE_H_
+#define DMLC_SRC_GPU_TEXT_PACK_DENSE_H_
+
+#include <cstddef>
+#include <cstdint>
+#include <vector>
+
+#include "./text_pack.h"
+
+namespace dmlc {
+namespace gpu {
+
+constexpr uint32_t kDenseMagic = 0x45534e44u;
+constexpr size_t kDenseMaxPayload = 192;
+constexpr size_t kDenseRangeAlign = 16;
+constexpr uint8_t kDenseRawMeta = 0xff;
+constexpr int kDenseMaxMulti = 2;
+
+struct DenseTable {
+  uint8_t bytes[16][4];
+  uint8_t len[16];
+  uint8_t escape;
+};
+
+struct DenseHeader {
+  uint64_t n;
+  uint32_t nranges;
+  uint32_t magic;
+  uint32_t range_blocks;
+  uint8_t escape;
+  uint8_t entry_bytes;
+  uint16_t reserved;
+  uint8_t len[8];
+};
+static_assert(sizeof(DenseHeader) == 32, "DenseHeader is 32 bytes");
+
+struct DenseDirEntry {
+  uint32_t offset;
+  uint32_t length;
+};
+
+inline size_t DenseAlign(size_t x, size_t a) { return (x + a - 1) / a * a; }
+inline size_t DenseRanges(size_t n, size_t range_blocks) {
+  return (PackBlocks(n) + range_blocks - 1) / range_blocks;
+}
+inline size_t DenseDirOffset(size_t entry_bytes) {
+  return sizeof(DenseHeader) + DenseAlign(entry_bytes, 8);
+}
+inline size_t DenseHeaderBytes(size_t nranges, size_t entry_bytes) {
+  return DenseAlign(DenseDirOffset(entry_bytes) + nranges * sizeof(DenseDirEntry),
+                    kDenseRangeAlign);
+}
+inline size_t DenseMetaBytes(size_t nblocks) { return DenseAlign(2 * nblocks, 16); }
+inline size_t DenseRangeCapacity(size_t nblocks) {
+  return DenseAlign(DenseMetaBytes(nblocks) + nblocks * kPackBlockBytes, kDenseRangeAlign) + 128;
+}
+inline size_t DenseMaxBytes(size_t n, size_t range_blocks) {
+  const size_t nranges = DenseRanges(n, range_blocks);
+  return DenseHeaderBytes(nranges, 60) + nranges * DenseRangeCapacity(range_blocks);
+}
+
+bool DenseCompatible(const uint8_t* a, int alen, const uint8_t* b, int blen);
+bool DenseTableValid(const DenseTable& t);
+inline size_t DenseEntryBytes(const DenseTable& t) {
+  size_t sum = 0;
+  for (int c = 0; c < 16; ++c) sum += t.len[c];
+  return sum;
+}
+DenseDirEntry DenseDirectory(const uint8_t* packed, size_t r);
+DenseTable DenseDefaultTable(bool csv, char delimiter);
+bool DenseMakeTable(const std::vector<std::vector<uint8_t>>& entries, DenseTable* out);
+
+DenseTable DenseSelectTable(const uint8_t* text, size_t n, bool csv, char delimiter);
+constexpr size_t kDenseSampleBytes = 4096;
+constexpr size_t kDenseSampleStride = size_t(4) << 20;
+
+struct DenseEncoder {
+  DenseTable table;
+  uint8_t enc[256];
+  int nmulti;
+  uint8_t mcode[15], mlen[15];
+  uint8_t mbytes[15][4];
+  explicit DenseEncoder(const DenseTable& t);
+};
+
+size_t PackRangeDense(const uint8_t* text, size_t n, size_t block_begin, size_t block_end,
+                      const DenseEncoder& encoder, uint8_t* out, size_t* escapes,
+                      size_t* raw_blocks, PackIsa isa = PackIsa::kAuto);
+bool PackIsaSupportedDense(PackIsa isa);
+
+void DenseWriteHeader(size_t n, size_t range_blocks, const DenseTable& table,
+                      const std::vector<DenseDirEntry>& dir, uint8_t* packed);
+void DenseCopyOut(const uint8_t* src, size_t bytes, uint8_t* dst);
+
+bool PackTextDense(const uint8_t* text, size_t n, const DenseTable& table, size_t range_blocks,
+                   double ratio, std::vector<uint8_t>* packed, PackIsa isa = PackIsa::kAuto,
+                   size_t* escapes = nullptr, size_t* raw_blocks = nullptr);
+
+bool IsDenseChunk(const uint8_t* packed, size_t bytes);
+size_t DenseCheck(const uint8_t* packed, size_t bytes);
+void UnpackDenseReference(const uint8_t* packed, uint8_t* dst);
+
+}
+}
+#endif
diff --git a/src/gpu/unpack_kernels.hip b/src/gpu/unpack_kernels.hip
--- a/src/gpu/unpack_kernels.hip
+++ b/src/gpu/unpack_kernels.hip
@@ -1,7 +1,10 @@
 #include <hip/hip_runtime.h>
+
+#include <algorithm>
 
 #include "./kernels.h"
 #include "./text_pack.h"
+#include "./text_pack_dense.h"
 
 namespace dmlc {
 namespace gpu {
@@ -60,6 +63,152 @@
   const size_t off = static_cast<size_t>(index[e]) * kPackBlockBytes + threadIdx.x;
   if (off < n) dst[off] = static_cast<char>(raw[e * kPackBlockBytes + threadIdx.x]);
 }
+constexpr int kGroupBlocks = 16;
+constexpr int kGroupBytes = kGroupBlocks * static_cast<int>(kPackBlockBytes);
+
+__device__ __forceinline__ uint32_t dense_payload(const uint8_t* meta, uint32_t i, uint32_t raw_len) {
+  const uint32_t m0 = meta[2 * i], m1 = meta[2 * i + 1];
+  return (m0 == kDenseRawMeta && m1 == kDenseRawMeta) ? raw_len : m0 + m1;
+}
+
+__global__ __launch_bounds__(kThreads) void k_unpack_dense(const uint8_t* __restrict__ packed,
+                                                           size_t n, uint32_t range_blocks,
+                                                           uint32_t groups_per_range,
+                                                           char* __restrict__ dst) {
+  __shared__ uint32_t s_out[kGroupBytes / 4 + 4];
+  __shared__ uint32_t s_entry[16], s_count[16];
+  __shared__ uint32_t s_off[kGroupBlocks];
+  __shared__ uint32_t s_base;
+  const uint32_t tid = threadIdx.x, lane = tid & 63u, wave = tid >> 6;
+  const uint32_t r = blockIdx.x / groups_per_range, g = blockIdx.x % groups_per_range;
+  const size_t total_blocks = (n + kPackBlockBytes - 1) / kPackBlockBytes;
+  const size_t rb0 = static_cast<size_t>(r) * range_blocks;
+  const uint32_t nblocks =
+      static_cast<uint32_t>(total_blocks - rb0 < range_blocks ? total_blocks - rb0 : range_blocks);
+  const uint32_t gb0 = g * kGroupBlocks;
+  if (gb0 >= nblocks) return;
+  const uint32_t gblocks = nblocks - gb0 < kGroupBlocks ? nblocks - gb0 : kGroupBlocks;
+
+  const DenseHeader* h = reinterpret_cast<const DenseHeader*>(packed);
+  const uint32_t entry_bytes = h->entry_bytes;
+  if (tid < 16) {
+    uint32_t at = 0, len = 0;
+    for (uint32_t c = 0; c <= tid; ++c) {
+      at += len;
+      len = (h->len[c / 2] >> (4 * (c & 1))) & 15u;
+    }
+    uint32_t e = 0;
+    for (uint32_t j = 0; j < 4; ++j) {
+      if (j < len && at + j < entry_bytes) {
+        e |= static_cast<uint32_t>(packed[sizeof(DenseHeader) + at + j]) << (8 * j);
+      }
+    }
+    s_entry[tid] = e;
+    s_count[tid] = tid == h->escape ? 0x10001u : (len <= 4 ? len : 0u);
+  }
+  if (tid == 0) s_base = 0;
+  const DenseDirEntry dir = reinterpret_cast<const DenseDirEntry*>(
+      packed + sizeof(DenseHeader) + ((entry_bytes + 7u) & ~7u))[r];
+  const uint8_t* meta = packed + dir.offset;
+  const uint8_t* payload = meta + ((2u * nblocks + 15u) & ~15u);
+  __syncthreads();
+  uint32_t sum = 0;
+  for (uint32_t i = tid; i < gb0; i += kThreads) sum += dense_payload(meta, i, kPackBlockBytes);
+  for (int d = 32; d > 0; d >>= 1) sum += __shfl_down(sum, d);
+  if (lane == 0 && sum != 0) atomicAdd(&s_base, sum);
+  __syncthreads();
+  if (tid < gblocks) {
+    uint32_t off = s_base;
+    for (uint32_t j = 0; j < tid; ++j) off += dense_payload(meta, gb0 + j, kPackBlockBytes);
+    s_off[tid] = off;
+  }
+  __syncthreads();
+
+  uint8_t* out8 = reinterpret_cast<uint8_t*>(s_out);
+  for (uint32_t k = 0; k < 4; ++k) {
+    const uint32_t bi = wave * 4 + k;
+    if (bi >= gblocks) break;
+    const size_t tb = rb0 + gb0 + bi;
+    const uint32_t blen = static_cast<uint32_t>(
+        n - tb * kPackBlockBytes < kPackBlockBytes ? n - tb * kPackBlockBytes : kPackBlockBytes);
+    const uint8_t* p = payload + s_off[bi];
+    uint8_t* o = out8 + bi * kPackBlockBytes;
+    const uint32_t m0 = meta[2 * (gb0 + bi)], m1 = meta[2 * (gb0 + bi) + 1];
+    if (m0 == kDenseRawMeta && m1 == kDenseRawMeta) {
+      for (uint32_t j = lane; j < blen; j += 64) o[j] = p[j];
+      continue;
+    }
+    const uint8_t* lit = p + m0;
+    const uint32_t b0 = 2 * lane < m0 ? p[2 * lane] : 0u;
+    const uint32_t b1 = 2 * lane + 1 < m0 ? p[2 * lane + 1] : 0u;
+    const uint32_t code[4] = {b0 & 15u, b0 >> 4, b1 & 15u, b1 >> 4};
+    uint32_t cnt[4], total = 0;
+#pragma unroll
+    for (int q = 0; q < 4; ++q) {
+      cnt[q] = s_count[code[q]];
+      total += cnt[q];
+    }
+    uint32_t incl = total;
+    for (int d = 1; d < 64; d <<= 1) {
+      const uint32_t t = __shfl_up(incl, d);
+      if (lane >= static_cast<uint32_t>(d)) incl += t;
+    }
+    uint32_t pos = (incl - total) & 0xffffu, esc = (incl - total) >> 16;
+#pragma unroll
+    for (int q = 0; q < 4; ++q) {
+      const uint32_t len = cnt[q] & 0xffffu;
+      if (cnt[q] >> 16) {
+        if (pos < blen && esc < m1) o[pos] = lit[esc];
+        ++esc;
+      } else {
+        const uint32_t e = s_entry[code[q]];
+#pragma unroll
+        for (uint32_t j = 0; j < 4; ++j) {
+          if (j < len && pos + j < blen) o[pos + j] = static_cast<uint8_t>(e >> (8 * j));
+        }
+      }
+      pos += len;
+    }
+  }
+  __syncthreads();
+
+  const size_t start = (rb0 + gb0) * kPackBlockBytes;
+  const uint32_t gbytes = static_cast<uint32_t>(
+      n - start < static_cast<size_t>(gblocks) * kPackBlockBytes ? n - start
+                                                                 : gblocks * kPackBlockBytes);
+  char* span = dst + start;
+  const uint32_t lead = static_cast<uint32_t>(reinterpret_cast<uintptr_t>(span) & 15u);
+  const uint32_t ngroups = (gbytes + lead + 15u) / 16u;
+  for (uint32_t gi = tid; gi < ngroups; gi += kThreads) {
+    const int s = static_cast<int>(gi * 16u) - static_cast<int>(lead);
+    if (s >= 0 && s + 16 <= static_cast<int>(gbytes)) {
+      const uint32_t w = static_cast<uint32_t>(s) >> 2;
+      const uint32_t sh = (static_cast<uint32_t>(s) & 3u) * 8u;
+      uint32_t v[5];
+#pragma unroll
+      for (int q = 0; q < 5; ++q) v[q] = s_out[w + q];
+      if (sh != 0) {
+#pragma unroll
+        for (int q = 0; q < 4; ++q) v[q] = (v[q] >> sh) | (v[q + 1] << (32u - sh));
+      }
+      *reinterpret_cast<uint4*>(span + s) = make_uint4(v[0], v[1], v[2], v[3]);
+    } else {
+      const int j0 = s < 0 ? 0 : s;
+      const int j1 = s + 16 < static_cast<int>(gbytes) ? s + 16 : static_cast<int>(gbytes);
+      for (int j = j0; j < j1; ++j) span[j] = static_cast<char>(out8[j]);
+    }
+  }
+}
+}
+
+void LaunchUnpackDense(const void* packed, size_t n, uint32_t nranges, uint32_t range_blocks,
+                       char* dst, hipStream_t stream) {
+  if (n == 0 || nranges == 0) return;
+  const size_t blocks = PackBlocks(n);
+  const size_t per_range = std::min<size_t>(range_blocks, blocks);
+  const uint32_t groups = static_cast<uint32_t>((per_range + kGroupBlocks - 1) / kGroupBlocks);
+  hipLaunchKernelGGL(k_unpack_dense, dim3(nranges * groups), dim3(kThreads), 0, stream,
+                     static_cast<const uint8_t*>(packed), n, range_blocks, groups, dst);
 }
 
 void LaunchUnpackText(const void* packed, size_t n, uint32_t nexc, const uint8_t alphabet[16],
diff --git a/src/python/module.cc b/src/python/module.cc
--- a/src/python/module.cc
+++ b/src/python/module.cc
@@ -22,7 +22,9 @@
 #include <vector>
 
 #include "../gpu/kernels.h"
+#include "../gpu/pack_pool.h"
 #include "../gpu/text_pack.h"
+#include "../gpu/text_pack_dense.h"
 #include "../io/http.h"
 #include "../io/line_split.h"
 #include "../io/recordio_split.h"
@@ -456,6 +458,9 @@
     d["raw_chunks"] = s.raw_chunks;
     d["link_bytes"] = s.link_bytes;
     d["exception_blocks"] = s.exception_blocks;
+    d["dense_chunks"] = s.dense_chunks;
+    d["escape_bytes"] = s.escape_bytes;
+    d["raw_blocks"] = s.raw_blocks;
     d["head_packed"] = s.head_packed;
     d["pack_sec"] = s.pack_sec;
     d["wait_pack_sec"] = s.wait_pack_sec;
@@ -670,9 +675,24 @@
 }
 
 py::object PackTextPy(const std::string& text, const std::string& format, const std::string& delimiter,
-                      double ratio, int isa) {
+                      double ratio, int isa, const std::string& code, size_t range_blocks) {
   CHECK(format == "libsvm" || format == "libfm" || format == "csv") << "unknown format " << format;
   CHECK_EQ(delimiter.size(), 1U) << "delimiter must be one character";
+  CHECK(code == "nibble" || code == "dense") << "unknown code " << code;
+  if (code == "dense") {
+    CHECK(gpu::PackIsaSupportedDense(static_cast<gpu::PackIsa>(isa)))
+        << "instruction set not supported";
+    CHECK_GE(range_blocks, 1U);
+    const uint8_t* bytes = reinterpret_cast<const uint8_t*>(text.data());
+    const gpu::DenseTable table =
+        gpu::DenseSelectTable(bytes, text.size(), format == "csv", delimiter[0]);
+    std::vector<uint8_t> packed;
+    if (!gpu::PackTextDense(bytes, text.size(), table, range_blocks, ratio, &packed,
+                            static_cast<gpu::PackIsa>(isa))) {
+      return py::none();
+    }
+    return py::bytes(reinterpret_cast<const char*>(packed.data()), packed.size());
+  }
   CHECK(gpu::PackIsaSupported(static_cast<gpu::PackIsa>(isa))) << "instruction set not supported";
   uint8_t alphabet[16];
   gpu::PackAlphabet(format == "csv", delimiter[0], alphabet);
@@ -684,7 +704,44 @@
   return py::bytes(reinterpret_cast<const char*>(packed.data()), packed.size());
 }
 
+py::object PackTextPoolPy(const std::string& text, const std::string& format,
+                          const std::string& delimiter, size_t range_blocks, int threads,
+                          const std::string& code, double ratio) {
+  CHECK(format == "libsvm" || format == "libfm" || format == "csv") << "unknown format " << format;
+  CHECK_EQ(delimiter.size(), 1U) << "delimiter must be one character";
+  CHECK(code == "nibble" || code == "dense") << "unknown code " << code;
+  CHECK_GE(range_blocks, 1U);
+  uint8_t alphabet[16];
+  gpu::PackAlphabet(format == "csv", delimiter[0], alphabet);
+  const bool dense = code == "dense";
+  const size_t n = text.size();
+  std::vector<uint8_t> out(
+      (dense ? gpu::DenseMaxBytes(n, range_blocks) : gpu::PackedBytes(n, gpu::PackBlocks(n))) + 128);
+  gpu::PackJob job;
+  job.ptr = text.data();
+  job.size = n;
+  job.ratio = ratio;
+  job.out = out.data() + ((64 - (reinterpret_cast<uintptr_t>(out.data()) & 63)) & 63);
+  {
+    py::gil_scoped_release release;
+    gpu::PackPool pool(threads, alphabet, 0, range_blocks,
+                       dense ? gpu::PackCode::kDense : gpu::PackCode::kNibble, format == "csv",
+                       delimiter[0]);
+    pool.Push(&job);
+    pool.Wait(&job);
+  }
+  if (job.state.load() != gpu::PackJob::kPacked) return py::none();
+  return py::bytes(reinterpret_cast<const char*>(job.out), job.packed_bytes);
+}
+
+bool IsDense(const std::string& packed) {
+  return gpu::IsDenseChunk(reinterpret_cast<const uint8_t*>(packed.data()), packed.size());
+}
+
 size_t CheckedPackedSize(const std::string& packed) {
+  if (IsDense(packed)) {
+    return gpu::DenseCheck(reinterpret_cast<const uint8_t*>(packed.data()), packed.size());
+  }
   CHECK_GE(packed.size(), sizeof(gpu::PackedHeader)) << "not a packed chunk";
   const gpu::PackedView v = gpu::ViewPacked(reinterpret_cast<const uint8_t*>(packed.data()));
   CHECK_EQ(v.bytes, packed.size()) << "packed chunk size mismatch";
@@ -698,6 +755,11 @@
 
 py::bytes UnpackTextReferencePy(const std::string& packed) {
   std::string out(CheckedPackedSize(packed), '\0');
+  if (IsDense(packed)) {
+    gpu::UnpackDenseReference(reinterpret_cast<const uint8_t*>(packed.data()),
+                              reinterpret_cast<uint8_t*>(&out[0]));
+    return py::bytes(out);
+  }
   gpu::UnpackReference(reinterpret_cast<const uint8_t*>(packed.data()),
                        reinterpret_cast<uint8_t*>(&out[0]));
   return py::bytes(out);
@@ -705,14 +767,26 @@
 
 py::bytes UnpackTextDevicePy(const std::string& packed, size_t dst_offset, size_t pad, int fill) {
   const size_t n = CheckedPackedSize(packed);
-  const gpu::PackedView v = gpu::ViewPacked(reinterpret_cast<const uint8_t*>(packed.data()));
+  const bool dense = IsDense(packed);
+  gpu::PackedView v;
+  gpu::DenseHeader dh;
+  if (dense) {
+    std::memcpy(&dh, packed.data(), sizeof(dh));
+  } else {
+    v = gpu::ViewPacked(reinterpret_cast<const uint8_t*>(packed.data()));
+  }
   gpu::DeviceBuffer src(packed.size()), dst(dst_offset + n + pad);
   gpu::Stream stream;
   DMLC_HIP_CHECK(hipMemcpyAsync(src.get(), packed.data(), packed.size(), hipMemcpyHostToDevice,
                                 stream.get()));
   DMLC_HIP_CHECK(hipMemsetAsync(dst.get(), fill, dst_offset + n + pad, stream.get()));
-  gpu::LaunchUnpackText(src.get(), n, v.header.nexc, v.header.alphabet,
-                        dst.get<char>() + dst_offset, stream.get());
+  if (dense) {
+    gpu::LaunchUnpackDense(src.get(), n, dh.nranges, dh.range_blocks,
+                           dst.get<char>() + dst_offset, stream.get());
+  } else {
+    gpu::LaunchUnpackText(src.get(), n, v.header.nexc, v.header.alphabet,
+                          dst.get<char>() + dst_offset, stream.get());
+  }
   DMLC_HIP_CHECK(hipGetLastError());
   std::string out(dst_offset + n + pad, '\0');
   DMLC_HIP_CHECK(hipMemcpyAsync(&out[0], dst.get(), out.size(), hipMemcpyDeviceToHost, stream.get()));
@@ -740,7 +814,13 @@
   m.doc() = "dmlc-core for MI355X: native runtime bindings";
   py::register_exception<dmlc::Error>(m, "DMLCError");
   m.def("pack_text", &PackTextPy, py::arg("text"), py::arg("format") = "libsvm",
-        py::arg("delimiter") = ",", py::arg("ratio") = gpu::kPackMaxRatio, py::arg("isa") = 0);
+        py::arg("delimiter") = ",", py::arg("ratio") = gpu::kPackMaxRatio, py::arg("isa") = 0,
+        py::arg("code") = "nibble", py::arg("range_blocks") = gpu::PackPool::kRangeBlocks);
+  m.def("pack_text_pool", &PackTextPoolPy, py::arg("text"), py::arg("format") = "libsvm",
+        py::arg("delimiter") = ",", py::arg("range_blocks") = gpu::PackPool::kRangeBlocks,
+        py::arg("threads") = 4, py::arg("code") = "dense", py::arg("ratio") = -1.0);
+  m.def("pack_isa_supported_dense",
+        [](int isa) { return gpu::PackIsaSupportedDense(static_cast<gpu::PackIsa>(isa)); });
   m.def("pack_isa_supported",
         [](int isa) { return gpu::PackIsaSupported(static_cast<gpu::PackIsa>(isa)); });
   m.def("unpack_text_reference", &UnpackTextReferencePy, py::arg("packed"));
```

New measurement: 197.8 million (median of 6 runs). 11.5% higher.
